# Openflight-sim/OPEN_Ludwig

Hardware: AMD Instinct MI355X
Metric: MLUPS (million lattice updates/s) at 256^3 D3Q27; % of HBM roofline (higher is better)
Workload: dtype f32

## Files before the change

### include/ludwig_hip.h

```cpp
#ifndef LUDWIG_HIP_H
#define LUDWIG_HIP_H

#include <stddef.h>
#include <stdint.h>

#ifdef __cplusplus
extern "C" {
#endif

#define LUDWIG_ABI_VERSION 1

#define LUDWIG_OK              0
#define LUDWIG_ERR_INVALID    -1
#define LUDWIG_ERR_HIP        -2
#define LUDWIG_ERR_NO_DEVICE  -3
#define LUDWIG_ERR_ALLOC      -4
#define LUDWIG_ERR_STATE      -5

enum LudwigField {
    LUDWIG_F = 0,
    LUDWIG_F_TEMP = 1,
    LUDWIG_F_POST = 2,
    LUDWIG_F_OLD = 3,
    LUDWIG_RHO = 4,
// ... 67 lines not shown
int  ludwig_level_upload(LudwigLevel *level, int field, const void *host, size_t bytes);
int  ludwig_level_download(const LudwigLevel *level, int field, void *host, size_t bytes);
int  ludwig_level_block_order(const LudwigLevel *level, int32_t *ref_to_internal);

int  ludwig_level_field_ptr(const LudwigLevel *level, int field, void **device_ptr, size_t *bytes);
int  ludwig_level_field_layout(const LudwigLevel *level, int field, int32_t *components, int64_t *block_stride, int64_t *component_stride);

int  ludwig_init_equilibrium(LudwigLevel *level);

int  ludwig_step(LudwigLevel *level, const LudwigLevel *parent, int64_t t_sub,
                 float u_curr, float parent_tau, float temporal_weight,
                 const LudwigStepFlags *flags);

int  ludwig_stream_collide(LudwigLevel *level, const LudwigLevel *parent, int64_t t_sub,
                           float u_curr, float parent_tau, float temporal_weight,
                           const LudwigStepFlags *flags, int part);
int  ludwig_bouzidi_correction(LudwigLevel *level, int64_t t_sub, float q_min_threshold);

int  ludwig_save_old(LudwigLevel *level, int64_t t_sub);

int  ludwig_execute_timestep_batch(LudwigLevel *const *levels, int32_t n_levels, int64_t t_start, int32_t batch_size,
                                   float u_curr, const LudwigStepFlags *flags);

enum { LUDWIG_OBSERVE_PROBES = 0, LUDWIG_OBSERVE_SURFACE = 1, LUDWIG_OBSERVE_FORCES = 2, LUDWIG_OBSERVE_TRACERS = 3,
       LUDWIG_OBSERVE_FLUXES = 4, LUDWIG_OBSERVE_MODES = 5 };
typedef struct LudwigBatchObserver {
    int32_t kind;
    void   *set;
    int64_t start_step;
    int32_t interval;
} LudwigBatchObserver;
int  ludwig_execute_timestep_batch_observed(LudwigLevel *const *levels, int32_t n_levels, int64_t t_start, int32_t batch_size,
                                            float u_curr, const LudwigStepFlags *flags, const LudwigBatchObserver *observers,
                                            int32_t n_observers);

int  ludwig_sync(const LudwigLevel *level);

typedef struct LudwigSurfaceParams {
    float   dx;
    float   tau;
    float   offset_x, offset_y, offset_z;
    float   pressure_scale, stress_scale;
    int32_t search_radius;
} LudwigSurfaceParams;

int  ludwig_map_surface_stresses(const LudwigLevel *level, int vel_field, int32_t n_triangles, const float *centers,
                                 const float *normals, const LudwigSurfaceParams *sp,
                                 float *pressure, float *shear_x, float *shear_y, float *shear_z);

int  ludwig_level_rho_min(const LudwigLevel *level, float *rho_min);

int  ludwig_level_set_rho_store(LudwigLevel *level, int every_step);

enum LudwigStat { LUDWIG_STAT_RHO = 0, LUDWIG_STAT_VEL = 1, LUDWIG_STAT_VEL2 = 2 };
int  ludwig_level_stats_reset(LudwigLevel *level);
int  ludwig_level_stats_accumulate(LudwigLevel *level, int64_t t_sub);
int  ludwig_level_stats_download(const LudwigLevel *level, int stat, double *host, size_t bytes, int64_t *n_samples);

int  ludwig_level_monitor(LudwigLevel *level, int64_t t_sub, int64_t *counts, int64_t *cells, float *extremes, double *sums);

#define LUDWIG_WALL_BINS 194
typedef struct LudwigWallCensus {
    uint64_t near_cells, evaluated, log_law, forced, non_finite;
    uint32_t min_bits, max_bits;
    uint64_t hist[LUDWIG_WALL_BINS];
} LudwigWallCensus;
int  ludwig_level_wall_census(LudwigLevel *level, int64_t t_sub, LudwigWallCensus *out);

typedef struct LudwigWallSurface LudwigWallSurface;
int  ludwig_wall_surface_create(LudwigLevel *level, int32_t n_tri, const int32_t *blocks, const int32_t *cells, const float *normals,
                                const LudwigSurfaceParams *sp, LudwigWallSurface **out);
void ludwig_wall_surface_destroy(LudwigWallSurface *set);
int  ludwig_wall_surface_compute(LudwigWallSurface *set, int64_t t_sub);
int  ludwig_wall_surface_download(LudwigWallSurface *set, float *values, size_t bytes);

enum LudwigGradField { LUDWIG_GRAD_VORTICITY = 0 , LUDWIG_GRAD_Q = 1  };
int  ludwig_level_gradient_fields_compute(LudwigLevel *level, int vel_field, float scale);
int  ludwig_level_gradient_fields_download(const LudwigLevel *level, int which, float *host, size_t bytes);

enum LudwigIsoScalar { LUDWIG_ISO_DENSITY = 0, LUDWIG_ISO_VELOCITY_MAGNITUDE = 1, LUDWIG_ISO_Q_CRITERION = 2,
                       LUDWIG_ISO_VORTICITY_MAGNITUDE = 3 };
#define LUDWIG_ISO_REFUSED     1
int  ludwig_level_isosurface_extract(LudwigLevel *level, int which, int vel_field, float scale, float value, const uint8_t *skip,
                                     const int32_t *cell_lo, const int32_t *cell_hi, int64_t max_triangles, int64_t *n_triangles);
int  ludwig_level_isosurface_download(LudwigLevel *level, float *positions, size_t position_bytes, float *attributes,
                                      size_t attribute_bytes, int32_t *keys, size_t key_bytes);

typedef struct LudwigProbes LudwigProbes;
int  ludwig_probes_create(LudwigLevel *const *levels, int32_t n_levels, int32_t n_probes, const int32_t *level_index,
                          const int32_t *blocks, const int32_t *cells, const float *weights, int32_t capacity, LudwigProbes **out);
void ludwig_probes_destroy(LudwigProbes *probes);
int  ludwig_probes_sample(LudwigProbes *probes, int32_t level_index, int64_t t_sub);
int  ludwig_probes_download(LudwigProbes *probes, float *values, int64_t *steps, int32_t max_samples, int32_t *n_samples);
int  ludwig_execute_timestep_batch_probes(LudwigLevel *const *levels, int32_t n_levels, int64_t t_start, int32_t batch_size,
                                          float u_curr, const LudwigStepFlags *flags, LudwigProbes *probes, int64_t start_step,
                                          int32_t interval);

typedef struct LudwigSurfaceStats LudwigSurfaceStats;
int  ludwig_surface_stats_create(LudwigLevel *level, int32_t n_tri, const int32_t *blocks, const int32_t *cells, const float *wall_dist,
                                 const float *normals, const LudwigSurfaceParams *sp, LudwigSurfaceStats **out);
void ludwig_surface_stats_destroy(LudwigSurfaceStats *stats);
int  ludwig_surface_stats_reset(LudwigSurfaceStats *stats);
int  ludwig_surface_stats_accumulate(LudwigSurfaceStats *stats, int64_t t_sub);
int  ludwig_surface_stats_download(LudwigSurfaceStats *stats, double *sums, size_t bytes, int64_t *n_samples);

typedef struct LudwigBatchSamplers {
// ... 130 lines not shown
```

### open_ludwig_amd/_lib.py

```python
from __future__ import annotations

import ctypes as C
import os

_HERE = os.path.dirname(os.path.abspath(__file__))
LIB_PATH = os.environ.get("LUDWIG_HIP_LIB") or os.path.join(_HERE, "csrc", "libludwig_hip.so")

F, F_TEMP, F_POST, F_OLD, RHO, RHO_OLD, VEL, VEL_TEMP, VEL_OLD, OBSTACLE, SPONGE, WALL_DIST = range(12)
FIELD_NAMES = {
    "f": F, "f_temp": F_TEMP, "f_post_collision": F_POST, "f_old": F_OLD, "rho": RHO, "rho_old": RHO_OLD,
    "vel": VEL, "vel_temp": VEL_TEMP, "vel_old": VEL_OLD, "obstacle": OBSTACLE, "sponge": SPONGE,
    "wall_dist": WALL_DIST,
}
STAT_RHO, STAT_VEL, STAT_VEL2 = range(3)
STAT_NAMES = {"rho": (STAT_RHO, 1), "vel": (STAT_VEL, 3), "vel2": (STAT_VEL2, 6)}
GRAD_VORTICITY, GRAD_Q = range(2)
GRAD_NAMES = {"vorticity": (GRAD_VORTICITY, 3), "q": (GRAD_Q, 1)}
SLICE_GRADIENT = 1
ISO_NAMES = {"density": 0, "velocity_magnitude": 1, "q_criterion": 2, "vorticity_magnitude": 3}
ISO_REFUSED = 1
SUBGRID_FIELD_NAMES = {"nu": 0, "code": 1}
SUBGRID_SUM_NAMES = {"nu": 0, "nunu": 1, "eps": 2}
PART_ALL, PART_BOUNDARY, PART_INTERIOR = 0, 1, 2

OBSERVE_PROBES, OBSERVE_SURFACE, OBSERVE_FORCES, OBSERVE_TRACERS, OBSERVE_FLUXES = range(5)
OBSERVE_MODES = 5

EXPORTED_SYMBOLS = [
    "ludwig_abi_version", "ludwig_last_error", "ludwig_device_count",
    "ludwig_level_create", "ludwig_level_destroy", "ludwig_level_set_stream", "ludwig_level_add_post_collision_readers", "ludwig_level_set_order",
    "ludwig_level_upload", "ludwig_level_download", "ludwig_level_field_ptr",
    "ludwig_init_equilibrium", "ludwig_step", "ludwig_stream_collide", "ludwig_bouzidi_correction",
    "ludwig_save_old", "ludwig_execute_timestep_batch", "ludwig_execute_timestep_batch_observed", "ludwig_sync", "ludwig_halo_pack", "ludwig_halo_unpack", "ludwig_level_info",
    "ludwig_map_surface_stresses", "ludwig_level_rho_min", "ludwig_level_block_order",
    "ludwig_stream_create", "ludwig_stream_destroy", "ludwig_level_field_layout", "ludwig_level_set_rho_store",
    "ludwig_comm_unique_id", "ludwig_comm_create", "ludwig_comm_destroy", "ludwig_comm_allreduce_f32",
    "ludwig_halo_plan_create", "ludwig_halo_plan_destroy", "ludwig_halo_exchange", "ludwig_halo_wait",
    "ludwig_halo_plan_pack", "ludwig_halo_plan_unpack", "ludwig_halo_plan_buffers", "ludwig_halo_plan_timing", "ludwig_halo_plan_in_stream",
    "ludwig_halo_plan_exchange_ms", "ludwig_step_distributed",
    "ludwig_level_stats_reset", "ludwig_level_stats_accumulate", "ludwig_level_stats_download",
    "ludwig_level_gradient_fields_compute", "ludwig_level_gradient_fields_download",
    "ludwig_level_subgrid_fields_compute", "ludwig_level_subgrid_fields_download", "ludwig_level_subgrid_stats_reset",
    "ludwig_level_subgrid_stats_accumulate", "ludwig_level_subgrid_stats_download",
    "ludwig_probes_create", "ludwig_probes_destroy", "ludwig_probes_sample", "ludwig_probes_download",
    "ludwig_execute_timestep_batch_probes",
    "ludwig_surface_stats_create", "ludwig_surface_stats_destroy", "ludwig_surface_stats_reset", "ludwig_surface_stats_accumulate",
    "ludwig_surface_stats_download", "ludwig_execute_timestep_batch_sampled",
    "ludwig_slices_create", "ludwig_slices_destroy", "ludwig_slices_sample", "ludwig_slices_download",
    "ludwig_streamlines_create", "ludwig_streamlines_destroy", "ludwig_streamlines_trace", "ludwig_streamlines_download",
    "ludwig_tracers_create", "ludwig_tracers_destroy", "ludwig_tracers_advance", "ludwig_tracers_snapshot", "ludwig_tracers_download",
    "ludwig_execute_timestep_batch_tracers",
    "ludwig_level_monitor",
    "ludwig_level_isosurface_extract", "ludwig_level_isosurface_download",
    "ludwig_level_wall_census", "ludwig_wall_surface_create", "ludwig_wall_surface_destroy", "ludwig_wall_surface_compute",
    "ludwig_wall_surface_download",
    "ludwig_force_series_create", "ludwig_force_series_destroy", "ludwig_force_series_sample", "ludwig_force_series_download",
    "ludwig_execute_timestep_batch_loads",
    "ludwig_flux_planes_create", "ludwig_flux_planes_destroy", "ludwig_flux_planes_sample", "ludwig_flux_planes_download",
    "ludwig_modes_create", "ludwig_modes_destroy", "ludwig_modes_reset", "ludwig_modes_accumulate", "ludwig_modes_download",
]
UNIQUE_ID_BYTES = 128
HALO_GROUPS = ("f", "vel", "f_post", "rho")


class LudwigError(RuntimeError):
    def __init__(self, code: int, msg: str):
        super().__init__(f"libludwig_hip error {code}: {msg}")
        self.code = code


class LevelHost(C.Structure):
    _fields_ = [
        ("level_id", C.c_int32), ("n_blocks", C.c_int32), ("n_owned", C.c_int32), ("tau", C.c_float),
        ("grid_dim_x", C.c_int32), ("grid_dim_y", C.c_int32), ("grid_dim_z", C.c_int32),
        ("block_pointer", C.c_void_p), ("neighbor_table", C.c_void_p),
        ("map_x", C.c_void_p), ("map_y", C.c_void_p), ("map_z", C.c_void_p),
        ("obstacle", C.c_void_p), ("sponge", C.c_void_p), ("wall_dist", C.c_void_p),
        ("enable_temporal_interpolation", C.c_int32), ("n_boundary_cells", C.c_int32),
        ("bouzidi_q_map", C.c_void_p), ("bouzidi_cell_block", C.c_void_p),
        ("bouzidi_cell_x", C.c_void_p), ("bouzidi_cell_y", C.c_void_p), ("bouzidi_cell_z", C.c_void_p),
        ("comm_boundary", C.c_void_p), ("store_post_collision_everywhere", C.c_int32),
    ]


class StepFlags(C.Structure):
    _fields_ = [
        ("domain_nx", C.c_int32), ("domain_ny", C.c_int32), ("domain_nz", C.c_int32),
        ("is_symmetric", C.c_int32), ("wall_model_active", C.c_int32), ("use_temporal_interp", C.c_int32),
        ("sponge_blend_distributions", C.c_int32),
        ("c_wale", C.c_float), ("nu_sgs_background", C.c_float), ("inlet_turbulence", C.c_float),
        ("q_min_threshold", C.c_float),
    ]


class SurfaceParams(C.Structure):
    _fields_ = [
        ("dx", C.c_float), ("tau", C.c_float), ("offset_x", C.c_float), ("offset_y", C.c_float), ("offset_z", C.c_float),
        ("pressure_scale", C.c_float), ("stress_scale", C.c_float), ("search_radius", C.c_int32),
    ]


class BatchObserver(C.Structure):
    _fields_ = [("kind", C.c_int32), ("set", C.c_void_p), ("start_step", C.c_int64), ("interval", C.c_int32)]


class BatchSamplers(C.Structure):
    _fields_ = [
        ("probes", C.c_void_p), ("probes_start_step", C.c_int64), ("probes_interval", C.c_int32),
        ("surface", C.c_void_p), ("surface_start_step", C.c_int64), ("surface_interval", C.c_int32),
    ]


# ... 17 lines not shown

class LevelInfo(C.Structure):
    _fields_ = [
        ("n_blocks", C.c_int32), ("n_owned", C.c_int32), ("n_fast_blocks", C.c_int32),
        ("n_general_blocks", C.c_int32), ("n_boundary_cells", C.c_int32),
        ("has_temporal_storage", C.c_int32), ("has_post_collision", C.c_int32), ("n_xrun_blocks", C.c_int32),
        ("device_bytes", C.c_int64),
    ]


_lib = None


def load() -> C.CDLL:
    global _lib
    if _lib is not None:
        return _lib
    if not os.path.exists(LIB_PATH):
        raise FileNotFoundError(
            f"{LIB_PATH} not found: build the HIP extension first (python -c 'import __graft_entry__ as g; g.build()')")
    lib = C.CDLL(LIB_PATH)
    vp, i32, i64, f32 = C.c_void_p, C.c_int, C.c_int64, C.c_float
    sig = {
        "ludwig_abi_version": (C.c_int, []),
        "ludwig_last_error": (C.c_char_p, []),
        "ludwig_device_count": (C.c_int, [C.POINTER(C.c_int)]),
        "ludwig_level_create": (C.c_int, [C.POINTER(LevelHost), i32, C.POINTER(vp)]),
        "ludwig_level_destroy": (None, [vp]),
        "ludwig_level_set_stream": (C.c_int, [vp, vp]),
        "ludwig_level_add_post_collision_readers": (C.c_int, [vp, vp, i64]),
        "ludwig_level_set_order": (C.c_int, [vp, i32, vp, i64]),
        "ludwig_level_upload": (C.c_int, [vp, i32, vp, C.c_size_t]),
        "ludwig_level_download": (C.c_int, [vp, i32, vp, C.c_size_t]),
        "ludwig_level_field_ptr": (C.c_int, [vp, i32, C.POINTER(vp), C.POINTER(C.c_size_t)]),
        "ludwig_init_equilibrium": (C.c_int, [vp]),
        "ludwig_step": (C.c_int, [vp, vp, i64, f32, f32, f32, C.POINTER(StepFlags)]),
        "ludwig_stream_collide": (C.c_int, [vp, vp, i64, f32, f32, f32, C.POINTER(StepFlags), i32]),
        "ludwig_bouzidi_correction": (C.c_int, [vp, i64, f32]),
        "ludwig_save_old": (C.c_int, [vp, i64]),
        "ludwig_execute_timestep_batch": (C.c_int, [C.POINTER(vp), i32, i64, i32, f32, C.POINTER(StepFlags)]),
        "ludwig_execute_timestep_batch_observed": (C.c_int, [C.POINTER(vp), i32, i64, i32, f32, C.POINTER(StepFlags),
                                                             C.POINTER(BatchObserver), i32]),
        "ludwig_sync": (C.c_int, [vp]),
        "ludwig_halo_pack": (C.c_int, [vp, i32, vp, i64, vp, vp]),
        "ludwig_halo_unpack": (C.c_int, [vp, i32, vp, i64, vp, vp]),
        "ludwig_map_surface_stresses": (C.c_int, [vp, i32, i32, vp, vp, C.POINTER(SurfaceParams), vp, vp, vp, vp]),
        "ludwig_level_info": (C.c_int, [vp, C.POINTER(LevelInfo)]),
        "ludwig_level_rho_min": (C.c_int, [vp, C.POINTER(C.c_float)]),
        "ludwig_level_block_order": (C.c_int, [vp, vp]),
        "ludwig_stream_create": (C.c_int, [i32, i32, C.POINTER(vp)]),
        "ludwig_stream_destroy": (C.c_int, [i32, vp]),
        "ludwig_level_field_layout": (C.c_int, [vp, i32, C.POINTER(C.c_int32), C.POINTER(C.c_int64), C.POINTER(C.c_int64)]),
        "ludwig_level_set_rho_store": (C.c_int, [vp, i32]),
        "ludwig_comm_unique_id": (C.c_int, [vp]),
        "ludwig_comm_create": (C.c_int, [vp, i32, i32, i32, C.POINTER(vp)]),
        "ludwig_comm_destroy": (None, [vp]),
        "ludwig_comm_allreduce_f32": (C.c_int, [vp, vp, i32, i32]),
        "ludwig_halo_plan_create": (C.c_int, [vp, vp, C.POINTER(HaloPlanDesc), C.POINTER(vp)]),
        "ludwig_halo_plan_destroy": (None, [vp]),
        "ludwig_halo_exchange": (C.c_int, [vp, i32, vp, vp]),
        "ludwig_halo_wait": (C.c_int, [vp]),
        "ludwig_halo_plan_pack": (C.c_int, [vp, i32, i32, vp]),
        "ludwig_halo_plan_unpack": (C.c_int, [vp, i32, i32, vp]),
        "ludwig_halo_plan_buffers": (C.c_int, [vp, i32, C.POINTER(vp), C.POINTER(i64), C.POINTER(vp), C.POINTER(i64)]),
        "ludwig_halo_plan_timing": (C.c_int, [vp, i32]),
        "ludwig_halo_plan_in_stream": (C.c_int, [vp, i32]),
        "ludwig_halo_plan_exchange_ms": (C.c_int, [vp, vp, i32, C.POINTER(C.c_int32)]),
        "ludwig_step_distributed": (C.c_int, [vp, vp, vp, i64, f32, f32, f32, C.POINTER(StepFlags)]),
        "ludwig_level_stats_reset": (C.c_int, [vp]),
        "ludwig_level_stats_accumulate": (C.c_int, [vp, i64]),
        "ludwig_level_monitor": (C.c_int, [vp, i64, vp, vp, vp, vp]),
        "ludwig_level_stats_download": (C.c_int, [vp, i32, vp, C.c_size_t, C.POINTER(C.c_int64)]),
        "ludwig_level_gradient_fields_compute": (C.c_int, [vp, i32, f32]),
        "ludwig_level_gradient_fields_download": (C.c_int, [vp, i32, vp, C.c_size_t]),
        "ludwig_level_subgrid_fields_compute": (C.c_int, [vp, i32]),
        "ludwig_level_subgrid_fields_download": (C.c_int, [vp, i32, vp, C.c_size_t]),
        "ludwig_level_subgrid_stats_reset": (C.c_int, [vp]),
        "ludwig_level_subgrid_stats_accumulate": (C.c_int, [vp, i64]),
        "ludwig_level_subgrid_stats_download": (C.c_int, [vp, i32, vp, C.c_size_t, C.POINTER(C.c_int64)]),
        "ludwig_probes_create": (C.c_int, [C.POINTER(vp), i32, i32, vp, vp, vp, vp, i32, C.POINTER(vp)]),
        "ludwig_probes_destroy": (None, [vp]),
        "ludwig_probes_sample": (C.c_int, [vp, i32, i64]),
        "ludwig_probes_download": (C.c_int, [vp, vp, vp, i32, C.POINTER(C.c_int32)]),
        "ludwig_execute_timestep_batch_probes": (C.c_int, [C.POINTER(vp), i32, i64, i32, f32, C.POINTER(StepFlags), vp, i64, i32]),
        "ludwig_surface_stats_create": (C.c_int, [vp, i32, vp, vp, vp, vp, C.POINTER(SurfaceParams), C.POINTER(vp)]),
        "ludwig_surface_stats_destroy": (None, [vp]),
        "ludwig_surface_stats_reset": (C.c_int, [vp]),
        "ludwig_surface_stats_accumulate": (C.c_int, [vp, i64]),
        "ludwig_surface_stats_download": (C.c_int, [vp, vp, C.c_size_t, C.POINTER(C.c_int64)]),
        "ludwig_execute_timestep_batch_sampled": (C.c_int, [C.POINTER(vp), i32, i64, i32, f32, C.POINTER(StepFlags), C.POINTER(BatchSamplers)]),
        "ludwig_slices_create": (C.c_int, [C.POINTER(vp), i32, i32, vp, vp, vp, vp, vp, vp, i32, C.POINTER(vp)]),
        "ludwig_slices_destroy": (None, [vp]),
        "ludwig_slices_sample": (C.c_int, [vp, i64]),
        "ludwig_slices_download": (C.c_int, [vp, vp, C.c_size_t]),
        "ludwig_streamlines_create": (C.c_int, [vp, i32, i32, vp, vp, f32, f32, i32, C.POINTER(vp)]),
        "ludwig_streamlines_destroy": (None, [vp]),
        "ludwig_streamlines_trace": (C.c_int, [vp, i64]),
        "ludwig_streamlines_download": (C.c_int, [vp, vp, vp, vp, C.c_size_t]),
        "ludwig_tracers_create": (C.c_int, [vp, i32, i32, vp, i32, i32, f32, C.POINTER(vp)]),
        "ludwig_tracers_destroy": (None, [vp]),
        "ludwig_tracers_advance": (C.c_int, [vp, i64]),
        "ludwig_tracers_snapshot": (C.c_int, [vp, i64]),
        "ludwig_tracers_download": (C.c_int, [vp, vp, C.c_size_t, C.POINTER(C.c_int64)]),
        "ludwig_level_isosurface_extract": (C.c_int, [vp, i32, i32, f32, f32, vp, vp, vp, i64, C.POINTER(C.c_int64)]),
        "ludwig_level_isosurface_download": (C.c_int, [vp, vp, C.c_size_t, vp, C.c_size_t, vp, C.c_size_t]),
        "ludwig_level_wall_census": (C.c_int, [vp, i64, C.POINTER(WallCensus)]),
# ... 104 lines not shown
```

### open_ludwig_amd/blocks.py

```python
from __future__ import annotations

import ctypes as C
from typing import List, Optional, Sequence, Tuple

import numpy as np

from . import _lib

BLOCK_SIZE = 8


def build_lattice_arrays():
    cx, cy, cz, w = [], [], [], []
    for dz in (-1, 0, 1):
        for dy in (-1, 0, 1):
            for dx in (-1, 0, 1):
                cx.append(dx); cy.append(dy); cz.append(dz)
                d2 = dx * dx + dy * dy + dz * dz
                w.append(np.float32(8) / np.float32(27) if d2 == 0 else np.float32(2) / np.float32(27) if d2 == 1
                         else np.float32(1) / np.float32(54) if d2 == 2 else np.float32(1) / np.float32(216))
    cx, cy, cz = (np.array(a, dtype=np.int32) for a in (cx, cy, cz))
    w = np.array(w, dtype=np.float32)
    opp = np.zeros(27, np.int32); my = np.zeros(27, np.int32); mz = np.zeros(27, np.int32)
    for i in range(27):
# ... 204 lines not shown
        return bool(self.info().has_post_collision)

    def add_post_collision_readers(self, offsets: np.ndarray) -> None:
        o = np.ascontiguousarray(offsets, dtype=np.int64)
        _lib.check(self._lib.ludwig_level_add_post_collision_readers(self.handle, o.ctypes.data if o.size else None, o.size))

    def set_stream(self, hip_stream: int) -> None:
        _lib.check(self._lib.ludwig_level_set_stream(self.handle, C.c_void_p(hip_stream)))

    def set_order(self, items: np.ndarray, part: int = _lib.PART_ALL) -> None:
        items = np.ascontiguousarray(items, dtype=np.int32)
        _lib.check(self._lib.ludwig_level_set_order(self.handle, part, items.ctypes.data, items.size))

    def _shape(self, name: str):
        B, n = BLOCK_SIZE, self.n_blocks
        if name in ("f", "f_temp", "f_post_collision", "f_old"):
            return (B, B, B, n, 27)
        if name in ("vel", "vel_temp", "vel_old"):
            return (B, B, B, n, 3)
        return (B, B, B, n)

    def upload(self, name: str, host: np.ndarray) -> None:
        dt = _FIELD_DTYPES.get(name, np.float32)
        a = host.view(np.uint8) if host.dtype == np.bool_ else host
        a = np.asfortranarray(a, dtype=dt)
        if a.shape != self._shape(name):
            raise ValueError(f"{name}: shape {a.shape} != {self._shape(name)}")
        _lib.check(self._lib.ludwig_level_upload(self.handle, _lib.FIELD_NAMES[name], a.ctypes.data, a.nbytes))

    def download(self, name: str) -> np.ndarray:
        dt = _FIELD_DTYPES.get(name, np.float32)
        a = np.empty(self._shape(name), dtype=dt, order="F")
        _lib.check(self._lib.ludwig_level_download(self.handle, _lib.FIELD_NAMES[name], a.ctypes.data, a.nbytes))
        return a.view(np.bool_) if name == "obstacle" else a

    def block_order(self) -> np.ndarray:
        a = np.zeros(self.n_blocks, dtype=np.int32)
        _lib.check(self._lib.ludwig_level_block_order(self.handle, a.ctypes.data))
        return a

    def field_ptr(self, name: str) -> Tuple[int, int]:
        p, n = C.c_void_p(), C.c_size_t()
        _lib.check(self._lib.ludwig_level_field_ptr(self.handle, _lib.FIELD_NAMES[name], C.byref(p), C.byref(n)))
        return p.value, n.value

    def field_layout(self, name: str) -> Tuple[int, int, int]:
        k, bs, cs = C.c_int32(), C.c_int64(), C.c_int64()
        _lib.check(self._lib.ludwig_level_field_layout(self.handle, _lib.FIELD_NAMES[name], C.byref(k), C.byref(bs), C.byref(cs)))
        return int(k.value), int(bs.value), int(cs.value)

    def set_rho_store(self, every_step: bool) -> None:
        _lib.check(self._lib.ludwig_level_set_rho_store(self.handle, 1 if every_step else 0))

    def rho_min(self) -> float:
        v = C.c_float()
        _lib.check(self._lib.ludwig_level_rho_min(self.handle, C.byref(v)))
        return float(v.value)

    def stats_reset(self) -> None:
        _lib.check(self._lib.ludwig_level_stats_reset(self.handle))

    def stats_accumulate(self, t_sub: int) -> None:
        _lib.check(self._lib.ludwig_level_stats_accumulate(self.handle, int(t_sub)))

    def stats_download(self, stat: str) -> Tuple[np.ndarray, int]:
        sid, k = _lib.STAT_NAMES[stat]
        B = BLOCK_SIZE
        a = np.empty((B, B, B, self.n_blocks) + ((k,) if k > 1 else ()), dtype=np.float64, order="F")
        n = C.c_int64(0)
        _lib.check(self._lib.ludwig_level_stats_download(self.handle, sid, a.ctypes.data if a.size else None, a.nbytes, C.byref(n)))
        return a, int(n.value)

    def monitor(self, t_sub: int):
        from . import monitor as monitor_mod
        counts, cells = np.zeros(2, np.int64), np.zeros(16, np.int64)
        extremes, sums = np.zeros(3, np.float32), np.zeros(2, np.float64)
        _lib.check(self._lib.ludwig_level_monitor(self.handle, int(t_sub), counts.ctypes.data, cells.ctypes.data, extremes.ctypes.data,
                                                  sums.ctypes.data))
        return monitor_mod.from_arrays(counts, cells, extremes, sums)

    def gradient_fields(self, vel_name: str, scale) -> Tuple[np.ndarray, np.ndarray]:
        if vel_name not in ("vel", "vel_temp"):
            raise ValueError(f"gradient fields: vel_name must be 'vel' or 'vel_temp', got {vel_name!r}")
        _lib.check(self._lib.ludwig_level_gradient_fields_compute(self.handle, _lib.FIELD_NAMES[vel_name], float(np.float32(scale))))
        B = BLOCK_SIZE
        out = []
        for name in ("vorticity", "q"):
            gid, k = _lib.GRAD_NAMES[name]
            a = np.empty((B, B, B, self.n_blocks) + ((k,) if k > 1 else ()), dtype=np.float32, order="F")
            _lib.check(self._lib.ludwig_level_gradient_fields_download(self.handle, gid, a.ctypes.data if a.size else None, a.nbytes))
            out.append(a)
        return out[0], out[1]

    def isosurface(self, field: str, value, vel_name: str = "vel", scale=1.0, skip=None, cell_lo=(0, 0, 0), cell_hi=None,
                   max_triangles: int = 50_000_000, download: bool = True):
        from .isosurface import CELL_MAX, check_field
        if vel_name not in ("vel", "vel_temp"):
            raise ValueError(f"isosurface: vel_name must be 'vel' or 'vel_temp', got {vel_name!r}")
        which = check_field(field)
        lo = np.ascontiguousarray(cell_lo, dtype=np.int32).reshape(3)
        hi = np.full(3, CELL_MAX, np.int32) if cell_hi is None else np.ascontiguousarray(cell_hi, dtype=np.int32).reshape(3)
        sk = None
        if skip is not None:
            sk = np.ascontiguousarray(skip, dtype=np.uint8).reshape(-1)
            if sk.size != self.n_blocks:
                raise ValueError(f"isosurface: skip has {sk.size} entries for {self.n_blocks} blocks")
# ... 72 lines not shown
```

### open_ludwig_amd/csrc/kernels.hpp

```cpp
#pragma once

#include <hip/hip_runtime.h>
#include <stdint.h>
#include <type_traits>

#include "lattice.hpp"
#include "jl_math.h"

namespace lw {

struct SCParams {
    const float *f_in;
    float *f_out;
    float *f_post;
    const uint32_t *post_rows;
    const float *vel_in;
    float *vel_out;
    float *rho;
    const uint8_t *obstacle;
    const float *sponge;
    const float *wall_dist;
    const int32_t *meta;
    const int32_t *items;
    const float *pf_new, *pf_old, *prho_new, *prho_old, *pvel_new, *pvel_old;
    float tau, tau_parent, c_wale, nu_bg, u_inlet, inlet_turbulence, temporal_weight;
    int32_t is_level_1, is_symmetric, nx_g, ny_g, nz_g;
    int32_t wall_model, seed, use_temporal, sponge_blend;
    float *f_iface;
    int32_t n_iface_blocks;
    int32_t store_rho;
    float *rho_old_save;
};

template <int K, int N, class F>
__device__ __forceinline__ void static_for(F &&f)
{
    if constexpr (K < N) {
        f(std::integral_constant<int, K>{});
        static_for<K + 1, N>(f);
    }
}

__device__ __forceinline__ float jl_max(float a, float b)
{
    return (a != a) ? a : ((b != b) ? b : (a > b ? a : b));
}
__device__ __forceinline__ float jl_clamp(float x, float lo, float hi)
{
    return x > hi ? hi : (x < lo ? lo : x);
}
__device__ __forceinline__ float jl_pow(float x, float y) { return lw_powf(x, y); }
__device__ __forceinline__ float jl_log(float x) { return lw_logf(x); }

template <int C>
__device__ __forceinline__ void acc_signed(float &sum, bool &empty, float v)
{
    if constexpr (C != 0) {
        const float t = C > 0 ? v : -v;
        sum = empty ? t : sum + t;
        empty = false;
    }
}
template <int K>
__device__ __forceinline__ float cdot(float a, float b, float c)
{
    float s = 0.0f;
    bool empty = true;
    acc_signed<CX(K)>(s, empty, a);
    acc_signed<CY(K)>(s, empty, b);
    acc_signed<CZ(K)>(s, empty, c);
    return s;
}

__device__ __forceinline__ float gradient_noise(int32_t gx, int32_t gy, int32_t gz, int32_t seed)
{
    uint32_t h = (uint32_t)gx * 374761393u + (uint32_t)gy * 668265263u + (uint32_t)gz * 1274126177u + (uint32_t)seed;
    h = (h ^ (h >> 16)) * 0x85ebca6bu;
    h = (h ^ (h >> 13)) * 0xc2b2ae35u;
    h = h ^ (h >> 16);
    return ((float)(h & 0xFFFFu) / 32768.0f) - 1.0f;
}

__device__ __forceinline__ float calculate_equilibrium(float rho, float ux, float uy, float uz, float w_k,
                                                       float cx, float cy, float cz)
// ... 110 lines not shown
    const bool xo = cx == 1 ? l.x0 : (cx == -1 ? l.x7 : false);
    const bool yo = cy == 1 ? l.y0 : (cy == -1 ? l.y7 : false);
    const int c00 = n.id[g][4], cX = n.id[g][4 - cx], cY = n.id[g][4 - 3 * cy], cXY = n.id[g][4 - cx - 3 * cy];
    int sel = c00;
    if constexpr (cx != 0 && cy != 0) sel = xo ? (yo ? cXY : cX) : (yo ? cY : c00);
    else if constexpr (cx != 0) sel = xo ? cX : c00;
    else if constexpr (cy != 0) sel = yo ? cY : c00;
    return sel;
}
constexpr int SUBGRID_NO_OP1 = 0, SUBGRID_NO_DENOM = 1, SUBGRID_FLOOR = 2, SUBGRID_MODEL = 3;
struct WaleState {
    float nu_eddy, s2;
    int code;
};
__device__ __forceinline__ WaleState wale_state(float g11, float g12, float g13, float g21, float g22, float g23, float g31, float g32,
                                                float g33, float c_wale, float nu_bg)
{
    const float gsq11 = g11 * g11 + g12 * g21 + g13 * g31;
    const float gsq12 = g11 * g12 + g12 * g22 + g13 * g32;
    const float gsq13 = g11 * g13 + g12 * g23 + g13 * g33;
    const float gsq21 = g21 * g11 + g22 * g21 + g23 * g31;
    const float gsq22 = g21 * g12 + g22 * g22 + g23 * g32;
    const float gsq23 = g21 * g13 + g22 * g23 + g23 * g33;
    const float gsq31 = g31 * g11 + g32 * g21 + g33 * g31;
    const float gsq32 = g31 * g12 + g32 * g22 + g33 * g32;
    const float gsq33 = g31 * g13 + g32 * g23 + g33 * g33;

    const float tr_gsq = gsq11 + gsq22 + gsq33;
    const float tr_term = tr_gsq / 3.0f;
    const float Sd11 = gsq11 - tr_term, Sd22 = gsq22 - tr_term, Sd33 = gsq33 - tr_term;
    const float Sd12 = 0.5f * (gsq12 + gsq21), Sd13 = 0.5f * (gsq13 + gsq31), Sd23 = 0.5f * (gsq23 + gsq32);
    const float S12 = 0.5f * (g12 + g21), S13 = 0.5f * (g13 + g31), S23 = 0.5f * (g23 + g32);
    const float OP1 = Sd11 * Sd11 + Sd22 * Sd22 + Sd33 * Sd33 + 2.0f * (Sd12 * Sd12 + Sd13 * Sd13 + Sd23 * Sd23);
    const float OP2 = g11 * g11 + g22 * g22 + g33 * g33 + 2.0f * (S12 * S12 + S13 * S13 + S23 * S23);

    WaleState w;
    w.code = SUBGRID_NO_OP1;
    float nu_eddy = 0.0f;
    if (OP1 > 1.0e-12f) {
        const float OP1_32 = OP1 * sqrtf(OP1);
        const float OP2_52 = OP2 * OP2 * sqrtf(jl_max(OP2, 1.0e-12f));
        const float denom = OP2_52 + OP1 * sqrtf(sqrtf(jl_max(OP1, 1.0e-12f)));
        w.code = SUBGRID_NO_DENOM;
        if (denom > 1.0e-12f) {
            nu_eddy = (c_wale * c_wale) * OP1_32 / denom;
            w.code = nu_eddy > nu_bg ? SUBGRID_MODEL : SUBGRID_FLOOR;
        }
    }
    w.nu_eddy = jl_max(nu_eddy, nu_bg);
    w.s2 = 2.0f * OP2;
    return w;
}

template <bool POST, bool WALL>
__device__ __forceinline__ void finish_cell(const SCParams &p, const int flags, const Own own, float (&fs)[Q],
                                            const float ux_E, const float uy_E, const float uz_E, const float ux_W, const float uy_W, const float uz_W,
                                            const float ux_N, const float uy_N, const float uz_N, const float ux_S, const float uy_S, const float uz_S,
                                            const float ux_T, const float uy_T, const float uz_T, const float ux_B, const float uy_B, const float uz_B)
{
    float rho = 0.0f, jx = 0.0f, jy = 0.0f, jz = 0.0f;
    static_for<0, Q>([&](auto kc) {
        constexpr int k = decltype(kc)::value;
        constexpr int cx = CX(k), cy = CY(k), cz = CZ(k);
        const float val = fs[k];
        rho += val;
        if constexpr (cx == 1) jx += val; else if constexpr (cx == -1) jx -= val;
        if constexpr (cy == 1) jy += val; else if constexpr (cy == -1) jy -= val;
        if constexpr (cz == 1) jz += val; else if constexpr (cz == -1) jz -= val;
    });

    bool store_post = false;
    if constexpr (POST) {
        if (flags & FLAG_STORE_POST) {
            store_post = true;
            if (p.post_rows) {
                const int zu = __builtin_amdgcn_readfirstlane((int)(own.cell4 >> 8));
                const uint32_t w = p.post_rows[(size_t)own.b * 2 + (zu >> 2)];
                store_post = ((w >> ((zu & 3) * 8 + ((own.cell4 >> 5) & 7))) & 1u) != 0;
            }
        }
    }
    bool is_obs = false;
    if (flags & FLAG_HAS_OBSTACLE) is_obs = p.obstacle[(size_t)own.b * CELLS + (own.cell4 >> 2)] != 0;
    if (is_obs) {
        st_f32(p.vel_out, own.b, V_BLOCK_BYTES, own.cell4, 0.0f);
        st_f32(p.vel_out, own.b, V_BLOCK_BYTES, COMP_BYTES + own.cell4, 0.0f);
        st_f32(p.vel_out, own.b, V_BLOCK_BYTES, 2 * COMP_BYTES + own.cell4, 0.0f);
        if (p.rho_old_save) st_f32(p.rho_old_save, own.b, S_BLOCK_BYTES, own.cell4, ld_own(p.rho, own.b, S_BLOCK_BYTES, own.cell4));
        if (p.store_rho) st_f32(p.rho, own.b, S_BLOCK_BYTES, own.cell4, 1.0f);
        static_for<0, Q>([&](auto kc) {
            constexpr int k = decltype(kc)::value;
            const float f_coll = fs[OPP(k)];
            st_f32(p.f_out, own.b, F_BLOCK_BYTES, k * COMP_BYTES + own.cell4, f_coll);
            if constexpr (POST) { if (store_post) st_f32(p.f_post, own.b, F_BLOCK_BYTES, k * COMP_BYTES + own.cell4, f_coll); }
        });
        return;
    }

    rho = jl_max(rho, 0.01f);
    const float inv_rho = 1.0f / rho;
    float ux = jx * inv_rho, uy = jy * inv_rho, uz = jz * inv_rho;

    if (flags & FLAG_HAS_SPONGE) {
        const float sp = ld_own(p.sponge, own.b, S_BLOCK_BYTES, own.cell4);
        if (sp > 0.0f) {
            const float rho_target = 1.0f, ux_target = p.u_inlet;
            rho = rho * (1.0f - sp) + rho_target * sp;
            ux = ux * (1.0f - sp) + ux_target * sp;
            uy = uy * (1.0f - sp);
            uz = uz * (1.0f - sp);
            if (p.sponge_blend == 1) {
                static_for<0, Q>([&](auto kc) {
                    constexpr int k = decltype(kc)::value;
                    const float feq_target = calculate_equilibrium(rho_target, ux_target, 0.0f, 0.0f, WEIGHT(k),
                                                                   (float)CX(k), (float)CY(k), (float)CZ(k));
                    fs[k] = fs[k] * (1.0f - sp) + feq_target * sp;
                });
            }
        }
    }

    float Fx = 0.0f, Fy = 0.0f, Fz = 0.0f;
    float ux_eq = ux, uy_eq = uy, uz_eq = uz;
    if constexpr (WALL) {
        if (flags & FLAG_HAS_NEAR_WALL) {
            const float u_mag = sqrtf(ux * ux + uy * uy + uz * uz);
            const float force_mag = wall_model_force_mag(ld_own(p.wall_dist, own.b, S_BLOCK_BYTES, own.cell4), p.tau, rho, u_mag);
            if (force_mag >= 0.0f) {
                Fx = -force_mag * ux / u_mag;
                Fy = -force_mag * uy / u_mag;
                Fz = -force_mag * uz / u_mag;
            }
        }
        ux_eq = ux + 0.5f * Fx * inv_rho;
        uy_eq = uy + 0.5f * Fy * inv_rho;
        uz_eq = uz + 0.5f * Fz * inv_rho;
    }
    const float usq_eq = ux_eq * ux_eq + uy_eq * uy_eq + uz_eq * uz_eq;

    st_f32(p.vel_out, own.b, V_BLOCK_BYTES, own.cell4, ux);
    st_f32(p.vel_out, own.b, V_BLOCK_BYTES, COMP_BYTES + own.cell4, uy);
    st_f32(p.vel_out, own.b, V_BLOCK_BYTES, 2 * COMP_BYTES + own.cell4, uz);
    if (p.rho_old_save) st_f32(p.rho_old_save, own.b, S_BLOCK_BYTES, own.cell4, ld_own(p.rho, own.b, S_BLOCK_BYTES, own.cell4));
    if (p.store_rho) st_f32(p.rho, own.b, S_BLOCK_BYTES, own.cell4, rho);

    const float g11 = 0.5f * (ux_E - ux_W), g12 = 0.5f * (ux_N - ux_S), g13 = 0.5f * (ux_T - ux_B);
    const float g21 = 0.5f * (uy_E - uy_W), g22 = 0.5f * (uy_N - uy_S), g23 = 0.5f * (uy_T - uy_B);
    const float g31 = 0.5f * (uz_E - uz_W), g32 = 0.5f * (uz_N - uz_S), g33 = 0.5f * (uz_T - uz_B);

    const float gsq11 = g11 * g11 + g12 * g21 + g13 * g31;
    const float gsq12 = g11 * g12 + g12 * g22 + g13 * g32;
    const float gsq13 = g11 * g13 + g12 * g23 + g13 * g33;
    const float gsq21 = g21 * g11 + g22 * g21 + g23 * g31;
    const float gsq22 = g21 * g12 + g22 * g22 + g23 * g32;
    const float gsq23 = g21 * g13 + g22 * g23 + g23 * g33;
    const float gsq31 = g31 * g11 + g32 * g21 + g33 * g31;
    const float gsq32 = g31 * g12 + g32 * g22 + g33 * g32;
    const float gsq33 = g31 * g13 + g32 * g23 + g33 * g33;

    const float tr_gsq = gsq11 + gsq22 + gsq33;
    const float tr_term = tr_gsq / 3.0f;
    const float Sd11 = gsq11 - tr_term, Sd22 = gsq22 - tr_term, Sd33 = gsq33 - tr_term;
    const float Sd12 = 0.5f * (gsq12 + gsq21), Sd13 = 0.5f * (gsq13 + gsq31), Sd23 = 0.5f * (gsq23 + gsq32);
    const float S12 = 0.5f * (g12 + g21), S13 = 0.5f * (g13 + g31), S23 = 0.5f * (g23 + g32);
    const float OP1 = Sd11 * Sd11 + Sd22 * Sd22 + Sd33 * Sd33 + 2.0f * (Sd12 * Sd12 + Sd13 * Sd13 + Sd23 * Sd23);
    const float OP2 = g11 * g11 + g22 * g22 + g33 * g33 + 2.0f * (S12 * S12 + S13 * S13 + S23 * S23);

    float nu_eddy = 0.0f;
    if (OP1 > 1.0e-12f) {
        const float OP1_32 = OP1 * sqrtf(OP1);
        const float OP2_52 = OP2 * OP2 * sqrtf(jl_max(OP2, 1.0e-12f));
        const float denom = OP2_52 + OP1 * sqrtf(sqrtf(jl_max(OP1, 1.0e-12f)));
        if (denom > 1.0e-12f) nu_eddy = (p.c_wale * p.c_wale) * OP1_32 / denom;
    }
    nu_eddy = jl_max(nu_eddy, p.nu_bg);
    const float tau_turb = p.tau + nu_eddy * 3.0f;
    const float omega = 1.0f / jl_max(tau_turb, 0.500001f);

    float Pi_xx = 0.0f, Pi_yy = 0.0f, Pi_zz = 0.0f, Pi_xy = 0.0f, Pi_yz = 0.0f, Pi_zx = 0.0f;
    static_for<0, Q>([&](auto kc) {
        constexpr int k = decltype(kc)::value;
        constexpr int cx = CX(k), cy = CY(k), cz = CZ(k);
        const float cu = cdot<k>(ux_eq, uy_eq, uz_eq);
        const float feq = rho * WEIGHT(k) * (1.0f + 3.0f * cu + 4.5f * cu * cu - 1.5f * usq_eq);
        const float f_neq = fs[k] - feq;
        if constexpr (cx != 0) Pi_xx += f_neq;
        if constexpr (cy != 0) Pi_yy += f_neq;
        if constexpr (cz != 0) Pi_zz += f_neq;
        if constexpr (cx * cy == 1) Pi_xy += f_neq; else if constexpr (cx * cy == -1) Pi_xy -= f_neq;
        if constexpr (cy * cz == 1) Pi_yz += f_neq; else if constexpr (cy * cz == -1) Pi_yz -= f_neq;
        if constexpr (cz * cx == 1) Pi_zx += f_neq; else if constexpr (cz * cx == -1) Pi_zx -= f_neq;
    });

    const float one_m_omega = 1.0f - omega;
    const float one_m_half_omega = 1.0f - 0.5f * omega;
    static_for<0, Q>([&](auto kc) {
        constexpr int k = decltype(kc)::value;
        constexpr int cx = CX(k), cy = CY(k), cz = CZ(k);
        constexpr float w_k = WEIGHT(k);
        constexpr float cx_f = (float)cx, cy_f = (float)cy, cz_f = (float)cz;
        const float cu = cdot<k>(ux_eq, uy_eq, uz_eq);
        const float feq = rho * w_k * (1.0f + 3.0f * cu + 4.5f * cu * cu - 1.5f * usq_eq);
        constexpr float Q_xx = cx_f * cx_f - CS2_PHYSICS, Q_yy = cy_f * cy_f - CS2_PHYSICS, Q_zz = cz_f * cz_f - CS2_PHYSICS;
        float od = 0.0f;
        bool od_empty = true;
        acc_signed<cx * cy>(od, od_empty, Pi_xy);
        acc_signed<cy * cz>(od, od_empty, Pi_yz);
        acc_signed<cz * cx>(od, od_empty, Pi_zx);
        float inner = Pi_xx * Q_xx + Pi_yy * Q_yy + Pi_zz * Q_zz;
        if constexpr (cx * cy != 0 || cy * cz != 0 || cz * cx != 0) inner = inner + 2.0f * od;
        const float f_neq_reg = (w_k * 4.5f) * inner;
        float f_coll = feq + one_m_omega * f_neq_reg;
        if constexpr (WALL) {
            const float force_term = (w_k * 3.0f) * ((cx_f - ux + 3.0f * cu * cx_f) * Fx + (cy_f - uy + 3.0f * cu * cy_f) * Fy +
                                                     (cz_f - uz + 3.0f * cu * cz_f) * Fz);
            f_coll = f_coll + one_m_half_omega * force_term;
        }
        if constexpr (POST) { if (store_post) st_f32(p.f_post, own.b, F_BLOCK_BYTES, k * COMP_BYTES + own.cell4, f_coll); }
        st_f32(p.f_out, own.b, F_BLOCK_BYTES, k * COMP_BYTES + own.cell4, f_coll);
    });
}

__device__ __forceinline__ void finish_rho_only(const SCParams &p, const int flags, const Own own, const float (&fs)[Q])
{
    float rho = 0.0f;
    static_for<0, Q>([&](auto kc) { rho += fs[decltype(kc)::value]; });
    bool is_obs = false;
    if (flags & FLAG_HAS_OBSTACLE) is_obs = p.obstacle[(size_t)own.b * CELLS + (own.cell4 >> 2)] != 0;
    if (is_obs) { st_f32(p.rho, own.b, S_BLOCK_BYTES, own.cell4, 1.0f); return; }
    rho = jl_max(rho, 0.01f);
    if (flags & FLAG_HAS_SPONGE) {
        const float sp = ld_own(p.sponge, own.b, S_BLOCK_BYTES, own.cell4);
        if (sp > 0.0f) rho = rho * (1.0f - sp) + 1.0f * sp;
    }
    st_f32(p.rho, own.b, S_BLOCK_BYTES, own.cell4, rho);
}

__device__ __forceinline__ void patch_missing_sources(const SCParams &p, const int32_t *__restrict__ meta, const NeighbourIds &nbr,
                                                      const LanePos &l, const int z, const Own own, float (&fs)[Q])
{
    const int gx = (meta[NBR_BX] - 1) * BS + l.x + 1, gy = (meta[NBR_BY] - 1) * BS + l.y + 1, gz = (meta[NBR_BZ] - 1) * BS + z + 1;
    const float *iface_own = p.is_level_1 == 0 ? p.f_iface + (size_t)meta[NBR_GBI] * CELLS + (own.cell4 >> 2) : nullptr;
    static_for<0, Q>([&](auto kc) {
        constexpr int k = decltype(kc)::value;
        constexpr int cx = CX(k), cy = CY(k), cz = CZ(k);
        if constexpr (k != 13) {
            if (source_block<k>(nbr, l) < 0) {
                const int src_gx = gx - cx, src_gy = gy - cy, src_gz = gz - cz;
                const bool is_inlet = src_gx < 1, is_outlet = src_gx > p.nx_g;
                const bool is_y_min = src_gy < 1, is_y_max = src_gy > p.ny_g;
                const bool is_z_min = src_gz < 1, is_z_max = src_gz > p.nz_g;
                float val;
                if (is_inlet) {
                    const float noise = p.inlet_turbulence > 0.0f
                                            ? gradient_noise(gy, gz, p.seed, 1234) * p.inlet_turbulence * p.u_inlet
                                            : 0.0f;
                    const float u_inst = p.u_inlet + noise;
                    const float cu_in = (float)cx * u_inst;
                    val = WEIGHT(k) * (1.0f + 3.0f * cu_in + 4.5f * cu_in * cu_in - 1.5f * u_inst * u_inst);
                } else if (is_outlet) {
                    const float cu_out = (float)cx * p.u_inlet;
                    val = WEIGHT(k) * (1.0f + 3.0f * cu_out + 4.5f * cu_out * cu_out - 1.5f * p.u_inlet * p.u_inlet);
                } else if (is_y_min && p.is_symmetric == 1) {
                    val = ld_own(p.f_in, own.b, F_BLOCK_BYTES, MIRROR_Y(k) * COMP_BYTES + own.cell4);
                } else if (is_y_min || is_y_max) {
                    val = ld_own(p.f_in, own.b, F_BLOCK_BYTES, MIRROR_Y(k) * COMP_BYTES + own.cell4);
                } else if (is_z_min || is_z_max) {
                    val = ld_own(p.f_in, own.b, F_BLOCK_BYTES, MIRROR_Z(k) * COMP_BYTES + own.cell4);
                } else if (p.is_level_1 == 0) {
                    val = iface_own[(size_t)k * p.n_iface_blocks * CELLS];
                } else {
                    val = WEIGHT(k);
                }
                fs[k] = val;
            }
        }
    });
}

__device__ __forceinline__ float dpp_from_lower_lane(float v)
{
    return __int_as_float(__builtin_amdgcn_update_dpp(__float_as_int(v), __float_as_int(v), 0x111, 0xF, 0xF, false));
}
__device__ __forceinline__ float dpp_from_upper_lane(float v)
{
    return __int_as_float(__builtin_amdgcn_update_dpp(__float_as_int(v), __float_as_int(v), 0x101, 0xF, 0xF, false));
}
__host__ __device__ constexpr int XSLOT(int k) { return CX(k) == 1 ? k / 3 : 9 + k / 3; }

constexpr int ITEM_LINK_W = 1 << 30;
constexpr int ITEM_LINK_E = 1 << 29;
constexpr int ITEM_ID_MASK = (1 << 29) - 1;

#ifndef LW_MIN_WAVES
#define LW_MIN_WAVES 5
#endif
template <int NW, bool GENERAL, bool POST, bool WALL, bool RHO_ONLY = false, bool WIDE = false>
__global__ __launch_bounds__(64 * NW) __attribute__((amdgpu_waves_per_eu((WIDE && GENERAL) ? LW_MIN_WAVES - 1 : LW_MIN_WAVES))) void k_stream_collide_xrun(const SCParams p)
{
    __shared__ float xch[NW][24][8];
    const int wave = __builtin_amdgcn_readfirstlane(threadIdx.x >> 6);
    const int raw = p.items[blockIdx.x * NW + wave];
    const bool active = raw >= 0;
    const int item = active ? (raw & ITEM_ID_MASK) : 0;
    const int b = item >> 3;
    const int z = item & 7;
    const int lane = threadIdx.x & 63;
    LanePos l;
    l.x = lane & 7; l.y = lane >> 3;
    l.x0 = l.x == 0; l.x7 = l.x == 7; l.y0 = l.y == 0; l.y7 = l.y == 7;
    const int32_t *__restrict__ meta = p.meta + (size_t)b * NBR_STRIDE;
    const int flags = meta[NBR_FLAGS];
    const NeighbourIds nbr = load_neighbour_ids(meta, z);
    const Own own{b, (uint32_t)((l.x + 8 * l.y + 64 * z) * 4)};
    const bool first = !active || (raw & ITEM_LINK_W) == 0, last = !active || (raw & ITEM_LINK_E) == 0;
    float fs[Q];
    float halo[Q];
    float uc[3], uT[3], uB[3], uy_edge[3], ux_edge_lo[3], ux_edge_hi[3];
    if (active) {
    static_for<0, Q>([&](auto kc) {
        constexpr int k = decltype(kc)::value;
        constexpr int cx = CX(k), cy = CY(k), g = 1 - CZ(k);
        const bool yo = cy == 1 ? l.y0 : (cy == -1 ? l.y7 : false);
        const int c00 = nbr.id[g][4], cY = nbr.id[g][4 - 3 * cy];
        int sel = cy != 0 ? (yo ? cY : c00) : c00;
        if constexpr (GENERAL) sel = sel >= 0 ? sel : b;
        const uint32_t rowz = (uint32_t)(k * COMP_BYTES) + (uint32_t)((8 * ((l.y - cy) & 7)) * 4) + (uint32_t)(nbr.zs[g] * 256);
        if constexpr (cy == 0) fs[k] = ld_f32<true>(p.f_in, sel, F_BLOCK_BYTES, rowz + (uint32_t)(l.x * 4));
        else fs[k] = ld_f32<WIDE>(p.f_in, sel, F_BLOCK_BYTES, rowz + (uint32_t)(l.x * 4));
        halo[k] = 0.0f;
        if constexpr (cx != 0) {
            if (cx == 1 ? first : last) {
                const int cX = nbr.id[g][4 - cx], cXY = nbr.id[g][4 - cx - 3 * cy];
                int selx = cy != 0 ? (yo ? cXY : cX) : cX;
                if constexpr (GENERAL) selx = selx >= 0 ? selx : b;
                if (cx == 1 ? l.x0 : l.x7)
                    halo[k] = ld_f32<(cy == 0) || WIDE>(p.f_in, selx, F_BLOCK_BYTES, rowz + (uint32_t)((cx == 1 ? 7 : 0) * 4));
            }
        }
    });
    if constexpr (!RHO_ONLY) {
        int bT = z == 7 ? nbr.id[2][4] : b, bB = z == 0 ? nbr.id[0][4] : b;
        const uint32_t xy = (uint32_t)((l.x + 8 * l.y) * 4);
        uint32_t inT = xy + (uint32_t)(((z + 1) & 7) * 256), inB = xy + (uint32_t)(((z - 1) & 7) * 256);
        int by_ = l.y0 ? nbr.id[1][4 - 3] : nbr.id[1][4 + 3];
        uint32_t inY = (uint32_t)((l.x + 8 * (l.y0 ? 7 : 0) + 64 * z) * 4);
        int bXlo = nbr.id[1][4 - 1], bXhi = nbr.id[1][4 + 1];
        uint32_t inXlo = (uint32_t)((7 + 8 * l.y + 64 * z) * 4), inXhi = (uint32_t)((0 + 8 * l.y + 64 * z) * 4);
        if constexpr (GENERAL) {
            if (bT < 0) { bT = b; inT = own.cell4; }
            if (bB < 0) { bB = b; inB = own.cell4; }
// ... 14 lines not shown
        }
    }

    static_for<0, Q>([&](auto kc) {
        constexpr int k = decltype(kc)::value;
        constexpr int cx = CX(k);
        if constexpr (cx == 1) { if (l.x7) xch[wave][XSLOT(k)][l.y] = fs[k]; }
        if constexpr (cx == -1) { if (l.x0) xch[wave][XSLOT(k)][l.y] = fs[k]; }
    });
    if constexpr (!RHO_ONLY) {
#pragma unroll
        for (int c = 0; c < 3; ++c) {
            if (l.x7) xch[wave][18 + c][l.y] = uc[c];
            if (l.x0) xch[wave][21 + c][l.y] = uc[c];
        }
    }
    }
    __syncthreads();
    if (!active) return;
    const int wlo = first ? 0 : wave - 1, whi = last ? NW - 1 : wave + 1;
    static_for<0, Q>([&](auto kc) {
        constexpr int k = decltype(kc)::value;
        constexpr int cx = CX(k);
        if constexpr (cx == 1) {
            const float inner = dpp_from_lower_lane(fs[k]);
            const float edge = first ? halo[k] : xch[wlo][XSLOT(k)][l.y];
            fs[k] = l.x0 ? edge : inner;
        }
        if constexpr (cx == -1) {
            const float inner = dpp_from_upper_lane(fs[k]);
            const float edge = last ? halo[k] : xch[whi][XSLOT(k)][l.y];
            fs[k] = l.x7 ? edge : inner;
        }
    });
    const bool needs_patch = GENERAL && (flags & FLAG_ALL_NEIGHBOURS) == 0;
    if constexpr (RHO_ONLY) {
        if constexpr (GENERAL) { if (needs_patch) patch_missing_sources(p, meta, nbr, l, z, own, fs); }
        finish_rho_only(p, flags, own, fs);
        return;
    }
    float uE[3], uW[3], uN[3], uS[3];
#pragma unroll
    for (int c = 0; c < 3; ++c) {
        const float e_edge = last ? ux_edge_hi[c] : xch[whi][21 + c][l.y];
        const float w_edge = first ? ux_edge_lo[c] : xch[wlo][18 + c][l.y];
        const float e_in = dpp_from_upper_lane(uc[c]), w_in = dpp_from_lower_lane(uc[c]);
        uE[c] = l.x7 ? e_edge : e_in;
        uW[c] = l.x0 ? w_edge : w_in;
        const float n_in = __shfl_down(uc[c], 8, 64), s_in = __shfl_up(uc[c], 8, 64);
        uN[c] = l.y7 ? uy_edge[c] : n_in;
        uS[c] = l.y0 ? uy_edge[c] : s_in;
    }
    if constexpr (GENERAL) { if (needs_patch) patch_missing_sources(p, meta, nbr, l, z, own, fs); }
    finish_cell<POST, WALL>(p, flags, own, fs, uE[0], uE[1], uE[2], uW[0], uW[1], uW[2], uN[0], uN[1], uN[2], uS[0], uS[1], uS[2],
                            uT[0], uT[1], uT[2], uB[0], uB[1], uB[2]);
}

__device__ __forceinline__ float weight_rt(int k)
{
    const int cx = k % 3 - 1, cy = (k / 3) % 3 - 1, cz = k / 9 - 1;
    const int d2 = cx * cx + cy * cy + cz * cz;
    return d2 == 0 ? WEIGHT(13) : d2 == 1 ? WEIGHT(12) : d2 == 2 ? WEIGHT(9) : WEIGHT(0);
}

struct InterfaceArgs {
    const int4 *corners;
    const float4 *weights;
    float4 *mac, *mac2;
    const int4 *links;
    float *f_iface2;
    float tw2;
    int n_sources, n_links;
};

__device__ __forceinline__ float blend_in_time(bool blend, float v_old, float v_new, float tw)
{
    return blend ? v_old * (1.0f - tw) + v_new * tw : v_new;
}

template <bool TWO>
__global__ __launch_bounds__(256) void k_interface_sources(const SCParams p, const InterfaceArgs a)
{
    const int i = blockIdx.x * 256 + threadIdx.x;
    if (i >= a.n_sources) return;
    const int4 c0 = a.corners[2 * i], c1 = a.corners[2 * i + 1];
    const int cc[8] = {c0.x, c0.y, c0.z, c0.w, c1.x, c1.y, c1.z, c1.w};
    const float4 w = a.weights[i];
    const float tw = p.temporal_weight, tw2 = a.tw2;
    const bool blend = p.use_temporal == 1 && tw < 0.99f, blend2 = TWO && p.use_temporal == 1 && tw2 < 0.99f;
    float v1[4][8], v2[4][8];
#pragma unroll
    for (int n = 0; n < 8; ++n) {
        v1[0][n] = 1.0f; v1[1][n] = 0.0f; v1[2][n] = 0.0f; v1[3][n] = 0.0f;
        v2[0][n] = 1.0f; v2[1][n] = 0.0f; v2[2][n] = 0.0f; v2[3][n] = 0.0f;
        if (cc[n] >= 0) {
            const int c = cc[n];
            const size_t cv = (size_t)(c >> 9) * (3 * CELLS) + (c & 511);
            const float vn[4] = {p.prho_new[c], p.pvel_new[cv], p.pvel_new[cv + CELLS], p.pvel_new[cv + 2 * CELLS]};
            float vo[4] = {0.0f, 0.0f, 0.0f, 0.0f};
            if (blend || blend2) { vo[0] = p.prho_old[c]; vo[1] = p.pvel_old[cv]; vo[2] = p.pvel_old[cv + CELLS]; vo[3] = p.pvel_old[cv + 2 * CELLS]; }
#pragma unroll
            for (int q = 0; q < 4; ++q) {
                v1[q][n] = blend_in_time(blend, vo[q], vn[q], tw);
                if (TWO) v2[q][n] = blend_in_time(blend2, vo[q], vn[q], tw2);
            }
        }
    }
#pragma unroll
// ... 1562 lines not shown
```

### open_ludwig_amd/csrc/ludwig_hip.hip

```cpp
#include <hip/hip_runtime.h>

#include <algorithm>
#include <climits>
#include <cstdarg>
#include <cstdio>
#include <cstdlib>
#include <cstring>
#include <ctime>
#include <new>
#include <string>
#include <vector>

#include "../../include/ludwig_hip.h"
#include "all_or_nothing.hpp"
#include "kernels.hpp"

using namespace lw;

namespace {

thread_local std::string g_err;

int fail(int code, const char *fmt, ...)
{
    char buf[512];
    va_list ap;
    va_start(ap, fmt);
    vsnprintf(buf, sizeof buf, fmt, ap);
    va_end(ap);
    g_err = buf;
    return code;
}

#define LW_HIP(call)                                                                                      \
    do {                                                                                                  \
        hipError_t e_ = (call);                                                                           \
        if (e_ != hipSuccess) return fail(LUDWIG_ERR_HIP, "%s failed: %s (%s:%d)", #call, hipGetErrorString(e_), __FILE__, __LINE__); \
    } while (0)

constexpr int N_PARTS = 3, N_CLASSES = 3;
constexpr int XRUN = 4, XRUN_MAX = 4;

namespace env {

bool is_set(const char *name) { return getenv(name) != nullptr; }
int flag(const char *name) { const char *e = getenv(name); return e ? (atoi(e) != 0 ? 1 : 0) : -1; }

int merge_classes() { return flag("LUDWIG_MERGE_CLASSES"); }
bool reference_block_order() { return is_set("LUDWIG_REFERENCE_BLOCK_ORDER"); }
bool wide_addr() { return is_set("LUDWIG_WIDE_ADDR"); }
bool full_post_collision() { return is_set("LUDWIG_FULL_POST_COLLISION"); }
bool post_rows_off() { const char *e = getenv("LUDWIG_POST_ROWS"); return e && e[0] == '0'; }
bool eager_rho() { static const bool v = is_set("LUDWIG_EAGER_RHO"); return v; }
bool no_iface_ahead() { return is_set("LUDWIG_NO_IFACE_AHEAD"); }
bool rho_old_copy() { return is_set("LUDWIG_RHO_OLD_COPY"); }
bool batch_serial() { static const bool v = is_set("LUDWIG_BATCH_SERIAL"); return v; }
bool child_side_iface() { static const bool v = is_set("LUDWIG_CHILD_SIDE_IFACE"); return v; }
int iface_hoist() { static const int v = flag("LUDWIG_IFACE_HOIST"); return v; }
int level_stream_priority() { const char *e = getenv("LUDWIG_LEVEL_STREAM_PRIORITY"); return e ? atoi(e) : 1; }
const char *rccl_lib() { return getenv("LUDWIG_RCCL_LIB"); }
bool halo_self_via_rccl() { return is_set("LUDWIG_HALO_SELF_VIA_RCCL"); }
bool halo_trace() { static const bool v = is_set("LUDWIG_HALO_TRACE"); return v; }

}

}

struct LudwigLevel {
    int device = 0;
    hipStream_t stream = nullptr;
    int level_id = 1, n_blocks = 0, n_owned = 0;
    float tau = 1.0f;
    int gdx = 0, gdy = 0, gdz = 0;
    int64_t sk = 0;
    bool wide = false;
    float *f[2] = {nullptr, nullptr};
    float *vel[2] = {nullptr, nullptr};
    float *rho = nullptr, *f_post = nullptr, *f_old = nullptr, *rho_old = nullptr, *vel_old = nullptr;
    uint8_t *obstacle = nullptr;
    float *sponge = nullptr, *wall_dist = nullptr;
    int32_t *meta = nullptr;
    bool has_temporal = false, has_post = false, bouzidi_enabled = false;
    int old_alias = -1;
    bool external_writer = false;
    int n_bc = 0;
    int4 *bouzidi_links = nullptr;
    int n_bouzidi_links = 0;
    uint32_t *post_rows = nullptr;
    std::vector<uint32_t> h_post_rows;
    int post_mode = 0;
    bool post_rows_used = false;
    _Float16 *q_map = nullptr;
    int32_t *cell_block = nullptr;
    int8_t *cell_x = nullptr, *cell_y = nullptr, *cell_z = nullptr;
    std::vector<int32_t> ref2int, int2ref;
    bool x_fastest_memory = false;
    int32_t *d_ref2int = nullptr;
    void *scratch = nullptr;
    std::vector<int32_t> h_meta;
    std::vector<uint8_t> h_comm_boundary;
    int32_t *items[N_PARTS][N_CLASSES] = {};
    int64_t n_items[N_PARTS][N_CLASSES] = {};
    int32_t *items_merged[N_PARTS] = {};
    int64_t n_items_merged[N_PARTS] = {};
    int n_fast_blocks = 0;
    bool general_in_runs[N_PARTS] = {};
    int64_t n_linked_items[N_PARTS] = {};
    int64_t device_bytes = 0;
    int n_iface_blocks = 0;
    float *f_iface = nullptr;
    int4 *links[N_PARTS] = {};
    int4 *sources[N_PARTS] = {};
    float4 *source_w[N_PARTS] = {};
    float4 *source_mac[N_PARTS] = {};
    float4 *source_mac2[N_PARTS] = {};
// ... 19 lines not shown
    };
    IfaceKey ahead[N_PARTS];
    IfaceKey prepared[N_PARTS];
    bool rho_eager = false;
    struct RhoReplay {
        bool stale = false;
        int64_t t_sub = -1;
        SCParams p;
    } rho_replay[N_PARTS];
    int64_t step_count = 0, last_step_t = -1, last_replay_step = -10;
    hipStream_t own_stream = nullptr;
    hipEvent_t parent_wait = nullptr;
    bool rho_old_pending = false;
    float *f_iface_b = nullptr, *f_iface2_b = nullptr;
    float4 *mac_b = nullptr, *mac2_b = nullptr;
    IfaceKey pair_ready;
    hipEvent_t ev_pair_done[2] = {nullptr, nullptr};
    bool pair_done_set[2] = {false, false};
    hipEvent_t ev_stepped = nullptr;
    hipEvent_t ev_consumed = nullptr;
    bool ev_consumed_set = false;
    uint64_t stepped_gen = 0;
    const LudwigLevel *waited_parent = nullptr;
    uint64_t waited_gen = 0;
    uint64_t version = 0;
    const LudwigLevel *iface_parent = nullptr;
    std::vector<int32_t> h_block_pointer;
    int n_links[N_PARTS] = {};
    int n_sources[N_PARTS] = {};
    int iface_dims[3] = {-1, -1, -1};
    double *stats = nullptr;
    bool stats_ready = false;
    int64_t stats_n = 0;
    float *grad = nullptr;
    bool grad_ready = false;
    bool wale_known = false;
    float c_wale = 0.0f, nu_bg = 0.0f;
    float *subgrid_fields = nullptr;
    bool subgrid_fields_ready = false;
    double *subgrid_sums = nullptr;
    bool subgrid_stats_ready = false;
    int64_t subgrid_n = 0;
    MonitorRecord *monitor_slab = nullptr;
    WallCensusRecord *wall_census = nullptr;
    float *iso_scalar = nullptr;
    int32_t *iso_counts = nullptr;
    int64_t *iso_offsets = nullptr;
    uint8_t *iso_skip = nullptr;
    int32_t *d_int2ref = nullptr;
    float *iso_pos = nullptr, *iso_att = nullptr;
    int32_t *iso_keys = nullptr;
    int64_t iso_capacity = 0;
    int64_t iso_n = -1;
};

namespace {

template <class T>
int dev_alloc(LudwigLevel *L, T **p, size_t count)
{
    *p = nullptr;
    if (count == 0) return LUDWIG_OK;
    hipError_t e = hipMalloc((void **)p, count * sizeof(T));
    if (e != hipSuccess) return fail(LUDWIG_ERR_ALLOC, "hipMalloc(%zu bytes) failed: %s", count * sizeof(T), hipGetErrorString(e));
    L->device_bytes += (int64_t)(count * sizeof(T));
    return LUDWIG_OK;
}

int fill(LudwigLevel *L, float *a, int64_t n, float v)
{
    if (n == 0) return LUDWIG_OK;
    hipLaunchKernelGGL(k_fill, dim3((unsigned)((n + 255) / 256)), dim3(256), 0, L->stream, a, n, v);
    LW_HIP(hipGetLastError());
    return LUDWIG_OK;
}

struct FieldDesc {
    void *ptr;
    size_t bytes;
    int comps = 1;
    int es = 4;
};

int ensure_rho(LudwigLevel *L);

int materialize_old(LudwigLevel *L)
{
    if (L->old_alias < 0) return LUDWIG_OK;
    ++L->version;
    const size_t c = (size_t)L->sk;
    const int a = L->old_alias;
    L->old_alias = -1;
    LW_HIP(hipSetDevice(L->device));
    LW_HIP(hipMemcpyAsync(L->f_old, L->f[a], c * Q * 4, hipMemcpyDeviceToDevice, L->stream));
    LW_HIP(hipMemcpyAsync(L->vel_old, L->vel[a], c * 3 * 4, hipMemcpyDeviceToDevice, L->stream));
    return LUDWIG_OK;
}

int before_external_write(LudwigLevel *L, int field)
{
    bool feeds_rho = field == LUDWIG_SPONGE || field == LUDWIG_OBSTACLE || field == LUDWIG_RHO;
    for (int a = 0; a < N_PARTS; ++a)
        if (L->rho_replay[a].stale && (field == LUDWIG_F || field == LUDWIG_F_TEMP) && L->f[field == LUDWIG_F ? 0 : 1] == L->rho_replay[a].p.f_in) feeds_rho = true;
    if (feeds_rho) {
        const int r = ensure_rho(L);
        if (r) return r;
    }
    if (L->old_alias < 0) return LUDWIG_OK;
    const int a = L->old_alias;
    const bool hits = field == LUDWIG_F_OLD || field == LUDWIG_VEL_OLD || (field == LUDWIG_F && a == 0) || (field == LUDWIG_F_TEMP && a == 1) ||
                      (field == LUDWIG_VEL && a == 0) || (field == LUDWIG_VEL_TEMP && a == 1);
    return hits ? materialize_old(L) : LUDWIG_OK;
}

FieldDesc field_desc(const LudwigLevel *L, int field)
{
    const size_t c = (size_t)L->sk;
    if (L->old_alias >= 0) {
        if (field == LUDWIG_F_OLD) return {L->f[L->old_alias], L->has_temporal ? c * Q * 4 : 0, Q, 4};
        if (field == LUDWIG_VEL_OLD) return {L->vel[L->old_alias], L->has_temporal ? c * 3 * 4 : 0, 3, 4};
    }
    switch (field) {
    case LUDWIG_F: return {L->f[0], c * Q * 4, Q, 4};
    case LUDWIG_F_TEMP: return {L->f[1], c * Q * 4, Q, 4};
    case LUDWIG_F_POST: return {L->f_post, L->has_post ? c * Q * 4 : 0, Q, 4};
    case LUDWIG_F_OLD: return {L->f_old, L->has_temporal ? c * Q * 4 : 0, Q, 4};
    case LUDWIG_RHO: return {L->rho, c * 4, 1, 4};
    case LUDWIG_RHO_OLD: return {L->rho_old, L->has_temporal ? c * 4 : 0, 1, 4};
    case LUDWIG_VEL: return {L->vel[0], c * 3 * 4, 3, 4};
    case LUDWIG_VEL_TEMP: return {L->vel[1], c * 3 * 4, 3, 4};
    case LUDWIG_VEL_OLD: return {L->vel_old, L->has_temporal ? c * 3 * 4 : 0, 3, 4};
    case LUDWIG_OBSTACLE: return {L->obstacle, c, 1, 1};
    case LUDWIG_SPONGE: return {L->sponge, c * 4, 1, 4};
    case LUDWIG_WALL_DIST: return {L->wall_dist, c * 4, 1, 4};
    default: return {nullptr, 0, 1, 4};
    }
}

void scan_flags(LudwigLevel *L, int field, const void *host)
{
    const int flag = field == LUDWIG_OBSTACLE ? FLAG_HAS_OBSTACLE : field == LUDWIG_SPONGE ? FLAG_HAS_SPONGE : FLAG_HAS_NEAR_WALL;
    for (int b = 0; b < L->n_blocks; ++b) {
        bool any = false;
        if (host) {
            if (field == LUDWIG_OBSTACLE) {
                const uint8_t *o = (const uint8_t *)host + (size_t)b * CELLS;
                for (int i = 0; i < CELLS && !any; ++i) any = o[i] != 0;
            } else if (field == LUDWIG_SPONGE) {
                const float *s = (const float *)host + (size_t)b * CELLS;
                for (int i = 0; i < CELLS && !any; ++i) any = s[i] > 0.0f;
            } else {
                const float *d = (const float *)host + (size_t)b * CELLS;
                for (int i = 0; i < CELLS && !any; ++i) any = d[i] > 0.0f && d[i] < 10.0f;
            }
        }
        int32_t &fl = L->h_meta[(size_t)b * NBR_STRIDE + NBR_FLAGS];
        fl = any ? (fl | flag) : (fl & ~flag);
    }
}

int upload_meta(LudwigLevel *L)
{
    if (L->n_blocks == 0) return LUDWIG_OK;
    LW_HIP(hipMemcpyAsync(L->meta, L->h_meta.data(), L->h_meta.size() * 4, hipMemcpyHostToDevice, L->stream));
    LW_HIP(hipStreamSynchronize(L->stream));
    return LUDWIG_OK;
}

bool block_in_part(const LudwigLevel *L, int b, int part)
{
    if (b >= L->n_owned) return false;
    if (part == LUDWIG_PART_ALL) return true;
    const bool bnd = !L->h_comm_boundary.empty() && L->h_comm_boundary[b] != 0;
    return part == LUDWIG_PART_BOUNDARY ? bnd : !bnd;
}

constexpr int MERGE_BELOW_BLOCKS = 8192;
bool merge_classes(const LudwigLevel *L, const std::vector<int32_t> &general, const std::vector<int32_t> &fast)
{
    if (general.empty() || fast.empty()) return false;
    const int e = env::merge_classes();
    return e >= 0 ? e != 0 : L->n_owned < MERGE_BELOW_BLOCKS;
}

int set_items(LudwigLevel *L, int part, const int32_t *items, int64_t n)
{
    std::vector<int32_t> cls[N_CLASSES];
    auto is_fast = [&](int b) { return (L->h_meta[(size_t)b * NBR_STRIDE + NBR_FLAGS] & FLAG_ALL_NEIGHBOURS) != 0; };
    for (int64_t i = 0; i < n; ++i) {
        if (items[i] >= 0) {
            const int b = items[i] >> 3;
            if (b < 0 || b >= L->n_owned) return fail(LUDWIG_ERR_INVALID, "work item %lld: block %d is not an owned block", (long long)i, b);
            if (!block_in_part(L, b, part)) return fail(LUDWIG_ERR_INVALID, "work item %lld: block %d is not in part %d", (long long)i, b, part);
        }
    }
    const bool use_xrun = true;
    L->general_in_runs[part] = true;
    {
        std::vector<int32_t> loose[2];
        for (int64_t g = 0; g < n; g += XRUN) {
            const int64_t m = std::min<int64_t>(XRUN, n - g);
            int n_fast = 0, n_gen = 0;
            for (int64_t w = 0; w < m; ++w)
                if (items[g + w] >= 0) (is_fast(items[g + w] >> 3) ? n_fast : n_gen)++;
            const bool pure = m == XRUN && (n_fast == 0 || n_gen == 0);
            for (int64_t w = 0; w < m; ++w) {
                const int32_t it = items[g + w];
                if (pure) { if (n_fast + n_gen > 0) cls[n_gen > 0 ? 1 : 2].push_back(it); }
                else if (it >= 0) loose[is_fast(it >> 3) ? 0 : 1].push_back(it);
            }
        }
        for (int c = 1; c <= 2; ++c) {
            const std::vector<int32_t> &lo = loose[c == 2 ? 0 : 1];
            cls[c].insert(cls[c].end(), lo.begin(), lo.end());
            while (cls[c].size() % XRUN) cls[c].push_back(-1);
            for (size_t g = 0; g < cls[c].size(); g += XRUN)
                for (int w = 0; w + 1 < XRUN; ++w) {
                    const int32_t a = cls[c][g + w], d = cls[c][g + w + 1];
                    if (a < 0 || d < 0 || (a & 7) != (d & 7)) continue;
                    const int ba = (a & ITEM_ID_MASK) >> 3, bd = d >> 3;
                    if (ba == bd || L->h_meta[(size_t)ba * NBR_STRIDE + DIR(1, 0, 0)] != bd) continue;
                    cls[c][g + w] |= ITEM_LINK_E;
                    cls[c][g + w + 1] |= ITEM_LINK_W;
                }
        }
        L->n_linked_items[part] = 0;
        for (int32_t it : cls[2])
            if (it >= 0 && (it & (ITEM_LINK_E | ITEM_LINK_W))) ++L->n_linked_items[part];
    }
    std::vector<int32_t> merged;
    if (use_xrun && merge_classes(L, cls[1], cls[2])) {
        merged = cls[2];
        merged.insert(merged.end(), cls[1].begin(), cls[1].end());
    }
    if (L->items_merged[part]) { (void)hipFree(L->items_merged[part]); L->items_merged[part] = nullptr; }
    L->n_items_merged[part] = (int64_t)merged.size();
    if (!merged.empty()) {
        LW_HIP(hipMalloc((void **)&L->items_merged[part], merged.size() * 4));
        LW_HIP(hipMemcpy(L->items_merged[part], merged.data(), merged.size() * 4, hipMemcpyHostToDevice));
    }
// ... 285 lines not shown
    return LUDWIG_OK;
}

static int make_second_iface_set(LudwigLevel *C, size_t n_side, size_t n_src)
{
    if (C->f_iface_b) return LUDWIG_OK;
    void **const bufs[4] = {(void **)&C->f_iface_b, (void **)&C->f_iface2_b, (void **)&C->mac_b, (void **)&C->mac2_b};
    const size_t bytes[4] = {n_side * sizeof(float), n_side * sizeof(float), n_src * sizeof(float4), n_src * sizeof(float4)};
    hipEvent_t *const evs[2] = {&C->ev_pair_done[0], &C->ev_pair_done[1]};
    hipError_t e = hipSuccess;
    const bool made = lw::make_all_or_nothing(
        bufs, bytes, evs, [&](void **q, size_t n) { return (e = hipMalloc(q, n)) == hipSuccess; }, [](void *q) { (void)hipFree(q); },
        [&](hipEvent_t *ev) { return (e = hipEventCreateWithFlags(ev, hipEventDisableTiming)) == hipSuccess; },
        [](hipEvent_t ev) { (void)hipEventDestroy(ev); });
    if (!made) return fail(LUDWIG_ERR_HIP, "second set of interface side buffers: %s", hipGetErrorString(e));
    C->device_bytes += (int64_t)(bytes[0] + bytes[1] + bytes[2] + bytes[3]);
    return LUDWIG_OK;
}

static int interface_pass_for_child(LudwigLevel *parent, LudwigLevel *C, int64_t t_pair, const LudwigStepFlags *fl)
{
    const int part = LUDWIG_PART_ALL;
    if (C->n_blocks == 0 || C->n_items[part][1] == 0 || parent->external_writer) return LUDWIG_OK;
    SCParams p{};
    fill_pass_params(p, C, parent, 2 * t_pair, parent->tau, 0.0f, fl);
    int rc = build_interface_links(C, parent, p.nx_g, p.ny_g, p.nz_g);
    if (rc) return rc;
    if (C->n_links[part] == 0) return LUDWIG_OK;
    if ((rc = make_second_iface_set(C, (size_t)C->n_iface_blocks * CELLS * Q, (size_t)C->n_sources[part]))) return rc;
    const int set = (int)(t_pair & 1);
    if (C->pair_done_set[set]) LW_HIP(hipStreamWaitEvent(parent->stream, C->ev_pair_done[set], 0));
    if ((rc = launch_interface_kernels(C, part, p, iface_buffers(C, part, set), true, parent->stream))) return rc;
    C->pair_ready.fill(parent, t_pair, 0.0f, parent->tau, p.use_temporal);
    C->pair_ready.set = set;
    C->ahead[part].valid = false;
    C->prepared[part].valid = false;
    return LUDWIG_OK;
}

static int interface_prepass(LudwigLevel *L, const LudwigLevel *parent, int64_t t_sub, float parent_tau, float temporal_weight,
                             const LudwigStepFlags *fl)
{
    const int part = LUDWIG_PART_ALL;
    if (!parent || L->n_blocks == 0 || L->n_items[part][1] == 0) return LUDWIG_OK;
    LW_HIP(hipSetDevice(L->device));
    SCParams p{};
    fill_pass_params(p, L, parent, t_sub, parent_tau, temporal_weight, fl);
    IfaceState state;
    const int r = interface_decide(L, parent, part, p, t_sub, parent_tau, temporal_weight, true, &state);
    if (r || state != IFACE_LAUNCH) return r;
    return interface_launch(L, parent, part, p, t_sub, parent_tau, temporal_weight, true, L->stream);
}

int launch_stream_collide(LudwigLevel *L, const LudwigLevel *parent, int64_t t_sub, float u_curr, float parent_tau,
                          float temporal_weight, const LudwigStepFlags *fl, int part)
{
    if (!L || !fl) return fail(LUDWIG_ERR_INVALID, "null level or flags");
    if (part < 0 || part >= N_PARTS) return fail(LUDWIG_ERR_INVALID, "bad part %d", part);
    if (t_sub < 0) return fail(LUDWIG_ERR_INVALID, "t_sub must be >= 0");
    L->wale_known = true;
    L->c_wale = fl->c_wale;
    L->nu_bg = fl->nu_sgs_background;
    if (L->n_blocks == 0) return LUDWIG_OK;
    if (parent && parent->device != L->device) return fail(LUDWIG_ERR_INVALID, "parent level lives on another device");
    LW_HIP(hipSetDevice(L->device));
    const int in = (t_sub % 2 == 0) ? 0 : 1, out = 1 - in;
    ++L->version;
    if (L->old_alias == out) {
        const int r = materialize_old(L);
        if (r) return r;
    }
    SCParams p{};
    p.f_in = L->f[in];
    p.f_out = L->f[out];
    p.vel_in = L->vel[in];
    p.vel_out = L->vel[out];
    p.rho = L->rho;
    p.f_post = L->has_post ? L->f_post : nullptr;
    p.post_rows = (p.f_post && fl->q_min_threshold >= 0.0f) ? L->post_rows : nullptr;
    if (p.f_post) L->post_rows_used = p.post_rows != nullptr;
    p.obstacle = L->obstacle;
    p.sponge = L->sponge;
    p.wall_dist = L->wall_dist;
    p.meta = L->meta;
    fill_pass_params(p, L, parent, t_sub, parent_tau, temporal_weight, fl);
    p.c_wale = fl->c_wale;
    p.nu_bg = fl->nu_sgs_background;
    p.u_inlet = u_curr;
    p.inlet_turbulence = fl->inlet_turbulence;
    p.is_symmetric = fl->is_symmetric ? 1 : 0;
    p.wall_model = fl->wall_model_active ? 1 : 0;
    p.seed = (int32_t)(t_sub % 1000000);
    p.sponge_blend = fl->sponge_blend_distributions ? 1 : 0;

    if (parent && !parent->rho_eager) {
        LudwigLevel *pm = const_cast<LudwigLevel *>(parent);
        pm->rho_eager = true;
        const int r = ensure_rho(pm);
        if (r) return r;
    }
    {
        if (t_sub != L->last_step_t) { ++L->step_count; L->last_step_t = t_sub; }
        const bool store = env::eager_rho() || L->rho_eager || part != LUDWIG_PART_ALL;
        if (part != LUDWIG_PART_ALL && L->rho_replay[LUDWIG_PART_ALL].stale) {
            const int r = ensure_rho(L);
            if (r) return r;
        }
        L->rho_replay[LUDWIG_PART_ALL].stale = false;
        p.store_rho = store ? 1 : 0;
        if (L->rho_old_pending) {
            if (part == LUDWIG_PART_ALL && store) p.rho_old_save = L->rho_old;
            else LW_HIP(hipMemcpyAsync(L->rho_old, L->rho, (size_t)L->sk * 4, hipMemcpyDeviceToDevice, L->stream));
            L->rho_old_pending = false;
        }
    }

    const bool post = p.f_post != nullptr, wall = p.wall_model != 0;
    const hipStream_t cs = L->stream;
    auto launch_list = [&](const int32_t *items, int64_t n_items, bool general) -> int {
        if (n_items == 0) return LUDWIG_OK;
        p.items = items;
        const dim3 grid((unsigned)(n_items / XRUN)), block(64 * XRUN);
#define LW_LAUNCH_X(G, P, W) do { if (L->wide) hipLaunchKernelGGL((k_stream_collide_xrun<XRUN, G, P, W, false, true>), grid, block, 0, cs, p); \
            else hipLaunchKernelGGL((k_stream_collide_xrun<XRUN, G, P, W, false, false>), grid, block, 0, cs, p); } while (0)
        if (general) {
            if (wall) LW_LAUNCH_X(true, true, true);
            else LW_LAUNCH_X(true, true, false);
        } else {
            if (wall) LW_LAUNCH_X(false, true, true);
            else if (post) LW_LAUNCH_X(false, true, false);
            else LW_LAUNCH_X(false, false, false);
        }
#undef LW_LAUNCH_X
        LW_HIP(hipGetLastError());
        return LUDWIG_OK;
    };
    const hipEvent_t parent_wait = L->parent_wait;
    L->parent_wait = nullptr;
    IfaceState istate;
    {
        const int r = interface_decide(L, parent, part, p, t_sub, parent_tau, temporal_weight, false, &istate);
        if (r) return r;
    }
    {
        if (parent_wait) LW_HIP(hipStreamWaitEvent(cs, parent_wait, 0));
        int r;
        if (istate == IFACE_LAUNCH && (r = interface_launch(L, parent, part, p, t_sub, parent_tau, temporal_weight, false, cs))) return r;
        if (L->n_items_merged[part] > 0) {
            if ((r = launch_list(L->items_merged[part], L->n_items_merged[part], true))) return r;
        } else {
            if ((r = launch_list(L->items[part][1], L->n_items[part][1], true))) return r;
            if ((r = launch_list(L->items[part][2], L->n_items[part][2], false))) return r;
        }
    }
    if (!p.store_rho) {
        LudwigLevel::RhoReplay &rr = L->rho_replay[part];
        rr.stale = true;
        rr.t_sub = t_sub;
        rr.p = p;
    }
    return LUDWIG_OK;
}

int ensure_rho(LudwigLevel *L)
{
    bool any = false;
    for (int a = 0; a < N_PARTS; ++a) any = any || L->rho_replay[a].stale;
    if (!any) return LUDWIG_OK;
    LW_HIP(hipSetDevice(L->device));
    if (L->last_replay_step == L->step_count - 1) L->rho_eager = true;
    L->last_replay_step = L->step_count;
    for (int part = 0; part < N_PARTS; ++part) {
        LudwigLevel::RhoReplay &rr = L->rho_replay[part];
        if (!rr.stale) continue;
        SCParams p = rr.p;
        p.store_rho = 1;
        for (int c = 1; c < N_CLASSES; ++c) {
            if (L->n_items[part][c] == 0) continue;
            p.items = L->items[part][c];
            const bool general = c == 1;
            const dim3 grid((unsigned)(L->n_items[part][c] / XRUN)), block(64 * XRUN);
            if (L->wide) {
                if (general) hipLaunchKernelGGL((k_stream_collide_xrun<XRUN, true, false, false, true, true>), grid, block, 0, L->stream, p);
                else hipLaunchKernelGGL((k_stream_collide_xrun<XRUN, false, false, false, true, true>), grid, block, 0, L->stream, p);
            } else {
                if (general) hipLaunchKernelGGL((k_stream_collide_xrun<XRUN, true, false, false, true, false>), grid, block, 0, L->stream, p);
                else hipLaunchKernelGGL((k_stream_collide_xrun<XRUN, false, false, false, true, false>), grid, block, 0, L->stream, p);
            }
            LW_HIP(hipGetLastError());
        }
        rr.stale = false;
    }
    return LUDWIG_OK;
}

int launch_bouzidi(LudwigLevel *L, int64_t t_sub, float q_min)
{
    if (!L) return fail(LUDWIG_ERR_INVALID, "null level");
    if (!(L->bouzidi_enabled && L->n_bc > 0)) return LUDWIG_OK;
    if (q_min < 0.0f && L->post_rows_used)
        return fail(LUDWIG_ERR_STATE, "q_min_threshold < 0 makes every direction a link: the stream-collide call must be given the same "
                                      "threshold (it stored f_post_collision for the links with q > 0 only)");
    ++L->version;
    LW_HIP(hipSetDevice(L->device));
    const int out = (t_sub % 2 == 0) ? 1 : 0;
    BouzidiParams p{};
    p.f_out = L->f[out];
    p.f_post = L->f_post;
    p.q_map = L->q_map;
    p.cell_block = L->cell_block;
    p.cell_x = L->cell_x; p.cell_y = L->cell_y; p.cell_z = L->cell_z;
    p.meta = L->meta;
    p.n_cells = L->n_bc;
    const bool compact = q_min >= 0.0f && L->bouzidi_links;
    p.links = compact ? L->bouzidi_links : nullptr;
    p.n_links = L->n_bouzidi_links;
    p.q_min = q_min;
    const int64_t n_threads = compact ? (int64_t)L->n_bouzidi_links : (int64_t)L->n_bc * Q;
// ... 51 lines not shown
        e = hipGetLastError();
        if (e == hipSuccess) e = hipMemcpyAsync((char *)host + (size_t)k * plane, tmp, plane, hipMemcpyDeviceToHost, L->stream);
        if (e == hipSuccess) e = hipStreamSynchronize(L->stream);
    }
    (void)hipFree(tmp);
    if (e != hipSuccess) return fail(LUDWIG_ERR_HIP, "%s: %s", what, hipGetErrorString(e));
    return LUDWIG_OK;
}

template <class T>
void upload_table(hipError_t &e, const std::vector<T> &h, T *&dev)
{
    if (e == hipSuccess) e = hipMalloc((void **)&dev, h.size() * sizeof(T));
    if (e == hipSuccess) e = hipMemcpy(dev, h.data(), h.size() * sizeof(T), hipMemcpyHostToDevice);
}

}

extern "C" {

int ludwig_abi_version(void) { return LUDWIG_ABI_VERSION; }

const char *ludwig_last_error(void) { return g_err.c_str(); }

int ludwig_device_count(int *count)
{
    if (!count) return fail(LUDWIG_ERR_INVALID, "null count");
    int n = 0;
    hipError_t e = hipGetDeviceCount(&n);
    if (e != hipSuccess) { *count = 0; return fail(LUDWIG_ERR_NO_DEVICE, "hipGetDeviceCount: %s", hipGetErrorString(e)); }
    *count = n;
    return LUDWIG_OK;
}

void ludwig_level_destroy(LudwigLevel *L)
{
    if (!L) return;
    (void)hipSetDevice(L->device);
    void *ptrs[] = {L->f[0], L->f[1], L->vel[0], L->vel[1], L->rho, L->f_post, L->f_old, L->rho_old, L->vel_old, L->obstacle,
                    L->sponge, L->wall_dist, L->meta, L->q_map, L->cell_block, L->cell_x, L->cell_y, L->cell_z};
    for (void *p : ptrs)
        if (p) (void)hipFree(p);
    for (int a = 0; a < N_PARTS; ++a) {
        for (int c = 0; c < N_CLASSES; ++c)
            if (L->items[a][c]) (void)hipFree(L->items[a][c]);
        if (L->items_merged[a]) (void)hipFree(L->items_merged[a]);
        if (L->links[a]) (void)hipFree(L->links[a]);
        if (L->sources[a]) (void)hipFree(L->sources[a]);
        if (L->source_w[a]) (void)hipFree(L->source_w[a]);
        if (L->source_mac[a]) (void)hipFree(L->source_mac[a]);
        if (L->source_mac2[a]) (void)hipFree(L->source_mac2[a]);
    }
    if (L->f_iface) (void)hipFree(L->f_iface);
    if (L->stats) (void)hipFree(L->stats);
    if (L->grad) (void)hipFree(L->grad);
    if (L->subgrid_fields) (void)hipFree(L->subgrid_fields);
    if (L->subgrid_sums) (void)hipFree(L->subgrid_sums);
    if (L->monitor_slab) (void)hipFree(L->monitor_slab);
    if (L->wall_census) (void)hipFree(L->wall_census);
    {
        void *iso[] = {L->iso_scalar, L->iso_counts, L->iso_offsets, L->iso_skip, L->d_int2ref, L->iso_pos, L->iso_att, L->iso_keys};
        for (void *q : iso)
            if (q) (void)hipFree(q);
    }
    if (L->d_ref2int) (void)hipFree(L->d_ref2int);
    if (L->scratch) (void)hipFree(L->scratch);
    if (L->own_stream) (void)hipStreamDestroy(L->own_stream);
    if (L->ev_stepped) (void)hipEventDestroy(L->ev_stepped);
    if (L->ev_consumed) (void)hipEventDestroy(L->ev_consumed);
    if (L->bouzidi_links) (void)hipFree(L->bouzidi_links);
    if (L->post_rows) (void)hipFree(L->post_rows);
    if (L->f_iface2) (void)hipFree(L->f_iface2);
    {
        void *more[] = {L->f_iface_b, L->f_iface2_b, L->mac_b, L->mac2_b};
        for (void *q : more)
            if (q) (void)hipFree(q);
        for (hipEvent_t ev : L->ev_pair_done)
            if (ev) (void)hipEventDestroy(ev);
    }
    delete L;
}

static int level_create_impl(const LudwigLevelHost *h, int device, LudwigLevel **out, bool x_fastest_memory);

int ludwig_level_create(const LudwigLevelHost *h, int device, LudwigLevel **out)
{
    if (out) *out = nullptr;
    if (!h || !out) return fail(LUDWIG_ERR_INVALID, "null argument");
    const int32_t nb = h->n_blocks;
    if (nb <= 1 || env::reference_block_order() || !h->neighbor_table || !h->map_x || !h->map_y || !h->map_z)
        return level_create_impl(h, device, out, false);
    const int n_owned = h->n_owned > 0 ? h->n_owned : (h->n_owned < 0 ? 0 : nb);
    if (n_owned > nb) return fail(LUDWIG_ERR_INVALID, "n_owned > n_blocks");
    std::vector<int32_t> int2ref((size_t)nb), ref2int((size_t)nb);
    for (int32_t b = 0; b < nb; ++b) int2ref[b] = b;
    std::stable_sort(int2ref.begin(), int2ref.end(), [&](int32_t a, int32_t c) {
        const bool oa = a < n_owned, oc = c < n_owned;
        if (oa != oc) return oa;
        if (h->map_z[a] != h->map_z[c]) return h->map_z[a] < h->map_z[c];
        if (h->map_y[a] != h->map_y[c]) return h->map_y[a] < h->map_y[c];
        return h->map_x[a] < h->map_x[c];
    });
    for (int32_t i = 0; i < nb; ++i) ref2int[int2ref[i]] = i;
    LudwigLevelHost hp = *h;
    const size_t n = (size_t)nb;
    std::vector<int32_t> nt(n * 27), mx(n), my(n), mz(n), bp, cellb;
// ... 334 lines not shown
        if (items[i] < 0) continue;
        ++real;
        const int b = items[i] >> 3;
        if (b >= L->n_owned) return fail(LUDWIG_ERR_INVALID, "bad work item %lld", (long long)i);
        if (seen[(size_t)items[i]]++) return fail(LUDWIG_ERR_INVALID, "work item %lld listed twice", (long long)i);
    }
    if (real != expect) return fail(LUDWIG_ERR_INVALID, "order has %lld work items, part has %lld", (long long)real, (long long)expect);
    if (L->ref2int.empty()) return set_items(L, part, items, n_items);
    std::vector<int32_t> tr(items, items + n_items);
    for (int32_t &it : tr)
        if (it >= 0) it = (L->ref2int[it >> 3] << 3) | (it & 7);
    return set_items(L, part, tr.data(), n_items);
}

int ludwig_level_upload(LudwigLevel *L, int field, const void *host, size_t bytes)
{
    if (!L || !host) return fail(LUDWIG_ERR_INVALID, "null argument");
    const FieldDesc d = field_desc(L, field);
    if (!d.ptr || d.bytes == 0) return fail(LUDWIG_ERR_STATE, "field %d is not allocated on this level", field);
    if (bytes != d.bytes) return fail(LUDWIG_ERR_INVALID, "field %d: got %zu bytes, expected %zu", field, bytes, d.bytes);
    LW_HIP(hipSetDevice(L->device));
    ++L->version;
    {
        const int r = before_external_write(L, field);
        if (r) return r;
    }
    const size_t es = (size_t)d.es;
    {
        const FieldDesc dn = field_desc(L, field);
        const int r = copy_field(L, dn.ptr, const_cast<void *>(host), dn.comps, es, true);
        if (r) return r;
    }
    if (field == LUDWIG_OBSTACLE || field == LUDWIG_SPONGE || field == LUDWIG_WALL_DIST) {
        if (!L->ref2int.empty()) {
            std::vector<char> tmp(bytes);
            for (size_t i = 0; i < (size_t)L->n_blocks; ++i)
                memcpy(&tmp[i * CELLS * es], (const char *)host + (size_t)L->int2ref[i] * CELLS * es, CELLS * es);
            scan_flags(L, field, tmp.data());
        } else {
            scan_flags(L, field, host);
        }
        return upload_meta(L);
    }
    return LUDWIG_OK;
}

int ludwig_level_download(const LudwigLevel *L, int field, void *host, size_t bytes)
{
    if (!L || !host) return fail(LUDWIG_ERR_INVALID, "null argument");
    const FieldDesc d = field_desc(L, field);
    if (!d.ptr || d.bytes == 0) return fail(LUDWIG_ERR_STATE, "field %d is not allocated on this level", field);
    if (bytes != d.bytes) return fail(LUDWIG_ERR_INVALID, "field %d: got %zu bytes, expected %zu", field, bytes, d.bytes);
    LW_HIP(hipSetDevice(L->device));
    if (field == LUDWIG_RHO) {
        const int r = ensure_rho(const_cast<LudwigLevel *>(L));
        if (r) return r;
    }
    return copy_field(const_cast<LudwigLevel *>(L), d.ptr, host, d.comps, (size_t)d.es, false);
}

int ludwig_level_block_order(const LudwigLevel *L, int32_t *ref_to_internal)
{
    if (!L || (!ref_to_internal && L->n_blocks > 0)) return fail(LUDWIG_ERR_INVALID, "null argument");
    for (int32_t b = 0; b < L->n_blocks; ++b) ref_to_internal[b] = L->ref2int.empty() ? b : L->ref2int[b];
    return LUDWIG_OK;
}

int ludwig_level_field_ptr(const LudwigLevel *L, int field, void **device_ptr, size_t *bytes)
{
    if (!L || !device_ptr) return fail(LUDWIG_ERR_INVALID, "null argument");
    ++const_cast<LudwigLevel *>(L)->version;
    {
        const int r = before_external_write(const_cast<LudwigLevel *>(L), field);
        if (r) return r;
    }
    const FieldDesc d = field_desc(L, field);
    if (!d.ptr || d.bytes == 0) return fail(LUDWIG_ERR_STATE, "field %d is not allocated on this level", field);
    if (field != LUDWIG_OBSTACLE && field != LUDWIG_SPONGE && field != LUDWIG_WALL_DIST) {
        LudwigLevel *m = const_cast<LudwigLevel *>(L);
        m->external_writer = true;
        m->rho_eager = true;
    }
    *device_ptr = d.ptr;
    if (bytes) *bytes = d.bytes;
    return LUDWIG_OK;
}

int ludwig_level_set_rho_store(LudwigLevel *L, int every_step)
{
    if (!L) return fail(LUDWIG_ERR_INVALID, "null level");
    if (every_step) {
        const int r = ensure_rho(L);
        if (r) return r;
        L->rho_eager = true;
    } else {
        L->rho_eager = false;
        L->last_replay_step = -10;
    }
    return LUDWIG_OK;
}

int ludwig_level_field_layout(const LudwigLevel *L, int field, int32_t *components, int64_t *block_stride, int64_t *component_stride)
{
    if (!L) return fail(LUDWIG_ERR_INVALID, "null level");
    const FieldDesc d = field_desc(L, field);
    if (field < 0 || field >= LUDWIG_FIELD_COUNT) return fail(LUDWIG_ERR_INVALID, "bad field %d", field);
    if (components) *components = d.comps;
    if (block_stride) *block_stride = (int64_t)d.comps * CELLS;
    if (component_stride) *component_stride = CELLS;
    return LUDWIG_OK;
}

int ludwig_init_equilibrium(LudwigLevel *L)
{
    if (!L) return fail(LUDWIG_ERR_INVALID, "null level");
    if (L->n_blocks == 0) return LUDWIG_OK;
    LW_HIP(hipSetDevice(L->device));
    const unsigned grid = (unsigned)((L->sk + 255) / 256);
    ++L->version;
    {
        const int r = ensure_rho(L);
        if (r) return r;
    }
    hipLaunchKernelGGL(k_fill_weights, dim3(grid), dim3(256), 0, L->stream, L->f[0], L->sk);
    hipLaunchKernelGGL(k_fill_weights, dim3(grid), dim3(256), 0, L->stream, L->f[1], L->sk);
    if (L->has_temporal) {
        L->old_alias = -1;
        hipLaunchKernelGGL(k_fill_weights, dim3(grid), dim3(256), 0, L->stream, L->f_old, L->sk);
        int r = fill(L, L->rho_old, L->sk, 1.0f);
        if (r) return r;
        LW_HIP(hipMemsetAsync(L->vel_old, 0, (size_t)L->sk * 3 * 4, L->stream));
    }
    LW_HIP(hipGetLastError());
    return LUDWIG_OK;
}

int ludwig_stream_collide(LudwigLevel *L, const LudwigLevel *parent, int64_t t_sub, float u_curr, float parent_tau,
                          float temporal_weight, const LudwigStepFlags *flags, int part)
{
    return launch_stream_collide(L, parent, t_sub, u_curr, parent_tau, temporal_weight, flags, part);
}

int ludwig_bouzidi_correction(LudwigLevel *L, int64_t t_sub, float q_min_threshold) { return launch_bouzidi(L, t_sub, q_min_threshold); }

int ludwig_step(LudwigLevel *L, const LudwigLevel *parent, int64_t t_sub, float u_curr, float parent_tau, float temporal_weight,
                const LudwigStepFlags *flags)
{
    int r = launch_stream_collide(L, parent, t_sub, u_curr, parent_tau, temporal_weight, flags, LUDWIG_PART_ALL);
    if (r) return r;
    return launch_bouzidi(L, t_sub, flags->q_min_threshold);
}

static int save_old_impl(LudwigLevel *L, int64_t t_sub, bool defer_rho);

int ludwig_save_old(LudwigLevel *L, int64_t t_sub) { return save_old_impl(L, t_sub, false); }

static int save_old_impl(LudwigLevel *L, int64_t t_sub, bool defer_rho)
{
    if (!L) return fail(LUDWIG_ERR_INVALID, "null level");
    if (!L->has_temporal) return LUDWIG_OK;
    LW_HIP(hipSetDevice(L->device));
    const int in = (t_sub % 2 == 0) ? 0 : 1;
    const size_t c = (size_t)L->sk;
    ++L->version;
    if (L->external_writer) {
        L->old_alias = -1;
        LW_HIP(hipMemcpyAsync(L->f_old, L->f[in], c * Q * 4, hipMemcpyDeviceToDevice, L->stream));
        LW_HIP(hipMemcpyAsync(L->vel_old, L->vel[in], c * 3 * 4, hipMemcpyDeviceToDevice, L->stream));
    } else {
        L->old_alias = in;
    }
    L->rho_eager = true;
    {
        const int r = ensure_rho(L);
        if (r) return r;
    }
    if (defer_rho && L->n_owned == L->n_blocks && !L->external_writer && !env::rho_old_copy()) {
        L->rho_old_pending = true;
        return LUDWIG_OK;
    }
    L->rho_old_pending = false;
    LW_HIP(hipMemcpyAsync(L->rho_old, L->rho, c * 4, hipMemcpyDeviceToDevice, L->stream));
    return LUDWIG_OK;
}

namespace {

const float *vel_out(const LudwigLevel *L, int64_t t_sub) { return L->vel[(t_sub % 2 == 0) ? 1 : 0]; }

int32_t internal_cell(const LudwigLevel *L, int32_t b, int32_t x) { return (L->ref2int.empty() ? b : L->ref2int[b]) * CELLS + x; }

#define LW_ENSURE_RHO(L)                                                                                  \
    do {                                                                                                  \
        const int r_ = ensure_rho(const_cast<LudwigLevel *>(L));                                          \
        if (r_) return r_;                                                                                \
    } while (0)

int set_device(int device)
{
    LW_HIP(hipSetDevice(device));
    return LUDWIG_OK;
}

int check_stencil_point(const char *noun, const char *set, int32_t p, LudwigLevel *const *levels, int32_t n_levels, const int32_t *level_index,
                        const int32_t *blocks, const int32_t *cells, const float *weights, const LudwigLevel *&first)
{
    const int li = level_index[p];
    if (li < 0 || li >= n_levels) return fail(LUDWIG_ERR_INVALID, "%s %d: level index %d not in 0..%d", noun, p, li, n_levels - 1);
    const LudwigLevel *L = levels[li];
    if (!L) return fail(LUDWIG_ERR_INVALID, "%s %d: level %d is null", noun, p, li);
    if (first && L->device != first->device) return fail(LUDWIG_ERR_INVALID, "%s: levels on different devices", set);
    if (!first) first = L;
    if ((int64_t)L->n_blocks * CELLS > (int64_t)INT32_MAX)
        return fail(LUDWIG_ERR_INVALID, "%s %d: level %d has %d blocks, more than 32-bit cell indices reach", noun, p, li, L->n_blocks);
    for (int c = 0; c < 8; ++c) {
        const int32_t b = blocks[8 * p + c], x = cells[8 * p + c];
        if (b < 0 || b >= L->n_blocks) return fail(LUDWIG_ERR_INVALID, "%s %d corner %d: block %d not in 0..%d", noun, p, c, b, L->n_blocks - 1);
        if (x < 0 || x >= CELLS) return fail(LUDWIG_ERR_INVALID, "%s %d corner %d: cell %d not in 0..511", noun, p, c, x);
    }
    for (int a = 0; a < 3; ++a) {
        const float w = weights[3 * p + a];
        if (!(w >= 0.0f && w <= 1.0f)) return fail(LUDWIG_ERR_INVALID, "%s %d: weight %d = %g not in [0, 1]", noun, p, a, (double)w);
    }
    return LUDWIG_OK;
}

int check_one_device(const char *set, LudwigLevel *const *levels, int32_t n_levels, const LudwigLevel *first)
{
    for (int li = 0; li < n_levels; ++li)
        if (levels[li] && levels[li]->device != first->device) return fail(LUDWIG_ERR_INVALID, "%s: levels on different devices", set);
    return LUDWIG_OK;
}

bool step_sampled(int64_t t, int64_t start_step, int32_t interval)
{
    return t >= start_step && (t - start_step) % interval == 0;
}

int64_t samples_in(int64_t first, int64_t last, int64_t start_step, int32_t interval)
{
    const int64_t lo = std::max(first, start_step);
    if (last < lo) return 0;
    const int64_t k0 = (lo - start_step + interval - 1) / interval, s0 = start_step + k0 * interval;
    return s0 > last ? 0 : (last - s0) / interval + 1;
}

// ... 139 lines not shown
    for (size_t s = 0; s < q.stage_groups.size(); ++s) {
        const int g = q.stage_groups[s];
        if (s == 0)
            hipLaunchKernelGGL(k_flux_chunks, dim3((unsigned)g), dim3(CELLS / 2), 0, L->stream, q.slab, dst, tab, q.cell, q.w, L->rho,
                               vel_out(L, t_sub));
        else
            hipLaunchKernelGGL(k_flux_combine, dim3((unsigned)g), dim3(CELLS / 2), 0, L->stream, q.slab, dst, tab);
        LW_HIP(hipGetLastError());
        tab += g;
    }
    return LUDWIG_OK;
}

struct LudwigModes {
    int device = 0;
    int n_levels = 0, n_columns = 0, n_rows = 0;
    std::vector<LudwigLevel *> levels;
    double *table = nullptr;
    std::vector<double *> sums;
    std::vector<size_t> sums_count;
    std::vector<int64_t> count;
};

static int64_t modes_row_of(int64_t t, int64_t start_step, int32_t interval, int n_rows)
{
    return ((t - start_step) / interval) % n_rows;
}

static int modes_launch(LudwigModes *S, int li, int64_t t_sub, int64_t row)
{
    if (S->sums[li]) {
        LudwigLevel *L = S->levels[li];
        LW_ENSURE_RHO(L);
        hipLaunchKernelGGL(k_accumulate_modes, dim3((unsigned)L->n_owned), dim3(CELLS / 2), 0, L->stream, S->sums[li],
                           (const double *)(S->table + (size_t)row * S->n_columns), S->n_columns, (const float *)L->rho, vel_out(L, t_sub));
        LW_HIP(hipGetLastError());
    }
    ++S->count[li];
    return LUDWIG_OK;
}

struct ObserverSchedule {
    int64_t start_step = 0;
    int32_t interval = 1;
    bool due(int64_t t) const { return step_sampled(t, start_step, interval); }
};
struct BatchObservers {
    struct : ObserverSchedule { LudwigProbes *set = nullptr; } probes;
    struct : ObserverSchedule { LudwigSurfaceStats *set = nullptr; } surface;
    struct : ObserverSchedule { LudwigForceSeries *set = nullptr; } forces;
    struct : ObserverSchedule { LudwigTracers *set = nullptr; } tracers;
    struct : ObserverSchedule { LudwigFluxPlanes *set = nullptr; } fluxes;
    struct : ObserverSchedule { LudwigModes *set = nullptr; } modes;
};
struct BatchHook {
    const BatchObservers *obs = nullptr;
    int64_t t = 0;
    int slot = -1;
    bool surface = false, forces = false;
    int flux_slot = -1;
    int64_t modes_row = -1;
};

static int recursive_step(LudwigLevel *const *levels, int n_levels, int lvl , int64_t t_sub, const LudwigLevel *parent,
                          float parent_tau, float temporal_weight, float u_vel, const LudwigStepFlags *fl, bool concurrent,
                          const BatchHook *ph = nullptr)
{
    if (lvl > n_levels) return LUDWIG_OK;
    LudwigLevel *L = levels[lvl - 1];
    const bool has_children = lvl < n_levels;
    int rc;
    if (concurrent) {
        const bool need_parent = parent && (L->waited_parent != parent || L->waited_gen != parent->stepped_gen);
        const bool wait_children = has_children && L->ev_consumed_set;
        const bool hoist = wait_children && (env::iface_hoist() >= 0 ? env::iface_hoist() != 0
                                                                     : 20 * (int64_t)L->n_blocks >= 9 * (int64_t)levels[lvl]->n_blocks);
        if (need_parent) {
            if (hoist) LW_HIP(hipStreamWaitEvent(L->stream, parent->ev_stepped, 0));
            else L->parent_wait = parent->ev_stepped;
            L->waited_parent = parent; L->waited_gen = parent->stepped_gen;
        }
        if (wait_children) {
            if (hoist && (rc = interface_prepass(L, parent, t_sub, parent_tau, temporal_weight, fl))) return rc;
            LW_HIP(hipStreamWaitEvent(L->stream, L->ev_consumed, 0));
        }
    }
    if (has_children && fl->use_temporal_interp && L->has_temporal)
        if ((rc = save_old_impl(L, t_sub, true))) return rc;
    if ((rc = ludwig_step(L, parent, t_sub, u_vel, parent_tau, temporal_weight, fl))) return rc;
    const bool parent_side = !env::child_side_iface();
    if (concurrent && parent && parent_side && (t_sub & 1) && L->ev_pair_done[0]) {
        const int set = (int)((t_sub >> 1) & 1);
        LW_HIP(hipEventRecord(L->ev_pair_done[set], L->stream));
        L->pair_done_set[set] = true;
    }
    if (concurrent && has_children) {
        if (parent_side && (rc = interface_pass_for_child(L, levels[lvl], t_sub, fl))) return rc;
        LW_HIP(hipEventRecord(L->ev_stepped, L->stream));
        ++L->stepped_gen;
    }
    if (ph && (ph->slot >= 0 || ph->surface || ph->forces || ph->flux_slot >= 0 || ph->modes_row >= 0)) {
        const int64_t m = (int64_t)1 << (lvl - 1);
        if (t_sub == m * ph->t + m - 1) {
            const BatchObservers &o = *ph->obs;
            if (ph->slot >= 0 && (rc = probes_launch(o.probes.set, lvl - 1, ph->slot, t_sub))) return rc;
            if (ph->surface && o.surface.set->level == L && (rc = surface_stats_launch(o.surface.set, t_sub))) return rc;
// ... 263 lines not shown
    LudwigLevel *L = S->level;
    if (S->n_tri > 0) {
        LW_HIP(hipSetDevice(S->device));
        LW_ENSURE_RHO(L);
        hipLaunchKernelGGL(k_wall_surface, dim3((unsigned)((S->n_tri + 255) / 256)), dim3(256), 0, L->stream, S->out, (const int32_t *)S->cell,
                           (const float *)S->nrm, S->n_tri, (const float *)L->rho, vel_out(L, t_sub), (const uint8_t *)L->obstacle,
                           (const float *)L->wall_dist, L->tau, S->pressure_scale, S->stress_scale);
        LW_HIP(hipGetLastError());
    }
    S->computed = true;
    return LUDWIG_OK;
}

int ludwig_wall_surface_download(LudwigWallSurface *S, float *values, size_t bytes)
{
    if (!S || (!values && bytes > 0)) return fail(LUDWIG_ERR_INVALID, "null argument");
    const size_t want = (size_t)S->n_tri * WALL_SURFACE_ROWS * sizeof(float);
    if (bytes != want) return fail(LUDWIG_ERR_INVALID, "wall surface: got %zu bytes, expected %zu", bytes, want);
    if (!S->computed) return fail(LUDWIG_ERR_STATE, "wall surface: download before ludwig_wall_surface_compute");
    if (want == 0) return LUDWIG_OK;
    LW_HIP(hipSetDevice(S->device));
    LW_HIP(hipStreamSynchronize(S->level->stream));
    LW_HIP(hipMemcpy(values, S->out, want, hipMemcpyDeviceToHost));
    return LUDWIG_OK;
}

int ludwig_level_stats_download(const LudwigLevel *L, int stat, double *host, size_t bytes, int64_t *n_samples)
{
    if (!L || (!host && bytes > 0)) return fail(LUDWIG_ERR_INVALID, "null argument");
    if (stat < LUDWIG_STAT_RHO || stat > LUDWIG_STAT_VEL2) return fail(LUDWIG_ERR_INVALID, "bad statistic %d", stat);
    if (!L->stats_ready) return fail(LUDWIG_ERR_STATE, "statistics: download before ludwig_level_stats_reset");
    const int K = stat == LUDWIG_STAT_RHO ? 1 : stat == LUDWIG_STAT_VEL ? 3 : 6, first = stat == LUDWIG_STAT_RHO ? 0 : stat == LUDWIG_STAT_VEL ? 1 : 4;
    const size_t plane = (size_t)L->sk * sizeof(double);
    if (bytes != plane * K) return fail(LUDWIG_ERR_INVALID, "statistic %d: got %zu bytes, expected %zu", stat, bytes, plane * K);
    if (n_samples) *n_samples = L->stats_n;
    if (plane == 0) return LUDWIG_OK;
    if (!L->stats) {
        memset(host, 0, bytes);
        return LUDWIG_OK;
    }
    return download_components(L, (const double *)L->stats, STAT_COMPONENTS, first, K, host, "statistics download");
}

int ludwig_level_gradient_fields_compute(LudwigLevel *L, int vel_field, float scale)
{
    if (!L) return fail(LUDWIG_ERR_INVALID, "null level");
    if (vel_field != LUDWIG_VEL && vel_field != LUDWIG_VEL_TEMP) return fail(LUDWIG_ERR_INVALID, "vel_field must be LUDWIG_VEL or LUDWIG_VEL_TEMP");
    if (!std::isfinite(scale) || scale == 0.0f) return fail(LUDWIG_ERR_INVALID, "gradient fields: scale %g must be finite and non-zero", (double)scale);
    if (L->n_owned == 0) {
        L->grad_ready = true;
        return LUDWIG_OK;
    }
    LW_HIP(hipSetDevice(L->device));
    if (!L->grad) {
        const size_t n = (size_t)L->n_blocks * GRAD_COMPONENTS * CELLS;
        const int r = dev_alloc(L, &L->grad, n);
        if (r) return r;
        LW_HIP(hipMemsetAsync(L->grad, 0, n * sizeof(float), L->stream));
    }
    hipLaunchKernelGGL(k_velocity_gradient_fields, dim3((unsigned)L->n_owned), dim3(CELLS / 2), 0, L->stream, L->grad,
                       (const float *)L->vel[vel_field == LUDWIG_VEL ? 0 : 1], (const uint8_t *)L->obstacle, (const int32_t *)L->meta, scale);
    LW_HIP(hipGetLastError());
    L->grad_ready = true;
    return LUDWIG_OK;
}

int ludwig_level_gradient_fields_download(const LudwigLevel *L, int which, float *host, size_t bytes)
{
    if (!L || (!host && bytes > 0)) return fail(LUDWIG_ERR_INVALID, "null argument");
    if (which != LUDWIG_GRAD_VORTICITY && which != LUDWIG_GRAD_Q) return fail(LUDWIG_ERR_INVALID, "bad gradient field %d", which);
    if (!L->grad_ready) return fail(LUDWIG_ERR_STATE, "gradient fields: download before ludwig_level_gradient_fields_compute");
    const int K = which == LUDWIG_GRAD_VORTICITY ? 3 : 1, first = which == LUDWIG_GRAD_VORTICITY ? 0 : 3;
    const size_t plane = (size_t)L->sk * sizeof(float);
    if (bytes != plane * K) return fail(LUDWIG_ERR_INVALID, "gradient field %d: got %zu bytes, expected %zu", which, bytes, plane * K);
    if (plane == 0) return LUDWIG_OK;
    if (!L->grad) {
        memset(host, 0, bytes);
        return LUDWIG_OK;
    }
    return download_components(L, (const float *)L->grad, GRAD_COMPONENTS, first, K, host, "gradient fields download");
}

#define LW_ISO_TRY(expr) do { const int r_ = (expr); if (r_) return r_; } while (0)
int ludwig_level_isosurface_extract(LudwigLevel *L, int which, int vel_field, float scale, float value, const uint8_t *skip,
                                    const int32_t *cell_lo, const int32_t *cell_hi, int64_t max_triangles, int64_t *n_triangles)
{
    if (!L || !cell_lo || !cell_hi || !n_triangles) return fail(LUDWIG_ERR_INVALID, "isosurface: null argument");
    *n_triangles = 0;
    if (which < LUDWIG_ISO_DENSITY || which > LUDWIG_ISO_VORTICITY_MAGNITUDE) return fail(LUDWIG_ERR_INVALID, "isosurface: unknown scalar %d", which);
    if (vel_field != LUDWIG_VEL && vel_field != LUDWIG_VEL_TEMP) return fail(LUDWIG_ERR_INVALID, "isosurface: vel_field must be LUDWIG_VEL or LUDWIG_VEL_TEMP");
    if (!std::isfinite(value)) return fail(LUDWIG_ERR_INVALID, "isosurface: value %g must be finite", (double)value);
    if (!std::isfinite(scale)) return fail(LUDWIG_ERR_INVALID, "isosurface: scale %g must be finite", (double)scale);
    const bool gradient = which == LUDWIG_ISO_Q_CRITERION || which == LUDWIG_ISO_VORTICITY_MAGNITUDE;
    if (gradient && scale == 0.0f) return fail(LUDWIG_ERR_INVALID, "isosurface: scale must be non-zero for a scalar of the velocity gradient");
    for (int a = 0; a < 3; ++a)
        if (cell_lo[a] > cell_hi[a]) return fail(LUDWIG_ERR_INVALID, "isosurface: cell_lo[%d] = %d > cell_hi[%d] = %d", a, cell_lo[a], a, cell_hi[a]);
    if (max_triangles < 0) return fail(LUDWIG_ERR_INVALID, "isosurface: max_triangles %lld < 0", (long long)max_triangles);
    if ((int64_t)L->n_blocks * CELLS > (int64_t)INT32_MAX)
        return fail(LUDWIG_ERR_INVALID, "isosurface: level has %d blocks, more than 32-bit vertex keys reach", L->n_blocks);
    if (L->n_owned == 0) {
        L->iso_n = 0;
        return LUDWIG_OK;
    }
    LW_HIP(hipSetDevice(L->device));
    LW_ENSURE_RHO(L);
    if (gradient) {
// ... 61 lines not shown
    o.counts = L->iso_counts;
    o.offsets = L->iso_offsets;
    o.n_triangles = total;
    o.int2ref = L->d_int2ref;
    o.rho = L->rho;
    o.vel = vel;
    o.pos = L->iso_pos;
    o.att = L->iso_att;
    o.keys = L->iso_keys;
    hipLaunchKernelGGL(k_iso_emit, dim3((unsigned)no), dim3(CELLS / 2), 0, L->stream, a, o);
    LW_HIP(hipGetLastError());
    LW_HIP(hipStreamSynchronize(L->stream));
    L->iso_n = total;
    return LUDWIG_OK;
}

int ludwig_level_isosurface_download(LudwigLevel *L, float *positions, size_t position_bytes, float *attributes, size_t attribute_bytes,
                                     int32_t *keys, size_t key_bytes)
{
    if (!L) return fail(LUDWIG_ERR_INVALID, "null level");
    if (L->iso_n < 0) return fail(LUDWIG_ERR_STATE, "isosurface: download before ludwig_level_isosurface_extract");
    const size_t n = (size_t)L->iso_n;
    const size_t want[3] = {n * ISO_POS_FLOATS * sizeof(float), n * ISO_ATT_FLOATS * sizeof(float), n * ISO_KEY_INTS * sizeof(int32_t)};
    if (position_bytes != want[0] || attribute_bytes != want[1] || key_bytes != want[2])
        return fail(LUDWIG_ERR_INVALID, "isosurface: got %zu, %zu, %zu bytes, expected %zu, %zu, %zu", position_bytes, attribute_bytes, key_bytes,
                    want[0], want[1], want[2]);
    if (n == 0) return LUDWIG_OK;
    if (!positions || !attributes || !keys) return fail(LUDWIG_ERR_INVALID, "isosurface: null output");
    LW_HIP(hipSetDevice(L->device));
    LW_HIP(hipStreamSynchronize(L->stream));
    LW_HIP(hipMemcpy(positions, L->iso_pos, want[0], hipMemcpyDeviceToHost));
    LW_HIP(hipMemcpy(attributes, L->iso_att, want[1], hipMemcpyDeviceToHost));
    LW_HIP(hipMemcpy(keys, L->iso_keys, want[2], hipMemcpyDeviceToHost));
    return LUDWIG_OK;
}
#undef LW_ISO_TRY

static int subgrid_model_known(const LudwigLevel *L, const char *what)
{
    if (L->wale_known) return LUDWIG_OK;
    return fail(LUDWIG_ERR_STATE, "subgrid %s: the level has not been stepped yet, so it holds no c_wale / nu_sgs_background", what);
}

int ludwig_level_subgrid_fields_compute(LudwigLevel *L, int vel_field)
{
    if (!L) return fail(LUDWIG_ERR_INVALID, "null level");
    if (vel_field != LUDWIG_VEL && vel_field != LUDWIG_VEL_TEMP) return fail(LUDWIG_ERR_INVALID, "vel_field must be LUDWIG_VEL or LUDWIG_VEL_TEMP");
    if (L->n_owned == 0) {
        L->subgrid_fields_ready = true;
        return LUDWIG_OK;
    }
    if (const int r = subgrid_model_known(L, "fields")) return r;
    LW_HIP(hipSetDevice(L->device));
    if (!L->subgrid_fields) {
        const size_t n = (size_t)L->n_blocks * SUBGRID_FIELD_COMPONENTS * CELLS;
        const int r = dev_alloc(L, &L->subgrid_fields, n);
        if (r) return r;
        LW_HIP(hipMemsetAsync(L->subgrid_fields, 0, n * sizeof(float), L->stream));
    }
    hipLaunchKernelGGL(k_subgrid<SUBGRID_FIELDS>, dim3((unsigned)L->n_owned), dim3(CELLS / 2), 0, L->stream, L->subgrid_fields,
                       (const float *)L->vel[vel_field == LUDWIG_VEL ? 0 : 1], (const uint8_t *)L->obstacle, (const int32_t *)L->meta,
                       L->c_wale, L->nu_bg);
    LW_HIP(hipGetLastError());
    L->subgrid_fields_ready = true;
    return LUDWIG_OK;
}

int ludwig_level_subgrid_fields_download(const LudwigLevel *L, int which, float *host, size_t bytes)
{
    if (!L || (!host && bytes > 0)) return fail(LUDWIG_ERR_INVALID, "null argument");
    if (which != LUDWIG_SUBGRID_NU && which != LUDWIG_SUBGRID_CODE) return fail(LUDWIG_ERR_INVALID, "bad subgrid field %d", which);
    if (!L->subgrid_fields_ready) return fail(LUDWIG_ERR_STATE, "subgrid fields: download before ludwig_level_subgrid_fields_compute");
    const size_t plane = (size_t)L->sk * sizeof(float);
    if (bytes != plane) return fail(LUDWIG_ERR_INVALID, "subgrid field %d: got %zu bytes, expected %zu", which, bytes, plane);
    if (plane == 0) return LUDWIG_OK;
    if (!L->subgrid_fields) {
        memset(host, 0, bytes);
        return LUDWIG_OK;
    }
    return download_components(L, (const float *)L->subgrid_fields, SUBGRID_FIELD_COMPONENTS, which, 1, host, "subgrid fields download");
}

int ludwig_level_subgrid_stats_reset(LudwigLevel *L)
{
    if (!L) return fail(LUDWIG_ERR_INVALID, "null level");
    L->subgrid_stats_ready = true;
    L->subgrid_n = 0;
    if (L->n_owned == 0) return LUDWIG_OK;
    LW_HIP(hipSetDevice(L->device));
    const size_t n = (size_t)L->n_blocks * SUBGRID_SUM_COMPONENTS * CELLS;
    if (!L->subgrid_sums) {
        const int r = dev_alloc(L, &L->subgrid_sums, n);
        if (r) { L->subgrid_stats_ready = false; return r; }
    }
    LW_HIP(hipMemsetAsync(L->subgrid_sums, 0, n * sizeof(double), L->stream));
    return LUDWIG_OK;
}

int ludwig_level_subgrid_stats_accumulate(LudwigLevel *L, int64_t t_sub)
{
    if (!L) return fail(LUDWIG_ERR_INVALID, "null level");
    if (!L->subgrid_stats_ready) return fail(LUDWIG_ERR_STATE, "subgrid statistics: accumulate before ludwig_level_subgrid_stats_reset");
    if (t_sub < 0) return fail(LUDWIG_ERR_INVALID, "subgrid statistics: t_sub %lld < 0", (long long)t_sub);
    if (L->n_owned == 0) return LUDWIG_OK;
    if (const int r = subgrid_model_known(L, "statistics")) return r;
    LW_HIP(hipSetDevice(L->device));
    hipLaunchKernelGGL(k_subgrid<SUBGRID_SUMS>, dim3((unsigned)L->n_owned), dim3(CELLS / 2), 0, L->stream, L->subgrid_sums,
                       (const float *)vel_out(L, t_sub), (const uint8_t *)L->obstacle, (const int32_t *)L->meta, L->c_wale, L->nu_bg);
    LW_HIP(hipGetLastError());
    ++L->subgrid_n;
    return LUDWIG_OK;
}

int ludwig_level_subgrid_stats_download(const LudwigLevel *L, int which, double *host, size_t bytes, int64_t *n_samples)
{
    if (!L || (!host && bytes > 0)) return fail(LUDWIG_ERR_INVALID, "null argument");
    if (which < LUDWIG_SUBGRID_SUM_NU || which > LUDWIG_SUBGRID_SUM_EPS) return fail(LUDWIG_ERR_INVALID, "bad subgrid statistic %d", which);
    if (!L->subgrid_stats_ready) return fail(LUDWIG_ERR_STATE, "subgrid statistics: download before ludwig_level_subgrid_stats_reset");
    const size_t plane = (size_t)L->sk * sizeof(double);
    if (bytes != plane) return fail(LUDWIG_ERR_INVALID, "subgrid statistic %d: got %zu bytes, expected %zu", which, bytes, plane);
    if (n_samples) *n_samples = L->subgrid_n;
    if (plane == 0) return LUDWIG_OK;
    if (!L->subgrid_sums) {
        memset(host, 0, bytes);
        return LUDWIG_OK;
    }
    return download_components(L, (const double *)L->subgrid_sums, SUBGRID_SUM_COMPONENTS, which, 1, host, "subgrid statistics download");
}

void ludwig_probes_destroy(LudwigProbes *P)
{
    if (!P) return;
    (void)hipSetDevice(P->device);
    for (LudwigProbes::PerLevel &q : P->per) {
        if (q.cell) (void)hipFree(q.cell);
        if (q.w) (void)hipFree(q.w);
        if (q.col) (void)hipFree(q.col);
    }
    if (P->ring) (void)hipFree(P->ring);
    delete P;
}

int ludwig_probes_create(LudwigLevel *const *levels, int32_t n_levels, int32_t n_probes, const int32_t *level_index,
                         const int32_t *blocks, const int32_t *cells, const float *weights, int32_t capacity, LudwigProbes **out)
{
    if (!out) return fail(LUDWIG_ERR_INVALID, "null argument");
    *out = nullptr;
    if (!levels || !level_index || !blocks || !cells || !weights) return fail(LUDWIG_ERR_INVALID, "null argument");
    if (n_levels < 1 || n_levels > 64) return fail(LUDWIG_ERR_INVALID, "probes: n_levels %d not in 1..64", n_levels);
    if (n_probes < 1) return fail(LUDWIG_ERR_INVALID, "probes: n_probes %d < 1", n_probes);
    if (capacity < 1) return fail(LUDWIG_ERR_INVALID, "probes: capacity %d < 1", capacity);
    if ((int64_t)capacity * n_probes * 16 > ((int64_t)1 << 34)) return fail(LUDWIG_ERR_INVALID, "probes: ring of %d x %d samples too large", capacity, n_probes);
    const LudwigLevel *first = nullptr;
    for (int32_t p = 0; p < n_probes; ++p) {
        const int r = check_stencil_point("probe", "probes", p, levels, n_levels, level_index, blocks, cells, weights, first);
        if (r) return r;
    }
    if (const int r = check_one_device("probes", levels, n_levels, first)) return r;
    LudwigProbes *P = new (std::nothrow) LudwigProbes;
// ... 926 lines not shown
    S->generations = generations;
    S->release_every = release_every;
    S->n_slots = (int64_t)n_seeds * generations;
    S->dt = dt;
    S->levels.assign(levels, levels + n_levels);
    S->bp.assign(n_levels, nullptr);
    int r = set_device(S->device);
    hipError_t e = hipSuccess;
    if (r == LUDWIG_OK) {
        upload_locator_table(e, levels, n_levels, false, S->bp, S->table);
        if (S->n_slots > 0) {
            const size_t n = (size_t)S->n_slots;
            const std::vector<float> hs(seeds, seeds + 3 * (size_t)n_seeds);
            const std::vector<int32_t> empty(n, TRACER_EMPTY);
            const std::vector<float> zero(3 * n, 0.0f);
            upload_table(e, hs, S->seeds);
            upload_table(e, zero, S->pos);
            upload_table(e, empty, S->state);
            if (e == hipSuccess) e = hipMalloc((void **)&S->rec, n * STREAM_REC_FLOATS * sizeof(float));
        }
        if (e == hipSuccess) e = hipEventCreateWithFlags(&S->ev, hipEventDisableTiming);
        if (e != hipSuccess) r = fail(LUDWIG_ERR_ALLOC, "tracers: %d seeds of %d generations: %s", n_seeds, generations, hipGetErrorString(e));
    }
    if (r != LUDWIG_OK) {
        ludwig_tracers_destroy(S);
        return r;
    }
    *out = S;
    return LUDWIG_OK;
}

static TracerArgs tracers_args(const LudwigTracers *S, int64_t t_coarse)
{
    TracerArgs a{};
    a.s.lv = S->table;
    a.s.n_levels = S->n_levels;
    for (int li = 0; li < S->n_levels; ++li)
        if (vel_out(S->levels[li], (t_coarse + 1) * ((int64_t)1 << li) - 1) == S->levels[li]->vel[1]) a.s.temp_mask |= 1u << li;
    a.seeds = S->seeds;
    a.pos = S->pos;
    a.state = S->state;
    a.rec = S->rec;
    a.n_seeds = S->n_seeds;
    a.n_slots = (int32_t)S->n_slots;
    a.released = -1;
    a.dt = S->dt;
    return a;
}

static int tracers_launch_advance(LudwigTracers *S, int64_t t_coarse, hipStream_t st)
{
    const int64_t k = S->n_advances++;
    if (S->n_slots == 0) return LUDWIG_OK;
    TracerArgs a = tracers_args(S, t_coarse);
    if (k % S->release_every == 0) a.released = (int32_t)((k / S->release_every) % S->generations);
    hipLaunchKernelGGL(k_tracers_advance, dim3((unsigned)((S->n_slots * 8 + 63) / 64)), dim3(64), 0, st, a);
    LW_HIP(hipGetLastError());
    return LUDWIG_OK;
}

static int tracers_join(LudwigTracers *S, hipStream_t st)
{
    for (int li = 0; li < S->n_levels; ++li)
        if (S->levels[li]->stream != st) {
            LW_HIP(hipEventRecord(S->ev, S->levels[li]->stream));
            LW_HIP(hipStreamWaitEvent(st, S->ev, 0));
        }
    return LUDWIG_OK;
}

static int tracers_release(LudwigTracers *S, hipStream_t st)
{
    bool others = false;
    for (int li = 1; li < S->n_levels; ++li) others = others || S->levels[li]->stream != st;
    if (!others) return LUDWIG_OK;
    LW_HIP(hipEventRecord(S->ev, st));
    for (int li = 1; li < S->n_levels; ++li)
        if (S->levels[li]->stream != st) LW_HIP(hipStreamWaitEvent(S->levels[li]->stream, S->ev, 0));
    return LUDWIG_OK;
}

int ludwig_tracers_advance(LudwigTracers *S, int64_t t_coarse)
{
    if (!S) return fail(LUDWIG_ERR_INVALID, "null tracer set");
    if (t_coarse < 0) return fail(LUDWIG_ERR_INVALID, "tracers: t_coarse %lld < 0", (long long)t_coarse);
    if (S->n_slots == 0) { ++S->n_advances; return LUDWIG_OK; }
    LW_HIP(hipSetDevice(S->device));
    hipStream_t st = S->levels[0]->stream;
    int r = tracers_join(S, st);
    if (r) return r;
    if ((r = tracers_launch_advance(S, t_coarse, st))) return r;
    return tracers_release(S, st);
}

int ludwig_tracers_snapshot(LudwigTracers *S, int64_t t_coarse)
{
    if (!S) return fail(LUDWIG_ERR_INVALID, "null tracer set");
    if (t_coarse < 0) return fail(LUDWIG_ERR_INVALID, "tracers: t_coarse %lld < 0", (long long)t_coarse);
    S->snapshot = true;
    if (S->n_slots == 0) return LUDWIG_OK;
    LW_HIP(hipSetDevice(S->device));
    hipStream_t st = S->levels[0]->stream;
    const int r = tracers_join(S, st);
    if (r) return r;
    const TracerArgs a = tracers_args(S, t_coarse);
    hipLaunchKernelGGL(k_tracers_snapshot, dim3((unsigned)((S->n_slots * 8 + 63) / 64)), dim3(64), 0, st, a);
    LW_HIP(hipGetLastError());
    return tracers_release(S, st);
}

int ludwig_tracers_download(LudwigTracers *S, float *records, size_t bytes, int64_t *n_advances)
{
    if (!S) return fail(LUDWIG_ERR_INVALID, "null tracer set");
    if (!S->snapshot) return fail(LUDWIG_ERR_STATE, "tracers: download before ludwig_tracers_snapshot");
    const size_t want = (size_t)S->n_slots * STREAM_REC_FLOATS * sizeof(float);
    if (bytes != want) return fail(LUDWIG_ERR_INVALID, "tracers: got %zu bytes, expected %zu", bytes, want);
    if (n_advances) *n_advances = S->n_advances;
    if (S->n_slots == 0) return LUDWIG_OK;
    if (!records) return fail(LUDWIG_ERR_INVALID, "null argument");
    LW_HIP(hipSetDevice(S->device));
    LW_HIP(hipStreamSynchronize(S->levels[0]->stream));
    LW_HIP(hipMemcpy(records, S->rec, want, hipMemcpyDeviceToHost));
    return LUDWIG_OK;
}

static int check_batch_levels(LudwigLevel *const *levels, int32_t n_levels, int32_t batch_size, const LudwigStepFlags *flags)
{
    if (!levels || !flags || n_levels < 1 || batch_size < 0) return fail(LUDWIG_ERR_INVALID, "bad argument");
    for (int i = 0; i < n_levels; ++i) {
        if (!levels[i]) return fail(LUDWIG_ERR_INVALID, "null level %d", i + 1);
        if (levels[i]->device != levels[0]->device || levels[i]->stream != levels[0]->stream)
            return fail(LUDWIG_ERR_INVALID, "all levels must share one device and one stream");
    }
    return LUDWIG_OK;
}

static int check_made_over(const char *what, const std::vector<LudwigLevel *> &made_over, LudwigLevel *const *levels, int32_t n_levels)
{
    if ((int)made_over.size() != n_levels)
        return fail(LUDWIG_ERR_INVALID, "%s: set made over %d levels, batch of %d", what, (int)made_over.size(), n_levels);
    for (int i = 0; i < n_levels; ++i)
        if (made_over[i] != levels[i]) return fail(LUDWIG_ERR_INVALID, "%s: set made over other levels (level %d)", what, i + 1);
    return LUDWIG_OK;
}

static int check_level_in_batch(const char *what, const LudwigLevel *level, LudwigLevel *const *levels, int32_t n_levels)
{
    bool in_batch = false;
    for (int i = 0; i < n_levels; ++i) in_batch = in_batch || levels[i] == level;
    return in_batch ? LUDWIG_OK : fail(LUDWIG_ERR_INVALID, "%s: the set's level is not in the batch", what);
}

static int check_ring_room(const char *what, const char *items, size_t used, int capacity, const ObserverSchedule &o, int64_t t_start,
                           int32_t batch_size)
{
    const int64_t k = batch_size > 0 ? samples_in(t_start, t_start + batch_size - 1, o.start_step, o.interval) : 0;
    if ((int64_t)used + k <= capacity) return LUDWIG_OK;
// ... 89 lines not shown

static int batch_impl(LudwigLevel *const *levels, int32_t n_levels, int64_t t_start, int32_t batch_size, float u_curr,
                      const LudwigStepFlags *flags, const BatchObservers &obs)
{
    const bool concurrent = n_levels > 1 && !env::batch_serial();
    hipStream_t user_stream = levels[0]->stream;
    if (concurrent) {
        LW_HIP(hipSetDevice(levels[0]->device));
        LW_HIP(hipStreamSynchronize(user_stream));
        int pr_least = 0, pr_greatest = 0;
        LW_HIP(hipDeviceGetStreamPriorityRange(&pr_least, &pr_greatest));
        const int pr_mode = env::level_stream_priority();
        hipError_t e = hipSuccess;
        for (int i = 0; i < n_levels && e == hipSuccess; ++i) {
            LudwigLevel *L = levels[i];
            if (L->own_stream && L->ev_stepped && L->ev_consumed) continue;
            int pr = pr_mode == 0 ? pr_least : (i == n_levels - 1 ? pr_greatest : pr_least);
            if (pr_mode == 2) pr = std::min(pr_least, pr_greatest + (n_levels - 1 - i));
            if (!L->own_stream) e = hipStreamCreateWithPriority(&L->own_stream, hipStreamNonBlocking, pr);
            if (e == hipSuccess && !L->ev_stepped) e = hipEventCreateWithFlags(&L->ev_stepped, hipEventDisableTiming);
            if (e == hipSuccess && !L->ev_consumed) e = hipEventCreateWithFlags(&L->ev_consumed, hipEventDisableTiming);
        }
        if (e != hipSuccess) {
            for (int i = 0; i < n_levels; ++i) {
                LudwigLevel *L = levels[i];
                if (L->own_stream && L->ev_stepped && L->ev_consumed) continue;
                hipEvent_t *evs[] = {&L->ev_stepped, &L->ev_consumed};
                for (hipEvent_t *ev : evs)
                    if (*ev) { (void)hipEventDestroy(*ev); *ev = nullptr; }
                if (L->own_stream) { (void)hipStreamDestroy(L->own_stream); L->own_stream = nullptr; }
            }
            return fail(LUDWIG_ERR_HIP, "batch: level streams: %s", hipGetErrorString(e));
        }
        auto restore = [&]() { for (int j = 0; j < n_levels; ++j) levels[j]->stream = user_stream; };
        for (int i = 0; i < n_levels; ++i) {
            LudwigLevel *L = levels[i];
            L->ev_consumed_set = false;
            L->waited_parent = nullptr;
            L->parent_wait = nullptr;
            L->pair_ready.valid = false;
            L->pair_done_set[0] = L->pair_done_set[1] = false;
            L->stream = L->own_stream;
        }
        for (int i = 0; i + 1 < n_levels; ++i) {
            LudwigLevel *L = levels[i];
            if (!L->rho_eager) {
                L->rho_eager = true;
                const int r = ensure_rho(L);
                if (r) { restore(); return r; }
            }
        }
    }
    for (int i = 0; i < n_levels; ++i) levels[i]->rho_old_pending = false;
    int rc = LUDWIG_OK;
    for (int32_t o = 0; o < batch_size && rc == LUDWIG_OK; ++o) {
        const int64_t t = t_start + o;
        BatchHook ph;
        ph.obs = &obs;
        ph.t = t;
        if (obs.probes.set && obs.probes.due(t)) ph.slot = probes_open_slot(obs.probes.set, t);
        ph.surface = obs.surface.set && obs.surface.due(t);
        ph.forces = obs.forces.set && obs.forces.due(t);
        if (obs.fluxes.set && obs.fluxes.due(t)) ph.flux_slot = flux_planes_open_slot(obs.fluxes.set, t);
        if (obs.modes.set && obs.modes.due(t)) ph.modes_row = modes_row_of(t, obs.modes.start_step, obs.modes.interval, obs.modes.set->n_rows);
        rc = recursive_step(levels, n_levels, 1, t, nullptr, 0.5f, 0.0f, u_curr, flags, concurrent, &ph);
        if (rc == LUDWIG_OK && obs.tracers.set && obs.tracers.due(t)) rc = batch_tracers_advance(levels, n_levels, obs.tracers.set, t, concurrent);
    }
    if (concurrent) {
        hipError_t e = hipSuccess;
        for (int i = 0; i < n_levels; ++i) {
            const hipError_t ei = hipStreamSynchronize(levels[i]->own_stream);
            if (e == hipSuccess) e = ei;
            levels[i]->stream = user_stream;
        }
        if (rc == LUDWIG_OK && e != hipSuccess) return fail(LUDWIG_ERR_HIP, "batch: %s", hipGetErrorString(e));
    }
    if (rc) return rc;
    return ludwig_sync(levels[0]);
}

int ludwig_execute_timestep_batch_observed(LudwigLevel *const *levels, int32_t n_levels, int64_t t_start, int32_t batch_size, float u_curr,
                                           const LudwigStepFlags *flags, const LudwigBatchObserver *observers, int32_t n_observers)
{
    BatchObservers obs;
    int r = check_batch_levels(levels, n_levels, batch_size, flags);
    if (r) return r;
    if ((r = check_batch_observers(levels, n_levels, t_start, batch_size, observers, n_observers, &obs))) return r;
    return batch_impl(levels, n_levels, t_start, batch_size, u_curr, flags, obs);
}

int ludwig_execute_timestep_batch(LudwigLevel *const *levels, int32_t n_levels, int64_t t_start, int32_t batch_size, float u_curr,
                                  const LudwigStepFlags *flags)
{
    return ludwig_execute_timestep_batch_observed(levels, n_levels, t_start, batch_size, u_curr, flags, nullptr, 0);
}

int ludwig_execute_timestep_batch_probes(LudwigLevel *const *levels, int32_t n_levels, int64_t t_start, int32_t batch_size, float u_curr,
                                         const LudwigStepFlags *flags, LudwigProbes *probes, int64_t start_step, int32_t interval)
{
    const LudwigBatchObserver o = {LUDWIG_OBSERVE_PROBES, probes, start_step, interval};
    return ludwig_execute_timestep_batch_observed(levels, n_levels, t_start, batch_size, u_curr, flags, &o, 1);
}

static void sampler_entries(const LudwigBatchSamplers *s, LudwigBatchObserver *o)
{
    const LudwigBatchSamplers none = {};
    if (!s) s = &none;
    o[0] = {LUDWIG_OBSERVE_PROBES, s->probes, s->probes_start_step, s->probes_interval};
    o[1] = {LUDWIG_OBSERVE_SURFACE, s->surface, s->surface_start_step, s->surface_interval};
}

int ludwig_execute_timestep_batch_sampled(LudwigLevel *const *levels, int32_t n_levels, int64_t t_start, int32_t batch_size, float u_curr,
                                          const LudwigStepFlags *flags, const LudwigBatchSamplers *s)
{
    LudwigBatchObserver o[2];
    sampler_entries(s, o);
    return ludwig_execute_timestep_batch_observed(levels, n_levels, t_start, batch_size, u_curr, flags, o, 2);
}

int ludwig_execute_timestep_batch_loads(LudwigLevel *const *levels, int32_t n_levels, int64_t t_start, int32_t batch_size, float u_curr,
                                        const LudwigStepFlags *flags, const LudwigBatchSamplers *s, LudwigForceSeries *fs, int64_t start_step,
                                        int32_t interval)
{
    LudwigBatchObserver o[3];
    sampler_entries(s, o);
    o[2] = {LUDWIG_OBSERVE_FORCES, fs, start_step, interval};
    return ludwig_execute_timestep_batch_observed(levels, n_levels, t_start, batch_size, u_curr, flags, o, 3);
}

int ludwig_execute_timestep_batch_tracers(LudwigLevel *const *levels, int32_t n_levels, int64_t t_start, int32_t batch_size, float u_curr,
                                          const LudwigStepFlags *flags, const LudwigBatchSamplers *s, LudwigForceSeries *fs,
                                          int64_t force_start_step, int32_t force_interval, LudwigTracers *tracers, int64_t start_step,
                                          int32_t interval)
{
    LudwigBatchObserver o[4];
    sampler_entries(s, o);
    o[2] = {LUDWIG_OBSERVE_FORCES, fs, force_start_step, force_interval};
    o[3] = {LUDWIG_OBSERVE_TRACERS, tracers, start_step, interval};
    return ludwig_execute_timestep_batch_observed(levels, n_levels, t_start, batch_size, u_curr, flags, o, 4);
}

int ludwig_halo_pack(const LudwigLevel *L, int field, const int64_t *index_dev, int64_t n, float *dst_dev, void *hip_stream)
{
    if (!L || (n > 0 && (!index_dev || !dst_dev))) return fail(LUDWIG_ERR_INVALID, "null argument");
    if (n == 0) return LUDWIG_OK;
    const FieldDesc d = field_desc(L, field);
    if (!d.ptr || field == LUDWIG_OBSTACLE) return fail(LUDWIG_ERR_STATE, "field %d cannot be packed", field);
    LW_HIP(hipSetDevice(L->device));
    if (field == LUDWIG_RHO) {
        bool stale = false;
        for (int a = 0; a < N_PARTS; ++a) stale = stale || L->rho_replay[a].stale;
        const int r = ensure_rho(const_cast<LudwigLevel *>(L));
        if (r) return r;
        if (stale && hip_stream && (hipStream_t)hip_stream != L->stream) LW_HIP(hipStreamSynchronize(L->stream));
    }
    hipLaunchKernelGGL(k_gather, dim3((unsigned)((n + 255) / 256)), dim3(256), 0, hip_stream ? (hipStream_t)hip_stream : L->stream, (const float *)d.ptr, index_dev, n, dst_dev, (const int32_t *)L->d_ref2int, L->sk, d.comps);
    LW_HIP(hipGetLastError());
    return LUDWIG_OK;
}

int ludwig_halo_unpack(LudwigLevel *L, int field, const int64_t *index_dev, int64_t n, const float *src_dev, void *hip_stream)
{
    if (!L || (n > 0 && (!index_dev || !src_dev))) return fail(LUDWIG_ERR_INVALID, "null argument");
    if (n == 0) return LUDWIG_OK;
    ++L->version;
    {
        const bool aliased = L->old_alias >= 0;
        const int r = before_external_write(L, field);
        if (r) return r;
        if (aliased && L->old_alias < 0 && hip_stream && (hipStream_t)hip_stream != L->stream) LW_HIP(hipStreamSynchronize(L->stream));
    }
    const FieldDesc d = field_desc(L, field);
    if (!d.ptr || field == LUDWIG_OBSTACLE) return fail(LUDWIG_ERR_STATE, "field %d cannot be unpacked", field);
    LW_HIP(hipSetDevice(L->device));
    hipLaunchKernelGGL(k_scatter, dim3((unsigned)((n + 255) / 256)), dim3(256), 0, hip_stream ? (hipStream_t)hip_stream : L->stream, (float *)d.ptr, index_dev, n, src_dev, (const int32_t *)L->d_ref2int, L->sk, d.comps);
    LW_HIP(hipGetLastError());
    return LUDWIG_OK;
}

int ludwig_level_info(const LudwigLevel *L, LudwigLevelInfo *info)
{
    if (!L || !info) return fail(LUDWIG_ERR_INVALID, "null argument");
    info->n_blocks = L->n_blocks;
    info->n_owned = L->n_owned;
    info->n_fast_blocks = L->n_fast_blocks;
    info->n_general_blocks = L->n_owned - L->n_fast_blocks;
    info->n_boundary_cells = L->n_bc;
    info->has_temporal_storage = L->has_temporal;
    info->has_post_collision = L->has_post;
    info->n_xrun_blocks = (int32_t)(L->n_linked_items[LUDWIG_PART_ALL] / 8);
    info->device_bytes = L->device_bytes;
    return LUDWIG_OK;
}

}

#include <dlfcn.h>
#include <link.h>
#include <rccl/rccl.h>

namespace {

struct RcclApi {
    void *handle = nullptr;
    std::string path;
    decltype(&ncclGetUniqueId) GetUniqueId = nullptr;
    decltype(&ncclCommInitRank) CommInitRank = nullptr;
    decltype(&ncclCommDestroy) CommDestroy = nullptr;
    decltype(&ncclGroupStart) GroupStart = nullptr;
    decltype(&ncclGroupEnd) GroupEnd = nullptr;
    decltype(&ncclSend) Send = nullptr;
    decltype(&ncclRecv) Recv = nullptr;
    decltype(&ncclAllReduce) AllReduce = nullptr;
    decltype(&ncclGetErrorString) GetErrorString = nullptr;
};

int find_loaded_rccl(struct dl_phdr_info *info, size_t, void *data)
{
    if (info->dlpi_name && strstr(info->dlpi_name, "librccl")) {
        *static_cast<std::string *>(data) = info->dlpi_name;
        return 1;
    }
    return 0;
}

RcclApi *rccl()
{
    static RcclApi api;
    static bool tried = false;
// ... 184 lines not shown
    if (c->scratch) (void)hipFree(c->scratch);
    if (c->stream) (void)hipStreamDestroy(c->stream);
    delete c;
}

int ludwig_comm_allreduce_f32(LudwigComm *c, float *buf, int32_t n, int32_t op)
{
    if (!c || !buf || n < 0 || n > 256) return fail(LUDWIG_ERR_INVALID, "bad argument (at most 256 values)");
    if (op != 0 && op != 2 && op != 3) return fail(LUDWIG_ERR_INVALID, "op must be 0 (sum), 2 (max) or 3 (min)");
    if (n == 0) return LUDWIG_OK;
    RcclApi *api = rccl();
    if (!api) return fail(LUDWIG_ERR_STATE, "RCCL unavailable");
    LW_HIP(hipSetDevice(c->device));
    float host[512];
    for (int i = 0; i < n; ++i) {
        const bool nan = buf[i] != buf[i];
        host[i] = (nan && op != 0) ? (op == 3 ? __builtin_inff() : -__builtin_inff()) : buf[i];
        host[256 + i] = nan ? 1.0f : 0.0f;
    }
    LW_HIP(hipMemcpyAsync(c->scratch, host, 512 * sizeof(float), hipMemcpyHostToDevice, c->stream));
    LW_NCCL(api, api->AllReduce(c->scratch, c->scratch, (size_t)n, ncclFloat, (ncclRedOp_t)op, c->comm, c->stream));
    if (op != 0) LW_NCCL(api, api->AllReduce(c->scratch + 256, c->scratch + 256, (size_t)n, ncclFloat, ncclMax, c->comm, c->stream));
    LW_HIP(hipMemcpyAsync(host, c->scratch, 512 * sizeof(float), hipMemcpyDeviceToHost, c->stream));
    LW_HIP(hipStreamSynchronize(c->stream));
    for (int i = 0; i < n; ++i) buf[i] = (op != 0 && host[256 + i] > 0.0f) ? __builtin_nanf("") : host[i];
    return LUDWIG_OK;
}

void ludwig_halo_plan_destroy(LudwigHaloPlan *P)
{
    if (!P) return;
    if (P->L) (void)hipSetDevice(P->L->device);
    if (P->s_comm) (void)hipStreamSynchronize(P->s_comm);
    for (auto &G : P->g) {
        void *ptrs[] = {G.send_buf, G.recv_buf, G.send_desc, G.recv_desc, G.send_single, G.recv_single};
        for (void *q : ptrs)
            if (q) (void)hipFree(q);
    }
    for (int i = 0; i < TIMING_RING; ++i) {
        if (P->t0[i]) (void)hipEventDestroy(P->t0[i]);
        if (P->t1[i]) (void)hipEventDestroy(P->t1[i]);
    }
    if (P->ev_ready) (void)hipEventDestroy(P->ev_ready);
    if (P->ev_done) (void)hipEventDestroy(P->ev_done);
    if (P->s_comm) (void)hipStreamDestroy(P->s_comm);
    delete P;
}

int ludwig_halo_plan_create(LudwigLevel *L, LudwigComm *comm, const LudwigHaloPlanDesc *desc, LudwigHaloPlan **out)
{
    if (out) *out = nullptr;
    if (!L || !desc || !out || desc->n_peers < 0 || (desc->n_peers > 0 && !desc->peer_ranks)) return fail(LUDWIG_ERR_INVALID, "bad argument");
    if (comm && comm->device != L->device) return fail(LUDWIG_ERR_INVALID, "communicator and level live on different devices");
    for (int p = 0; p < desc->n_peers; ++p) {
        const int r = desc->peer_ranks[p];
        if (comm ? (r < 0 || r >= comm->world) : r != 0) return fail(LUDWIG_ERR_INVALID, "peer %d: rank %d not in the communicator", p, r);
    }
    LW_HIP(hipSetDevice(L->device));
    LudwigHaloPlan *P = new (std::nothrow) LudwigHaloPlan();
    if (!P) return fail(LUDWIG_ERR_ALLOC, "host allocation failed");
    P->L = L; P->comm = comm;
    P->peers.assign(desc->peer_ranks, desc->peer_ranks + desc->n_peers);
    P->self_via_rccl = comm && env::halo_self_via_rccl();
    int rc = LUDWIG_OK;
    auto upload = [&](const auto &v, auto **dst) -> int {
        *dst = nullptr;
        if (v.empty()) return LUDWIG_OK;
        LW_HIP(hipMalloc((void **)dst, v.size() * sizeof(v[0])));
        LW_HIP(hipMemcpy(*dst, v.data(), v.size() * sizeof(v[0]), hipMemcpyHostToDevice));
        return LUDWIG_OK;
    };
    for (int g = 0; g < LUDWIG_HALO_GROUPS && rc == LUDWIG_OK; ++g) {
        LudwigHaloPlan::Group &G = P->g[g];
        G.send_off.assign((size_t)desc->n_peers + 1, 0);
        G.recv_off.assign((size_t)desc->n_peers + 1, 0);
        for (int p = 0; p < desc->n_peers; ++p) {
            const int64_t ns = desc->send_count[g] ? desc->send_count[g][p] : 0, nr = desc->recv_count[g] ? desc->recv_count[g][p] : 0;
            if (ns < 0 || nr < 0) rc = fail(LUDWIG_ERR_INVALID, "negative count");
            G.send_off[(size_t)p + 1] = G.send_off[(size_t)p] + ns;
            G.recv_off[(size_t)p + 1] = G.recv_off[(size_t)p] + nr;
        }
        if (rc) break;
        G.n_send = G.send_off.back(); G.n_recv = G.recv_off.back();
        if ((G.n_send > 0 && !desc->send_index[g]) || (G.n_recv > 0 && !desc->recv_index[g])) { rc = fail(LUDWIG_ERR_INVALID, "group %d: index list missing", g); break; }
        if (g == 2 && (G.n_send || G.n_recv) && !L->has_post) { rc = fail(LUDWIG_ERR_STATE, "group 2 (f_post_collision) on a level without that array"); break; }
        std::vector<uint4> sd, rd;
        std::vector<uint2> ss, rs;
        if ((rc = build_octets(L, HALO_GROUP_COMPS[g], desc->send_index[g], G.n_send, sd, ss))) break;
        if ((rc = build_octets(L, HALO_GROUP_COMPS[g], desc->recv_index[g], G.n_recv, rd, rs))) break;
        G.n_send_oct = (int64_t)sd.size(); G.n_recv_oct = (int64_t)rd.size();
        G.n_send_single = (int64_t)ss.size(); G.n_recv_single = (int64_t)rs.size();
        if ((rc = upload(sd, &G.send_desc)) || (rc = upload(rd, &G.recv_desc)) || (rc = upload(ss, &G.send_single)) || (rc = upload(rs, &G.recv_single))) break;
        hipError_t e = hipSuccess;
        if (G.n_send) e = hipMalloc((void **)&G.send_buf, (size_t)G.n_send * 4);
        if (e == hipSuccess && G.n_recv) e = hipMalloc((void **)&G.recv_buf, (size_t)G.n_recv * 4);
        if (e != hipSuccess) rc = fail(LUDWIG_ERR_ALLOC, "halo buffers: %s", hipGetErrorString(e));
    }
    if (rc == LUDWIG_OK) {
        int pr_least = 0, pr_greatest = 0;
        hipError_t e = hipDeviceGetStreamPriorityRange(&pr_least, &pr_greatest);
        if (e == hipSuccess) e = hipStreamCreateWithPriority(&P->s_comm, hipStreamNonBlocking, pr_greatest);
        if (e == hipSuccess) e = hipEventCreateWithFlags(&P->ev_ready, hipEventDisableTiming);
        if (e == hipSuccess) e = hipEventCreateWithFlags(&P->ev_done, hipEventDisableTiming);
        if (e != hipSuccess) rc = fail(LUDWIG_ERR_HIP, "halo plan streams: %s", hipGetErrorString(e));
    }
    if (rc) { ludwig_halo_plan_destroy(P); return rc; }
    *out = P;
    return LUDWIG_OK;
}

int ludwig_halo_plan_timing(LudwigHaloPlan *P, int enable)
{
    if (!P) return fail(LUDWIG_ERR_INVALID, "null plan");
    LW_HIP(hipSetDevice(P->L->device));
    if (enable && !P->t0[0])
        for (int i = 0; i < TIMING_RING; ++i) { LW_HIP(hipEventCreate(&P->t0[i])); LW_HIP(hipEventCreate(&P->t1[i])); }
    P->timing = enable != 0;
    P->n_read = P->n_timed;
    return LUDWIG_OK;
}

int ludwig_halo_plan_in_stream(LudwigHaloPlan *P, int enable)
{
    if (!P) return fail(LUDWIG_ERR_INVALID, "null plan");
    if (P->pending) {
        const int r = ludwig_halo_wait(P);
        if (r) return r;
    }
    P->in_stream = enable != 0;
    return LUDWIG_OK;
}

int ludwig_halo_plan_exchange_ms(LudwigHaloPlan *P, float *ms_out, int32_t max, int32_t *n_out)
{
    if (!P || !n_out || (max > 0 && !ms_out)) return fail(LUDWIG_ERR_INVALID, "null argument");
    *n_out = 0;
    if (P->n_timed - P->n_read > TIMING_RING) P->n_read = P->n_timed - TIMING_RING;
    while (P->n_read < P->n_timed && *n_out < max) {
        const int i = (int)(P->n_read % TIMING_RING);
        float ms = 0.0f;
        LW_HIP(hipEventElapsedTime(&ms, P->t0[i], P->t1[i]));
        ms_out[(*n_out)++] = ms;
        ++P->n_read;
    }
    return LUDWIG_OK;
}

int ludwig_halo_plan_pack(LudwigHaloPlan *P, int32_t group, int32_t field, void *hip_stream)
{
    if (!P || group < 0 || group >= LUDWIG_HALO_GROUPS) return fail(LUDWIG_ERR_INVALID, "bad argument");
    LW_HIP(hipSetDevice(P->L->device));
    if (field == LUDWIG_RHO) { const int r = ensure_rho(P->L); if (r) return r; }
    return halo_pack_group(P, group, field, hip_stream ? (hipStream_t)hip_stream : P->L->stream);
}

int ludwig_halo_plan_unpack(LudwigHaloPlan *P, int32_t group, int32_t field, void *hip_stream)
{
    if (!P || group < 0 || group >= LUDWIG_HALO_GROUPS) return fail(LUDWIG_ERR_INVALID, "bad argument");
    LW_HIP(hipSetDevice(P->L->device));
    ++P->L->version;
    { const int r = before_external_write(P->L, field); if (r) return r; }
    return halo_unpack_group(P, group, field, hip_stream ? (hipStream_t)hip_stream : P->L->stream);
}

int ludwig_halo_plan_buffers(const LudwigHaloPlan *P, int32_t group, void **send_dev, int64_t *n_send, void **recv_dev, int64_t *n_recv)
{
    if (!P || group < 0 || group >= LUDWIG_HALO_GROUPS) return fail(LUDWIG_ERR_INVALID, "bad argument");
    const LudwigHaloPlan::Group &G = P->g[group];
    if (send_dev) *send_dev = G.send_buf;
    if (n_send) *n_send = G.n_send;
    if (recv_dev) *recv_dev = G.recv_buf;
    if (n_recv) *n_recv = G.n_recv;
    return LUDWIG_OK;
}

static double host_now_us()
{
    struct timespec ts;
    clock_gettime(CLOCK_MONOTONIC, &ts);
    return ts.tv_sec * 1e6 + ts.tv_nsec * 1e-3;
}

int ludwig_halo_exchange(LudwigHaloPlan *P, int32_t n, const int32_t *groups, const int32_t *fields)
{
    if (!P || n < 0 || n > LUDWIG_HALO_GROUPS || (n > 0 && (!groups || !fields))) return fail(LUDWIG_ERR_INVALID, "bad argument");
    const bool trace = env::halo_trace();
    const double h0 = trace ? host_now_us() : 0.0;
    double h1 = 0.0, h2 = 0.0;
    LudwigLevel *L = P->L;
    LW_HIP(hipSetDevice(L->device));
    for (int i = 0; i < n; ++i) {
        if (groups[i] < 0 || groups[i] >= LUDWIG_HALO_GROUPS) return fail(LUDWIG_ERR_INVALID, "bad group %d", groups[i]);
        const int r = halo_prepare_field(L, groups[i], fields[i]);
        if (r) return r;
    }
    {
        int64_t moved = 0;
        for (int i = 0; i < n; ++i) moved += P->g[groups[i]].n_send + P->g[groups[i]].n_recv;
        if (moved == 0) return LUDWIG_OK;
    }
    ++L->version;
    const hipStream_t xs = P->in_stream ? L->stream : P->s_comm;
    if (!P->in_stream) {
        LW_HIP(hipEventRecord(P->ev_ready, L->stream));
// ... 80 lines not shown
```

Measured before the change: 24570.

## Store per-cell moment records instead of 27 populations for eligible uniform levels

Adds a record-based timestep path for single-level, fully interior, non-wall configurations. Each step stores 11 moments per cell (rho, velocity, stress components, relaxation factor) instead of 27 post-collision populations and rebuilds streamed populations from neighbour records, cutting HBM traffic per lattice update. Populations are rebuilt lazily whenever other APIs need f, rho or velocity, which adds bookkeeping and a conversion kernel. The kernel recomputes the regularized equilibrium for each pulled direction, so arithmetic per update rises in exchange for fewer bytes moved.

Result: faster. 25680 (median of 6 runs) (+4.5%).

```diff
diff --git a/include/ludwig_hip.h b/include/ludwig_hip.h
--- a/include/ludwig_hip.h
+++ b/include/ludwig_hip.h
@@ -143,6 +143,10 @@
 
 int  ludwig_level_set_rho_store(LudwigLevel *level, int every_step);
 
+int  ludwig_record_step_rule(const int32_t *block_flags, int32_t n_blocks, int32_t n_owned, int32_t has_parent,
+                             int32_t has_temporal_storage, int32_t has_post_collision, int32_t wall_model_active);
+int  ludwig_level_record_steps(const LudwigLevel *level, int64_t *n_steps);
+
 enum LudwigStat { LUDWIG_STAT_RHO = 0, LUDWIG_STAT_VEL = 1, LUDWIG_STAT_VEL2 = 2 };
 int  ludwig_level_stats_reset(LudwigLevel *level);
 int  ludwig_level_stats_accumulate(LudwigLevel *level, int64_t t_sub);
diff --git a/open_ludwig_amd/_lib.py b/open_ludwig_amd/_lib.py
--- a/open_ludwig_amd/_lib.py
+++ b/open_ludwig_amd/_lib.py
@@ -58,6 +58,7 @@
     "ludwig_execute_timestep_batch_loads",
     "ludwig_flux_planes_create", "ludwig_flux_planes_destroy", "ludwig_flux_planes_sample", "ludwig_flux_planes_download",
     "ludwig_modes_create", "ludwig_modes_destroy", "ludwig_modes_reset", "ludwig_modes_accumulate", "ludwig_modes_download",
+    "ludwig_record_step_rule", "ludwig_level_record_steps",
 ]
 UNIQUE_ID_BYTES = 128
 HALO_GROUPS = ("f", "vel", "f_post", "rho")
@@ -181,6 +182,8 @@
         "ludwig_stream_destroy": (C.c_int, [i32, vp]),
         "ludwig_level_field_layout": (C.c_int, [vp, i32, C.POINTER(C.c_int32), C.POINTER(C.c_int64), C.POINTER(C.c_int64)]),
         "ludwig_level_set_rho_store": (C.c_int, [vp, i32]),
+        "ludwig_record_step_rule": (C.c_int, [vp, i32, i32, i32, i32, i32, i32]),
+        "ludwig_level_record_steps": (C.c_int, [vp, C.POINTER(C.c_int64)]),
         "ludwig_comm_unique_id": (C.c_int, [vp]),
         "ludwig_comm_create": (C.c_int, [vp, i32, i32, i32, C.POINTER(vp)]),
         "ludwig_comm_destroy": (None, [vp]),
diff --git a/open_ludwig_amd/blocks.py b/open_ludwig_amd/blocks.py
--- a/open_ludwig_amd/blocks.py
+++ b/open_ludwig_amd/blocks.py
@@ -280,6 +280,11 @@
     def set_rho_store(self, every_step: bool) -> None:
         _lib.check(self._lib.ludwig_level_set_rho_store(self.handle, 1 if every_step else 0))
 
+    def record_steps(self) -> int:
+        n = C.c_int64()
+        _lib.check(self._lib.ludwig_level_record_steps(self.handle, C.byref(n)))
+        return int(n.value)
+
     def rho_min(self) -> float:
         v = C.c_float()
         _lib.check(self._lib.ludwig_level_rho_min(self.handle, C.byref(v)))
diff --git a/open_ludwig_amd/csrc/kernels.hpp b/open_ludwig_amd/csrc/kernels.hpp
--- a/open_ludwig_amd/csrc/kernels.hpp
+++ b/open_ludwig_amd/csrc/kernels.hpp
@@ -30,6 +30,8 @@
     int32_t n_iface_blocks;
     int32_t store_rho;
     float *rho_old_save;
+    float *rec_out;
+    const float *rec_in;
 };
 
 template <int K, int N, class F>
@@ -246,7 +248,88 @@
     return w;
 }
 
-template <bool POST, bool WALL>
+template <int K>
+__device__ __forceinline__ float collide_value(float rho, float ux_eq, float uy_eq, float uz_eq, float Pi_xx, float Pi_yy, float Pi_zz,
+                                               float Pi_xy, float Pi_yz, float Pi_zx, float one_m_omega)
+{
+    constexpr int cx = CX(K), cy = CY(K), cz = CZ(K);
+    constexpr float w_k = WEIGHT(K);
+    constexpr float cx_f = (float)cx, cy_f = (float)cy, cz_f = (float)cz;
+    const float usq_eq = ux_eq * ux_eq + uy_eq * uy_eq + uz_eq * uz_eq;
+    const float cu = cdot<K>(ux_eq, uy_eq, uz_eq);
+    const float feq = rho * w_k * (1.0f + 3.0f * cu + 4.5f * cu * cu - 1.5f * usq_eq);
+    constexpr float Q_xx = cx_f * cx_f - CS2_PHYSICS, Q_yy = cy_f * cy_f - CS2_PHYSICS, Q_zz = cz_f * cz_f - CS2_PHYSICS;
+    float od = 0.0f;
+    bool od_empty = true;
+    acc_signed<cx * cy>(od, od_empty, Pi_xy);
+    acc_signed<cy * cz>(od, od_empty, Pi_yz);
+    acc_signed<cz * cx>(od, od_empty, Pi_zx);
+    float inner = Pi_xx * Q_xx + Pi_yy * Q_yy + Pi_zz * Q_zz;
+    if constexpr (cx * cy != 0 || cy * cz != 0 || cz * cx != 0) inner = inner + 2.0f * od;
+    const float f_neq_reg = (w_k * 4.5f) * inner;
+    return feq + one_m_omega * f_neq_reg;
+}
+
+constexpr int R_COMP = 11;
+constexpr uint32_t R_PLANE_BYTES = R_COMP * 64 * 4, R_BLOCK_BYTES = 8 * R_PLANE_BYTES;
+enum { R_RHO, R_UX, R_UY, R_UZ, R_PXX, R_PYY, R_PZZ, R_PXY, R_PYZ, R_PZX, R_OMO };
+
+__device__ __forceinline__ const char *record_plane(const float *base, int blk, int z)
+{
+    return reinterpret_cast<const char *>(base) + (uint64_t)(uint32_t)blk * R_BLOCK_BYTES + (uint32_t)z * R_PLANE_BYTES;
+}
+__device__ __forceinline__ void load_record(float (&r)[R_COMP], const char *plane, uint32_t lane4)
+{
+    const float *q = reinterpret_cast<const float *>(plane + lane4);
+#pragma unroll
+    for (int c = 0; c < R_COMP; ++c) r[c] = q[c * 64];
+}
+template <bool WIDE>
+using record_off_t = std::conditional_t<WIDE, uint64_t, uint32_t>;
+template <bool WIDE>
+__device__ __forceinline__ record_off_t<WIDE> record_offset(int blk, int z)
+{
+    return (record_off_t<WIDE>)(uint32_t)blk * R_BLOCK_BYTES + (uint32_t)z * R_PLANE_BYTES;
+}
+template <class OFF>
+__device__ __forceinline__ void load_record_at(float (&r)[R_COMP], const float *base, OFF off)
+{
+    const float *q = reinterpret_cast<const float *>(reinterpret_cast<const char *>(base) + off);
+#pragma unroll
+    for (int c = 0; c < R_COMP; ++c) r[c] = q[c * 64];
+}
+__device__ __forceinline__ void store_record(float *base, const Own own, float rho, float ux, float uy, float uz, float Pi_xx, float Pi_yy,
+                                             float Pi_zz, float Pi_xy, float Pi_yz, float Pi_zx, float one_m_omega)
+{
+    char *plane = const_cast<char *>(record_plane(base, own.b, __builtin_amdgcn_readfirstlane((int)(own.cell4 >> 8))));
+    float *q = reinterpret_cast<float *>(plane + (own.cell4 & 255u));
+    const float v[R_COMP] = {rho, ux, uy, uz, Pi_xx, Pi_yy, Pi_zz, Pi_xy, Pi_yz, Pi_zx, one_m_omega};
+#pragma unroll
+    for (int c = 0; c < R_COMP; ++c) {
+#ifdef LW_NT_STORES
+        __builtin_nontemporal_store(v[c], q + c * 64);
+#else
+        q[c * 64] = v[c];
+#endif
+    }
+}
+template <int CY_, int CZ_>
+__device__ __forceinline__ void record_row(float (&fs)[Q], const float (&r)[R_COMP])
+{
+    static_for<0, 3>([&](auto ic) {
+        constexpr int k = decltype(ic)::value + 3 * (CY_ + 1) + 9 * (CZ_ + 1);
+        fs[k] = collide_value<k>(r[R_RHO], r[R_UX], r[R_UY], r[R_UZ], r[R_PXX], r[R_PYY], r[R_PZZ], r[R_PXY], r[R_PYZ], r[R_PZX], r[R_OMO]);
+    });
+}
+template <int CY_, int CZ_>
+__device__ __forceinline__ float record_face(const float (&r)[R_COMP], bool plus)
+{
+    constexpr int k = 2 + 3 * (CY_ + 1) + 9 * (CZ_ + 1);
+    return collide_value<k>(r[R_RHO], plus ? r[R_UX] : -r[R_UX], r[R_UY], r[R_UZ], r[R_PXX], r[R_PYY], r[R_PZZ],
+                            plus ? r[R_PXY] : -r[R_PXY], r[R_PYZ], plus ? r[R_PZX] : -r[R_PZX], r[R_OMO]);
+}
+
+template <bool POST, bool WALL, bool REC_OUT = false>
 __device__ __forceinline__ void finish_cell(const SCParams &p, const int flags, const Own own, float (&fs)[Q],
                                             const float ux_E, const float uy_E, const float uz_E, const float ux_W, const float uy_W, const float uz_W,
                                             const float ux_N, const float uy_N, const float uz_N, const float ux_S, const float uy_S, const float uz_S,
@@ -332,11 +415,13 @@
     }
     const float usq_eq = ux_eq * ux_eq + uy_eq * uy_eq + uz_eq * uz_eq;
 
-    st_f32(p.vel_out, own.b, V_BLOCK_BYTES, own.cell4, ux);
-    st_f32(p.vel_out, own.b, V_BLOCK_BYTES, COMP_BYTES + own.cell4, uy);
-    st_f32(p.vel_out, own.b, V_BLOCK_BYTES, 2 * COMP_BYTES + own.cell4, uz);
-    if (p.rho_old_save) st_f32(p.rho_old_save, own.b, S_BLOCK_BYTES, own.cell4, ld_own(p.rho, own.b, S_BLOCK_BYTES, own.cell4));
-    if (p.store_rho) st_f32(p.rho, own.b, S_BLOCK_BYTES, own.cell4, rho);
+    if constexpr (!REC_OUT) {
+        st_f32(p.vel_out, own.b, V_BLOCK_BYTES, own.cell4, ux);
+        st_f32(p.vel_out, own.b, V_BLOCK_BYTES, COMP_BYTES + own.cell4, uy);
+        st_f32(p.vel_out, own.b, V_BLOCK_BYTES, 2 * COMP_BYTES + own.cell4, uz);
+        if (p.rho_old_save) st_f32(p.rho_old_save, own.b, S_BLOCK_BYTES, own.cell4, ld_own(p.rho, own.b, S_BLOCK_BYTES, own.cell4));
+        if (p.store_rho) st_f32(p.rho, own.b, S_BLOCK_BYTES, own.cell4, rho);
+    }
 
     const float g11 = 0.5f * (ux_E - ux_W), g12 = 0.5f * (ux_N - ux_S), g13 = 0.5f * (ux_T - ux_B);
     const float g21 = 0.5f * (uy_E - uy_W), g22 = 0.5f * (uy_N - uy_S), g23 = 0.5f * (uy_T - uy_B);
@@ -388,24 +473,17 @@
 
     const float one_m_omega = 1.0f - omega;
     const float one_m_half_omega = 1.0f - 0.5f * omega;
+    if constexpr (REC_OUT) {
+        store_record(p.rec_out, own, rho, ux_eq, uy_eq, uz_eq, Pi_xx, Pi_yy, Pi_zz, Pi_xy, Pi_yz, Pi_zx, one_m_omega);
+        return;
+    }
     static_for<0, Q>([&](auto kc) {
         constexpr int k = decltype(kc)::value;
-        constexpr int cx = CX(k), cy = CY(k), cz = CZ(k);
-        constexpr float w_k = WEIGHT(k);
-        constexpr float cx_f = (float)cx, cy_f = (float)cy, cz_f = (float)cz;
-        const float cu = cdot<k>(ux_eq, uy_eq, uz_eq);
-        const float feq = rho * w_k * (1.0f + 3.0f * cu + 4.5f * cu * cu - 1.5f * usq_eq);
-        constexpr float Q_xx = cx_f * cx_f - CS2_PHYSICS, Q_yy = cy_f * cy_f - CS2_PHYSICS, Q_zz = cz_f * cz_f - CS2_PHYSICS;
-        float od = 0.0f;
-        bool od_empty = true;
-        acc_signed<cx * cy>(od, od_empty, Pi_xy);
-        acc_signed<cy * cz>(od, od_empty, Pi_yz);
-        acc_signed<cz * cx>(od, od_empty, Pi_zx);
-        float inner = Pi_xx * Q_xx + Pi_yy * Q_yy + Pi_zz * Q_zz;
-        if constexpr (cx * cy != 0 || cy * cz != 0 || cz * cx != 0) inner = inner + 2.0f * od;
-        const float f_neq_reg = (w_k * 4.5f) * inner;
-        float f_coll = feq + one_m_omega * f_neq_reg;
+        float f_coll = collide_value<k>(rho, ux_eq, uy_eq, uz_eq, Pi_xx, Pi_yy, Pi_zz, Pi_xy, Pi_yz, Pi_zx, one_m_omega);
         if constexpr (WALL) {
+            constexpr float w_k = WEIGHT(k);
+            constexpr float cx_f = (float)CX(k), cy_f = (float)CY(k), cz_f = (float)CZ(k);
+            const float cu = cdot<k>(ux_eq, uy_eq, uz_eq);
             const float force_term = (w_k * 3.0f) * ((cx_f - ux + 3.0f * cu * cx_f) * Fx + (cy_f - uy + 3.0f * cu * cy_f) * Fy +
                                                      (cz_f - uz + 3.0f * cu * cz_f) * Fz);
             f_coll = f_coll + one_m_half_omega * force_term;
@@ -489,8 +567,8 @@
 #ifndef LW_MIN_WAVES
 #define LW_MIN_WAVES 5
 #endif
-template <int NW, bool GENERAL, bool POST, bool WALL, bool RHO_ONLY = false, bool WIDE = false>
-__global__ __launch_bounds__(64 * NW) __attribute__((amdgpu_waves_per_eu((WIDE && GENERAL) ? LW_MIN_WAVES - 1 : LW_MIN_WAVES))) void k_stream_collide_xrun(const SCParams p)
+template <int NW, bool GENERAL, bool POST, bool WALL, bool RHO_ONLY, bool WIDE, bool REC_OUT>
+__device__ __forceinline__ void stream_collide_xrun(const SCParams p)
 {
     __shared__ float xch[NW][24][8];
     const int wave = __builtin_amdgcn_readfirstlane(threadIdx.x >> 6);
@@ -611,8 +689,162 @@
         uS[c] = l.y0 ? uy_edge[c] : s_in;
     }
     if constexpr (GENERAL) { if (needs_patch) patch_missing_sources(p, meta, nbr, l, z, own, fs); }
-    finish_cell<POST, WALL>(p, flags, own, fs, uE[0], uE[1], uE[2], uW[0], uW[1], uW[2], uN[0], uN[1], uN[2], uS[0], uS[1], uS[2],
-                            uT[0], uT[1], uT[2], uB[0], uB[1], uB[2]);
+    finish_cell<POST, WALL, REC_OUT>(p, flags, own, fs, uE[0], uE[1], uE[2], uW[0], uW[1], uW[2], uN[0], uN[1], uN[2], uS[0], uS[1], uS[2],
+                                     uT[0], uT[1], uT[2], uB[0], uB[1], uB[2]);
+}
+template <int NW, bool GENERAL, bool POST, bool WALL, bool RHO_ONLY = false, bool WIDE = false>
+__global__ __launch_bounds__(64 * NW) __attribute__((amdgpu_waves_per_eu((WIDE && GENERAL) ? LW_MIN_WAVES - 1 : LW_MIN_WAVES))) void k_stream_collide_xrun(const SCParams p)
+{
+    stream_collide_xrun<NW, GENERAL, POST, WALL, RHO_ONLY, WIDE, false>(p);
+}
+template <int NW, bool WIDE>
+__global__ __launch_bounds__(64 * NW) __attribute__((amdgpu_waves_per_eu(LW_MIN_WAVES))) void k_records_from_populations(const SCParams p)
+{
+    stream_collide_xrun<NW, false, false, false, false, WIDE, true>(p);
+}
+
+#ifndef LW_REC_WAVES
+#define LW_REC_WAVES 4
+#endif
+#ifndef LW_REC_AHEAD
+#define LW_REC_AHEAD 3
+#endif
+template <int NW, bool WIDE>
+__global__ __launch_bounds__(64 * NW) __attribute__((amdgpu_waves_per_eu(LW_REC_WAVES))) void k_step_records(const SCParams p)
+{
+    __shared__ float xch[NW][24][8];
+    const int wave = __builtin_amdgcn_readfirstlane(threadIdx.x >> 6);
+    const int raw = p.items[blockIdx.x * NW + wave];
+    const bool active = raw >= 0;
+    const int item = active ? (raw & ITEM_ID_MASK) : 0;
+    const int b = item >> 3;
+    const int z = item & 7;
+    const int lane = threadIdx.x & 63;
+    LanePos l;
+    l.x = lane & 7; l.y = lane >> 3;
+    l.x0 = l.x == 0; l.x7 = l.x == 7; l.y0 = l.y == 0; l.y7 = l.y == 7;
+    const int32_t *__restrict__ meta = p.meta + (size_t)b * NBR_STRIDE;
+    const NeighbourIds nbr = load_neighbour_ids(meta, z);
+    const Own own{b, (uint32_t)((l.x + 8 * l.y + 64 * z) * 4)};
+    const bool first = !active || (raw & ITEM_LINK_W) == 0, last = !active || (raw & ITEM_LINK_E) == 0;
+    __shared__ float xedge[NW][2][12][8];
+    float fs[Q];
+    float uc[3], uT[3], uB[3], uN[3], uS[3];
+    if (active) {
+    if ((first && l.x0) || (last && l.x7)) {
+        float r[9][R_COMP];
+        auto load_face = [&](auto jc) {
+            constexpr int j = decltype(jc)::value;
+            constexpr int cy = j % 3 - 1, g = 1 - (j / 3 - 1);
+            const bool yo = cy == 1 ? l.y0 : (cy == -1 ? l.y7 : false);
+            const int wX = nbr.id[g][4 - 1], wXY = nbr.id[g][4 - 1 - 3 * cy], eX = nbr.id[g][4 + 1], eXY = nbr.id[g][4 + 1 - 3 * cy];
+            const auto oW = record_offset<WIDE>(wX, nbr.zs[g]), oWY = record_offset<WIDE>(wXY, nbr.zs[g]);
+            const auto oE = record_offset<WIDE>(eX, nbr.zs[g]), oEY = record_offset<WIDE>(eXY, nbr.zs[g]);
+            const auto off = l.x0 ? (yo ? oWY : oW) : (yo ? oEY : oE);
+            load_record_at(r[j], p.rec_in, off + (uint32_t)(((l.x0 ? 7 : 0) + 8 * ((l.y - cy) & 7)) * 4));
+        };
+        static_for<0, LW_REC_AHEAD>(load_face);
+        static_for<0, 9>([&](auto jc) {
+            constexpr int j = decltype(jc)::value;
+            constexpr int cy = j % 3 - 1, cz = j / 3 - 1;
+            if constexpr (j + LW_REC_AHEAD < 9) load_face(std::integral_constant<int, j + LW_REC_AHEAD>{});
+            __builtin_amdgcn_sched_barrier(0);
+            float(&mine)[12][8] = xedge[wave][l.x0 ? 0 : 1];
+            mine[j][l.y] = record_face<cy, cz>(r[j], l.x0);
+            if constexpr (cy == 0 && cz == 0) { mine[9][l.y] = r[j][R_UX]; mine[10][l.y] = r[j][R_UY]; mine[11][l.y] = r[j][R_UZ]; }
+            __builtin_amdgcn_sched_barrier(0);
+        });
+    }
+    {
+        float r[9][R_COMP];
+        auto load_pulled = [&](auto jc) {
+            constexpr int j = decltype(jc)::value;
+            constexpr int cy = j % 3 - 1, g = 1 - (j / 3 - 1);
+            const uint32_t lane4 = (uint32_t)((l.x + 8 * ((l.y - cy) & 7)) * 4);
+            if constexpr (cy == 0) {
+                load_record(r[j], record_plane(p.rec_in, nbr.id[g][4], nbr.zs[g]), lane4);
+            } else {
+                const bool yo = cy == 1 ? l.y0 : l.y7;
+                const auto o0 = record_offset<WIDE>(nbr.id[g][4], nbr.zs[g]), oY = record_offset<WIDE>(nbr.id[g][4 - 3 * cy], nbr.zs[g]);
+                load_record_at(r[j], p.rec_in, (yo ? oY : o0) + lane4);
+            }
+        };
+        static_for<0, LW_REC_AHEAD>(load_pulled);
+        static_for<0, 9>([&](auto jc) {
+            constexpr int j = decltype(jc)::value;
+            constexpr int cy = j % 3 - 1, cz = j / 3 - 1;
+            if constexpr (j + LW_REC_AHEAD < 9) load_pulled(std::integral_constant<int, j + LW_REC_AHEAD>{});
+            __builtin_amdgcn_sched_barrier(0);
+            const float(&q)[R_COMP] = r[j];
+            record_row<cy, cz>(fs, q);
+            if constexpr (cy == 0 && cz == 0) { uc[0] = q[R_UX]; uc[1] = q[R_UY]; uc[2] = q[R_UZ]; }
+            if constexpr (cy == 0 && cz == 1) { uB[0] = q[R_UX]; uB[1] = q[R_UY]; uB[2] = q[R_UZ]; }
+            if constexpr (cy == 0 && cz == -1) { uT[0] = q[R_UX]; uT[1] = q[R_UY]; uT[2] = q[R_UZ]; }
+            if constexpr (cy == 1 && cz == 0) { uS[0] = q[R_UX]; uS[1] = q[R_UY]; uS[2] = q[R_UZ]; }
+            if constexpr (cy == -1 && cz == 0) { uN[0] = q[R_UX]; uN[1] = q[R_UY]; uN[2] = q[R_UZ]; }
+            __builtin_amdgcn_sched_barrier(0);
+        });
+    }
+    static_for<0, Q>([&](auto kc) {
+        constexpr int k = decltype(kc)::value;
+        constexpr int cx = CX(k);
+        if constexpr (cx == 1) { if (l.x7) xch[wave][XSLOT(k)][l.y] = fs[k]; }
+        if constexpr (cx == -1) { if (l.x0) xch[wave][XSLOT(k)][l.y] = fs[k]; }
+    });
+#pragma unroll
+    for (int c = 0; c < 3; ++c) {
+        if (l.x7) xch[wave][18 + c][l.y] = uc[c];
+        if (l.x0) xch[wave][21 + c][l.y] = uc[c];
+    }
+    }
+    __syncthreads();
+    if (!active) return;
+    const int wlo = first ? 0 : wave - 1, whi = last ? NW - 1 : wave + 1;
+    static_for<0, Q>([&](auto kc) {
+        constexpr int k = decltype(kc)::value;
+        constexpr int cx = CX(k);
+        if constexpr (cx == 1) {
+            const float inner = dpp_from_lower_lane(fs[k]);
+            const float edge = first ? xedge[wave][0][k / 3][l.y] : xch[wlo][XSLOT(k)][l.y];
+            fs[k] = l.x0 ? edge : inner;
+        }
+        if constexpr (cx == -1) {
+            const float inner = dpp_from_upper_lane(fs[k]);
+            const float edge = last ? xedge[wave][1][k / 3][l.y] : xch[whi][XSLOT(k)][l.y];
+            fs[k] = l.x7 ? edge : inner;
+        }
+    });
+    float uE[3], uW[3];
+#pragma unroll
+    for (int c = 0; c < 3; ++c) {
+        const float e_edge = last ? xedge[wave][1][9 + c][l.y] : xch[whi][21 + c][l.y];
+        const float w_edge = first ? xedge[wave][0][9 + c][l.y] : xch[wlo][18 + c][l.y];
+        const float e_in = dpp_from_upper_lane(uc[c]), w_in = dpp_from_lower_lane(uc[c]);
+        uE[c] = l.x7 ? e_edge : e_in;
+        uW[c] = l.x0 ? w_edge : w_in;
+    }
+    finish_cell<false, false, true>(p, 0, own, fs, uE[0], uE[1], uE[2], uW[0], uW[1], uW[2], uN[0], uN[1], uN[2], uS[0], uS[1], uS[2],
+                                    uT[0], uT[1], uT[2], uB[0], uB[1], uB[2]);
+}
+
+__global__ __launch_bounds__(256) void k_materialise(const SCParams p, int64_t n_cells)
+{
+    const int64_t i = (int64_t)blockIdx.x * 256 + threadIdx.x;
+    if (i >= n_cells) return;
+    const int b = (int)(i >> 9);
+    const uint32_t cell = (uint32_t)(i & 511);
+    float r[R_COMP];
+    load_record(r, record_plane(p.rec_in, b, (int)(cell >> 6)), (cell & 63u) * 4);
+    const Own own{b, cell * 4};
+    st_f32(p.vel_out, b, V_BLOCK_BYTES, own.cell4, r[R_UX]);
+    st_f32(p.vel_out, b, V_BLOCK_BYTES, COMP_BYTES + own.cell4, r[R_UY]);
+    st_f32(p.vel_out, b, V_BLOCK_BYTES, 2 * COMP_BYTES + own.cell4, r[R_UZ]);
+    if (p.rho) st_f32(p.rho, b, S_BLOCK_BYTES, own.cell4, r[R_RHO]);
+    static_for<0, Q>([&](auto kc) {
+        constexpr int k = decltype(kc)::value;
+        st_f32(p.f_out, b, F_BLOCK_BYTES, k * COMP_BYTES + own.cell4,
+               collide_value<k>(r[R_RHO], r[R_UX], r[R_UY], r[R_UZ], r[R_PXX], r[R_PYY], r[R_PZZ], r[R_PXY], r[R_PYZ], r[R_PZX], r[R_OMO]));
+    });
 }
 
 __device__ __forceinline__ float weight_rt(int k)
diff --git a/open_ludwig_amd/csrc/ludwig_hip.hip b/open_ludwig_amd/csrc/ludwig_hip.hip
--- a/open_ludwig_amd/csrc/ludwig_hip.hip
+++ b/open_ludwig_amd/csrc/ludwig_hip.hip
@@ -61,6 +61,8 @@
 const char *rccl_lib() { return getenv("LUDWIG_RCCL_LIB"); }
 bool halo_self_via_rccl() { return is_set("LUDWIG_HALO_SELF_VIA_RCCL"); }
 bool halo_trace() { static const bool v = is_set("LUDWIG_HALO_TRACE"); return v; }
+bool record_step_off() { return flag("LUDWIG_RECORD_STEP") == 0; }
+int record_order() { const int v = flag("LUDWIG_RECORD_ORDER"); return v < 0 ? 1 : v; }
 
 }
 
@@ -186,6 +188,14 @@
     int32_t *iso_keys = nullptr;
     int64_t iso_capacity = 0;
     int64_t iso_n = -1;
+    float *rec[2] = {nullptr, nullptr};
+    bool f_valid[2] = {true, true}, rec_valid[2] = {false, false};
+    int rho_in_rec = -1;
+    int rec_eligible = -1;
+    bool rec_banned = false;
+    bool rec_hold = false;
+    int32_t *rec_items = nullptr;
+    int64_t n_record_steps = 0;
 };
 
 namespace {
@@ -217,6 +227,30 @@
 };
 
 int ensure_rho(LudwigLevel *L);
+
+int ensure_populations(LudwigLevel *L, int parity)
+{
+    for (int q = 0; q < 2; ++q) {
+        if ((parity >= 0 && parity != q) || L->f_valid[q]) continue;
+        LW_HIP(hipSetDevice(L->device));
+        SCParams p{};
+        p.rec_in = L->rec[q];
+        p.f_out = L->f[q];
+        p.vel_out = L->vel[q];
+        p.rho = L->rho_in_rec == q ? L->rho : nullptr;
+        hipLaunchKernelGGL(k_materialise, dim3((unsigned)((L->sk + 255) / 256)), dim3(256), 0, L->stream, p, L->sk);
+        LW_HIP(hipGetLastError());
+        L->f_valid[q] = true;
+        if (L->rho_in_rec == q) L->rho_in_rec = -1;
+    }
+    return LUDWIG_OK;
+}
+
+#define LW_ENSURE_POPULATIONS(L)                                                                          \
+    do {                                                                                                  \
+        const int rp_ = ensure_populations(const_cast<LudwigLevel *>(L), -1);                             \
+        if (rp_) return rp_;                                                                              \
+    } while (0)
 
 int materialize_old(LudwigLevel *L)
 {
@@ -233,6 +267,11 @@
 
 int before_external_write(LudwigLevel *L, int field)
 {
+    {
+        const int r = ensure_populations(L, -1);
+        if (r) return r;
+        L->rec_valid[0] = L->rec_valid[1] = false;
+    }
     bool feeds_rho = field == LUDWIG_SPONGE || field == LUDWIG_OBSTACLE || field == LUDWIG_RHO;
     for (int a = 0; a < N_PARTS; ++a)
         if (L->rho_replay[a].stale && (field == LUDWIG_F || field == LUDWIG_F_TEMP) && L->f[field == LUDWIG_F ? 0 : 1] == L->rho_replay[a].p.f_in) feeds_rho = true;
@@ -295,6 +334,7 @@
 
 int upload_meta(LudwigLevel *L)
 {
+    L->rec_eligible = -1;
     if (L->n_blocks == 0) return LUDWIG_OK;
     LW_HIP(hipMemcpyAsync(L->meta, L->h_meta.data(), L->h_meta.size() * 4, hipMemcpyHostToDevice, L->stream));
     LW_HIP(hipStreamSynchronize(L->stream));
@@ -320,6 +360,10 @@
 int set_items(LudwigLevel *L, int part, const int32_t *items, int64_t n)
 {
     std::vector<int32_t> cls[N_CLASSES];
+    if (part == LUDWIG_PART_ALL) {
+        L->rec_eligible = -1;
+        if (L->rec_items) { (void)hipFree(L->rec_items); L->rec_items = nullptr; }
+    }
     auto is_fast = [&](int b) { return (L->h_meta[(size_t)b * NBR_STRIDE + NBR_FLAGS] & FLAG_ALL_NEIGHBOURS) != 0; };
     for (int64_t i = 0; i < n; ++i) {
         if (items[i] >= 0) {
@@ -711,6 +755,98 @@
     return interface_launch(L, parent, part, p, t_sub, parent_tau, temporal_weight, true, L->stream);
 }
 
+int ban_records(LudwigLevel *L)
+{
+    L->rec_banned = true;
+    const bool behind = !L->f_valid[0] || !L->f_valid[1];
+    const int r = ensure_populations(L, -1);
+    if (r) return r;
+    L->rec_valid[0] = L->rec_valid[1] = false;
+    if (behind) LW_HIP(hipStreamSynchronize(L->stream));
+    return LUDWIG_OK;
+}
+
+bool record_level_ok(LudwigLevel *L)
+{
+    if (L->rec_eligible < 0) {
+        std::vector<int32_t> flags((size_t)L->n_blocks);
+        for (int b = 0; b < L->n_blocks; ++b) flags[b] = L->h_meta[(size_t)b * NBR_STRIDE + NBR_FLAGS];
+        const bool one_list = L->n_items_merged[LUDWIG_PART_ALL] == 0 && L->n_items[LUDWIG_PART_ALL][1] == 0 && L->n_items[LUDWIG_PART_ALL][2] > 0;
+        L->rec_eligible = one_list && ludwig_record_step_rule(flags.data(), L->n_blocks, L->n_owned, 0, L->has_temporal ? 1 : 0,
+                                                              (L->has_post || L->bouzidi_enabled) ? 1 : 0, 0) == 1;
+    }
+    return L->rec_eligible == 1;
+}
+
+int build_record_items(LudwigLevel *L)
+{
+    const int64_t n = L->n_items[LUDWIG_PART_ALL][2];
+    std::vector<int32_t> src((size_t)n), dst;
+    LW_HIP(hipMemcpy(src.data(), L->items[LUDWIG_PART_ALL][2], (size_t)n * 4, hipMemcpyDeviceToHost));
+    dst = src;
+    if (env::record_order() == 1) {
+        const int64_t n_wg = n / XRUN;
+        for (int64_t t0 = 0; t0 + 64 <= n_wg; t0 += 64)
+            for (int j = 0; j < 8; ++j)
+                for (int x = 0; x < 8; ++x)
+                    for (int w = 0; w < XRUN; ++w) dst[(size_t)(t0 + 8 * j + x) * XRUN + w] = src[(size_t)(t0 + 8 * x + j) * XRUN + w];
+    }
+    LW_HIP(hipMalloc((void **)&L->rec_items, (size_t)n * 4));
+    LW_HIP(hipMemcpy(L->rec_items, dst.data(), (size_t)n * 4, hipMemcpyHostToDevice));
+    return LUDWIG_OK;
+}
+
+int record_step_wanted(LudwigLevel *L, const LudwigLevel *parent, const LudwigStepFlags *fl, int part, bool *yes)
+{
+    *yes = false;
+    if (env::record_step_off() || L->rec_banned || L->rec_hold || L->external_writer || L->rho_old_pending || parent || part != LUDWIG_PART_ALL ||
+        fl->wall_model_active || !record_level_ok(L))
+        return LUDWIG_OK;
+    if (!L->rec[0]) {
+        const size_t bytes = (size_t)L->n_blocks * R_BLOCK_BYTES;
+        float *a = nullptr, *b = nullptr;
+        if (hipMalloc((void **)&a, bytes) != hipSuccess || hipMalloc((void **)&b, bytes) != hipSuccess) {
+            (void)hipGetLastError();
+            if (a) (void)hipFree(a);
+            L->rec_banned = true;
+            return LUDWIG_OK;
+        }
+        L->rec[0] = a; L->rec[1] = b;
+        L->device_bytes += (int64_t)(2 * bytes);
+    }
+    if (!L->rec_items) {
+        const int r = build_record_items(L);
+        if (r) return r;
+    }
+    *yes = true;
+    return LUDWIG_OK;
+}
+
+int launch_record_step(LudwigLevel *L, SCParams p, int in, int out, int64_t t_sub)
+{
+    if (t_sub != L->last_step_t) { ++L->step_count; L->last_step_t = t_sub; }
+    L->rho_replay[LUDWIG_PART_ALL].stale = false;
+    p.items = L->rec_items;
+    p.rec_out = L->rec[out];
+    p.store_rho = 0;
+    const dim3 grid((unsigned)(L->n_items[LUDWIG_PART_ALL][2] / XRUN)), block(64 * XRUN);
+    if (L->rec_valid[in]) {
+        p.rec_in = L->rec[in];
+        if ((uint64_t)L->n_blocks * R_BLOCK_BYTES >= (1ull << 32)) hipLaunchKernelGGL((k_step_records<XRUN, true>), grid, block, 0, L->stream, p);
+        else hipLaunchKernelGGL((k_step_records<XRUN, false>), grid, block, 0, L->stream, p);
+    } else if (L->wide) {
+        hipLaunchKernelGGL((k_records_from_populations<XRUN, true>), grid, block, 0, L->stream, p);
+    } else {
+        hipLaunchKernelGGL((k_records_from_populations<XRUN, false>), grid, block, 0, L->stream, p);
+    }
+    LW_HIP(hipGetLastError());
+    L->rec_valid[out] = true;
+    L->f_valid[out] = false;
+    L->rho_in_rec = out;
+    ++L->n_record_steps;
+    return LUDWIG_OK;
+}
+
 int launch_stream_collide(LudwigLevel *L, const LudwigLevel *parent, int64_t t_sub, float u_curr, float parent_tau,
                           float temporal_weight, const LudwigStepFlags *fl, int part)
 {
@@ -752,6 +888,19 @@
     p.seed = (int32_t)(t_sub % 1000000);
     p.sponge_blend = fl->sponge_blend_distributions ? 1 : 0;
 
+    if (parent && !parent->rec_banned) {
+        const int r = ban_records(const_cast<LudwigLevel *>(parent));
+        if (r) return r;
+    }
+    {
+        bool by_records = false;
+        int r = record_step_wanted(L, parent, fl, part, &by_records);
+        if (r) return r;
+        if (by_records) return launch_record_step(L, p, in, out, t_sub);
+        if ((r = ensure_populations(L, -1))) return r;
+        L->rec_valid[out] = false;
+    }
+
     if (parent && !parent->rho_eager) {
         LudwigLevel *pm = const_cast<LudwigLevel *>(parent);
         pm->rho_eager = true;
@@ -823,6 +972,10 @@
 
 int ensure_rho(LudwigLevel *L)
 {
+    if (L->rho_in_rec >= 0) {
+        const int r = ensure_populations(L, L->rho_in_rec);
+        if (r) return r;
+    }
     bool any = false;
     for (int a = 0; a < N_PARTS; ++a) any = any || L->rho_replay[a].stale;
     if (!any) return LUDWIG_OK;
@@ -980,6 +1133,9 @@
         if (L->source_mac2[a]) (void)hipFree(L->source_mac2[a]);
     }
     if (L->f_iface) (void)hipFree(L->f_iface);
+    if (L->rec[0]) (void)hipFree(L->rec[0]);
+    if (L->rec[1]) (void)hipFree(L->rec[1]);
+    if (L->rec_items) (void)hipFree(L->rec_items);
     if (L->stats) (void)hipFree(L->stats);
     if (L->grad) (void)hipFree(L->grad);
     if (L->subgrid_fields) (void)hipFree(L->subgrid_fields);
@@ -1420,6 +1576,12 @@
     if (!d.ptr || d.bytes == 0) return fail(LUDWIG_ERR_STATE, "field %d is not allocated on this level", field);
     if (bytes != d.bytes) return fail(LUDWIG_ERR_INVALID, "field %d: got %zu bytes, expected %zu", field, bytes, d.bytes);
     LW_HIP(hipSetDevice(L->device));
+    {
+        const bool p0 = field == LUDWIG_F || field == LUDWIG_VEL, p1 = field == LUDWIG_F_TEMP || field == LUDWIG_VEL_TEMP;
+        const int r = (p0 || p1) ? ensure_populations(const_cast<LudwigLevel *>(L), p0 ? 0 : 1)
+                                 : (field == LUDWIG_RHO ? LUDWIG_OK : ensure_populations(const_cast<LudwigLevel *>(L), -1));
+        if (r) return r;
+    }
     if (field == LUDWIG_RHO) {
         const int r = ensure_rho(const_cast<LudwigLevel *>(L));
         if (r) return r;
@@ -1487,7 +1649,10 @@
     const unsigned grid = (unsigned)((L->sk + 255) / 256);
     ++L->version;
     {
-        const int r = ensure_rho(L);
+        int r = ensure_populations(L, -1);
+        if (r) return r;
+        L->rec_valid[0] = L->rec_valid[1] = false;
+        r = ensure_rho(L);
         if (r) return r;
     }
     hipLaunchKernelGGL(k_fill_weights, dim3(grid), dim3(256), 0, L->stream, L->f[0], L->sk);
@@ -1560,6 +1725,7 @@
 
 #define LW_ENSURE_RHO(L)                                                                                  \
     do {                                                                                                  \
+        LW_ENSURE_POPULATIONS(L);                                                                         \
         const int r_ = ensure_rho(const_cast<LudwigLevel *>(L));                                          \
         if (r_) return r_;                                                                                \
     } while (0)
@@ -1805,6 +1971,7 @@
     struct : ObserverSchedule { LudwigTracers *set = nullptr; } tracers;
     struct : ObserverSchedule { LudwigFluxPlanes *set = nullptr; } fluxes;
     struct : ObserverSchedule { LudwigModes *set = nullptr; } modes;
+    bool any() const { return probes.set || surface.set || forces.set || tracers.set || fluxes.set || modes.set; }
 };
 struct BatchHook {
     const BatchObservers *obs = nullptr;
@@ -2174,6 +2341,7 @@
         return LUDWIG_OK;
     }
     LW_HIP(hipSetDevice(L->device));
+    LW_ENSURE_POPULATIONS(L);
     if (!L->grad) {
         const size_t n = (size_t)L->n_blocks * GRAD_COMPONENTS * CELLS;
         const int r = dev_alloc(L, &L->grad, n);
@@ -2341,6 +2509,7 @@
     }
     if (const int r = subgrid_model_known(L, "fields")) return r;
     LW_HIP(hipSetDevice(L->device));
+    LW_ENSURE_POPULATIONS(L);
     if (!L->subgrid_fields) {
         const size_t n = (size_t)L->n_blocks * SUBGRID_FIELD_COMPONENTS * CELLS;
         const int r = dev_alloc(L, &L->subgrid_fields, n);
@@ -2394,6 +2563,7 @@
     if (L->n_owned == 0) return LUDWIG_OK;
     if (const int r = subgrid_model_known(L, "statistics")) return r;
     LW_HIP(hipSetDevice(L->device));
+    LW_ENSURE_POPULATIONS(L);
     hipLaunchKernelGGL(k_subgrid<SUBGRID_SUMS>, dim3((unsigned)L->n_owned), dim3(CELLS / 2), 0, L->stream, L->subgrid_sums,
                        (const float *)vel_out(L, t_sub), (const uint8_t *)L->obstacle, (const int32_t *)L->meta, L->c_wale, L->nu_bg);
     LW_HIP(hipGetLastError());
@@ -3426,6 +3596,7 @@
 {
     const int64_t k = S->n_advances++;
     if (S->n_slots == 0) return LUDWIG_OK;
+    for (int li = 0; li < S->n_levels; ++li) LW_ENSURE_POPULATIONS(S->levels[li]);
     TracerArgs a = tracers_args(S, t_coarse);
     if (k % S->release_every == 0) a.released = (int32_t)((k / S->release_every) % S->generations);
     hipLaunchKernelGGL(k_tracers_advance, dim3((unsigned)((S->n_slots * 8 + 63) / 64)), dim3(64), 0, st, a);
@@ -3477,6 +3648,7 @@
     hipStream_t st = S->levels[0]->stream;
     const int r = tracers_join(S, st);
     if (r) return r;
+    for (int li = 0; li < S->n_levels; ++li) LW_ENSURE_POPULATIONS(S->levels[li]);
     const TracerArgs a = tracers_args(S, t_coarse);
     hipLaunchKernelGGL(k_tracers_snapshot, dim3((unsigned)((S->n_slots * 8 + 63) / 64)), dim3(64), 0, st, a);
     LW_HIP(hipGetLastError());
@@ -3672,6 +3844,8 @@
         }
     }
     for (int i = 0; i < n_levels; ++i) levels[i]->rho_old_pending = false;
+    const bool hold_records = n_levels > 1 || obs.any();
+    for (int i = 0; i < n_levels; ++i) levels[i]->rec_hold = hold_records;
     int rc = LUDWIG_OK;
     for (int32_t o = 0; o < batch_size && rc == LUDWIG_OK; ++o) {
         const int64_t t = t_start + o;
@@ -3695,6 +3869,7 @@
         }
         if (rc == LUDWIG_OK && e != hipSuccess) return fail(LUDWIG_ERR_HIP, "batch: %s", hipGetErrorString(e));
     }
+    for (int i = 0; i < n_levels; ++i) levels[i]->rec_hold = false;
     if (rc) return rc;
     return ludwig_sync(levels[0]);
 }
@@ -3767,6 +3942,7 @@
     const FieldDesc d = field_desc(L, field);
     if (!d.ptr || field == LUDWIG_OBSTACLE) return fail(LUDWIG_ERR_STATE, "field %d cannot be packed", field);
     LW_HIP(hipSetDevice(L->device));
+    LW_ENSURE_POPULATIONS(L);
     if (field == LUDWIG_RHO) {
         bool stale = false;
         for (int a = 0; a < N_PARTS; ++a) stale = stale || L->rho_replay[a].stale;
@@ -3795,6 +3971,23 @@
     LW_HIP(hipSetDevice(L->device));
     hipLaunchKernelGGL(k_scatter, dim3((unsigned)((n + 255) / 256)), dim3(256), 0, hip_stream ? (hipStream_t)hip_stream : L->stream, (float *)d.ptr, index_dev, n, src_dev, (const int32_t *)L->d_ref2int, L->sk, d.comps);
     LW_HIP(hipGetLastError());
+    return LUDWIG_OK;
+}
+
+int ludwig_record_step_rule(const int32_t *block_flags, int32_t n_blocks, int32_t n_owned, int32_t has_parent, int32_t has_temporal_storage,
+                            int32_t has_post_collision, int32_t wall_model_active)
+{
+    if (n_blocks < 0 || (n_blocks > 0 && !block_flags)) return fail(LUDWIG_ERR_INVALID, "record step rule: bad argument");
+    if (n_blocks == 0 || n_owned != n_blocks || has_parent || has_temporal_storage || has_post_collision || wall_model_active) return 0;
+    for (int32_t b = 0; b < n_blocks; ++b)
+        if (block_flags[b] != FLAG_ALL_NEIGHBOURS) return 0;
+    return 1;
+}
+
+int ludwig_level_record_steps(const LudwigLevel *L, int64_t *n_steps)
+{
+    if (!L || !n_steps) return fail(LUDWIG_ERR_INVALID, "null argument");
+    *n_steps = L->n_record_steps;
     return LUDWIG_OK;
 }
 
@@ -4085,6 +4278,7 @@
     if (out) *out = nullptr;
     if (!L || !desc || !out || desc->n_peers < 0 || (desc->n_peers > 0 && !desc->peer_ranks)) return fail(LUDWIG_ERR_INVALID, "bad argument");
     if (comm && comm->device != L->device) return fail(LUDWIG_ERR_INVALID, "communicator and level live on different devices");
+    if (const int r = ban_records(L)) return r;
     for (int p = 0; p < desc->n_peers; ++p) {
         const int r = desc->peer_ranks[p];
         if (comm ? (r < 0 || r >= comm->world) : r != 0) return fail(LUDWIG_ERR_INVALID, "peer %d: rank %d not in the communicator", p, r);
@@ -4183,6 +4377,7 @@
 {
     if (!P || group < 0 || group >= LUDWIG_HALO_GROUPS) return fail(LUDWIG_ERR_INVALID, "bad argument");
     LW_HIP(hipSetDevice(P->L->device));
+    LW_ENSURE_POPULATIONS(P->L);
     if (field == LUDWIG_RHO) { const int r = ensure_rho(P->L); if (r) return r; }
     return halo_pack_group(P, group, field, hip_stream ? (hipStream_t)hip_stream : P->L->stream);
 }
```
